# Stehsaer/nodey-audio-editor

Measured on AMD Instinct MI355X. Metric: stereo f32 sample-frames/s through the 4-node graph input->mix(2)->pitch->FFT-spectrum @48 kHz, higher is better.
Workload: dtype f32

## Files before the change

### include/nae_gpu.h

```cpp
#ifndef NAE_GPU_H
#define NAE_GPU_H
#include <stddef.h>
#include <stdint.h>

#ifdef __cplusplus
extern "C" {
#endif

#define NAE_ABI_VERSION 3

typedef enum nae_status {
    NAE_OK = 0,
    NAE_ERR_INVALID = -1,
    NAE_ERR_UNSUPPORTED = -2,
    NAE_ERR_HIP = -3,
    NAE_ERR_NOMEM = -4,
    NAE_ERR_STATE = -5
} nae_status;

typedef enum nae_fmt {
    NAE_FMT_S16 = 1, NAE_FMT_S32 = 2, NAE_FMT_FLT = 3, NAE_FMT_S16P = 6, NAE_FMT_S32P = 7, NAE_FMT_FLTP = 8
} nae_fmt;

typedef struct nae_ctx nae_ctx;
typedef struct nae_event nae_event;
typedef struct nae_stretch nae_stretch;
typedef struct nae_spectrum nae_spectrum;
typedef struct nae_fir nae_fir;
typedef struct nae_conv nae_conv;
typedef struct nae_eq nae_eq;
typedef struct nae_dyn nae_dyn;

int nae_abi_version(void);
int nae_device_count(void);
int nae_ctx_create(int device, nae_ctx** out);
int nae_ctx_destroy(nae_ctx* ctx);
int nae_ctx_set_stream(nae_ctx* ctx, void* hip_stream);
void* nae_ctx_stream(nae_ctx* ctx);
int nae_sync(nae_ctx* ctx);
int nae_poll(nae_ctx* ctx);
const char* nae_last_error(nae_ctx* ctx);
const char* nae_device_name(nae_ctx* ctx);

int nae_malloc(nae_ctx* ctx, size_t bytes, void** dptr);
int nae_free(nae_ctx* ctx, void* dptr);
int nae_malloc_host(nae_ctx* ctx, size_t bytes, void** hptr);
int nae_free_host(nae_ctx* ctx, void* hptr);
int nae_memcpy_h2d(nae_ctx* ctx, void* dst, const void* src_host, size_t bytes);
int nae_memcpy_d2h(nae_ctx* ctx, void* dst_host, const void* src, size_t bytes);
int nae_memcpy_d2d(nae_ctx* ctx, void* dst, const void* src, size_t bytes);
int nae_memset(nae_ctx* ctx, void* dst, int value, size_t bytes);

int nae_event_create(nae_ctx* ctx, nae_event** ev);
int nae_event_record(nae_ctx* ctx, nae_event* ev);
int nae_event_query(nae_event* ev);
int nae_ctx_wait_event(nae_ctx* ctx, nae_event* ev);
int nae_event_elapsed_ms(nae_event* start, nae_event* stop, float* ms);
int nae_event_destroy(nae_event* ev);

int nae_prof_enable(nae_ctx* ctx, int on);
int nae_prof_reset(nae_ctx* ctx);
int nae_prof_get(nae_ctx* ctx, int index, char* name, size_t name_cap, double* total_ms, uint64_t* launches);

int nae_debug_clock_ghz(nae_ctx* ctx, double* ghz);

int nae_debug_set(nae_ctx* ctx, const char* key, long long value);

int nae_debug_diff_u32(nae_ctx* ctx, const void* a, const void* b, size_t n_words, uint64_t* d_count);

int nae_fill_uniform_f32(nae_ctx* ctx, float* dst, size_t n_per_stream, size_t stream_stride, size_t n_streams,
                         uint64_t first_stream, uint64_t input_index);

typedef struct nae_sig {
    void* base;
    size_t stream_stride;
    size_t chan_stride;
    size_t frame_stride;
} nae_sig;

int nae_gain_f32(nae_ctx* ctx, const float* const* src_planes, float* const* dst_planes, int planes,
                 size_t elems, float volume);
int nae_gain_s16(nae_ctx* ctx, const int16_t* const* src_planes, int16_t* const* dst_planes, int planes,
                 size_t elems, float volume);
int nae_gain_s32(nae_ctx* ctx, const int32_t* const* src_planes, int32_t* const* dst_planes, int planes,
                 size_t elems, float volume);
int nae_gain_frame(nae_ctx* ctx, int fmt, const void* const* src_planes, void* const* dst_planes, size_t S,
                   int ch, float volume);

int nae_deinterleave_f32(nae_ctx* ctx, const float* src, float* const* dst_planes, size_t S, int ch);
int nae_interleave_f32(nae_ctx* ctx, const float* const* src_planes, float* dst, size_t S, int ch);
int nae_copy_sig_f32(nae_ctx* ctx, const nae_sig* src, const nae_sig* dst, size_t S, int ch, size_t n_streams);
int nae_gain_sig_f32(nae_ctx* ctx, const nae_sig* src, const nae_sig* dst, size_t S, int ch, size_t n_streams,
                     float volume);

int nae_amix_f32(nae_ctx* ctx, const float* const* inL, const float* const* inR, const float* vol_host, int n,
                 float* outL, float* outR, size_t S);
int nae_amix_sig_f32(nae_ctx* ctx, const nae_sig* inputs, const float* vol_host, int n, const nae_sig* out,
                     size_t S, size_t n_streams);

int nae_bimix_f32(nae_ctx* ctx, const float* ll, const float* lr, const float* rl, const float* rr, float bias,
                  float* outL, float* outR, size_t S);

int nae_bimix2_downmix_f32(nae_ctx* ctx, const float* l, const float* r, float* mono, size_t S);
int nae_bimix2_interleave_f32(nae_ctx* ctx, float* dst, const float* earlier, const float* later,
                              size_t unaligned, size_t aligned, int earlier_offset);

int nae_to_f32_interleaved(nae_ctx* ctx, int fmt, const void* const* planes, size_t S, int ch, float* dst);

int nae_clamp_f32(nae_ctx* ctx, float* data, size_t n);

typedef struct nae_stretch_plan {
    int pv_on, rs_on;
    double tempo_eff, rate_eff;
    int64_t ha_q24;
    int32_t d0;
    uint32_t r_q24[2];
    uint64_t step_q32;
    size_t out_len, mid_len, frames;
    int rs_first;
} nae_stretch_plan;
int nae_stretch_plan_make(double rate, double pitch, size_t in_len, nae_stretch_plan* plan);

int nae_stretch_block_f32(nae_ctx* ctx, double rate, double pitch, const nae_sig* src, size_t in_len, int ch,
                          size_t n_streams, const nae_sig* dst);
int nae_debug_pv_tile_phase(nae_ctx* ctx, double rate, double pitch, const nae_sig* src, size_t in_len, int ch,
                            size_t n_streams, int32_t* dst_host, size_t dst_capacity, size_t* n_tiles,
                            size_t* tile_frames);

#define NAE_STRETCH_PHASE_LOCK 1u
int nae_stretch_block_ex_f32(nae_ctx* ctx, double rate, double pitch, unsigned flags, const nae_sig* src, size_t in_len, int ch,
                             size_t n_streams, const nae_sig* dst);
int nae_debug_pv_tile_phase_ex(nae_ctx* ctx, double rate, double pitch, unsigned flags, const nae_sig* src, size_t in_len, int ch,
                               size_t n_streams, int32_t* dst_host, size_t dst_capacity, size_t* n_tiles, size_t* tile_frames);

int nae_stretch_create(nae_ctx* ctx, int sample_rate, int channels, float rate, float pitch, nae_stretch** h);
int nae_stretch_create_ex(nae_ctx* ctx, int sample_rate, int channels, float rate, float pitch, unsigned flags, nae_stretch** h);

int nae_stretch_plan_make_n(double rate, double pitch, int n_fft, size_t in_len, nae_stretch_plan* plan);
int nae_stretch_block_n_f32(nae_ctx* ctx, double rate, double pitch, unsigned flags, int n_fft, const nae_sig* src, size_t in_len, int ch,
                            size_t n_streams, const nae_sig* dst);
int nae_debug_pv_tile_phase_n(nae_ctx* ctx, double rate, double pitch, unsigned flags, int n_fft, const nae_sig* src, size_t in_len, int ch,
                              size_t n_streams, int32_t* dst_host, size_t dst_capacity, size_t* n_tiles, size_t* tile_frames);
int nae_stretch_create_n(nae_ctx* ctx, int sample_rate, int channels, float rate, float pitch, unsigned flags, int n_fft, nae_stretch** h);

int nae_stretch_formant_lifter(int sample_rate, int n_fft);
int nae_stretch_block_formant_f32(nae_ctx* ctx, double rate, double pitch, unsigned flags, int n_fft, int lifter,
                                  const nae_sig* src, size_t in_len, int ch, size_t n_streams, const nae_sig* dst);
int nae_stretch_create_formant(nae_ctx* ctx, int sample_rate, int channels, float rate, float pitch, unsigned flags,
                               int n_fft, int lifter, nae_stretch** h);

int nae_stretch_plan_make_shift(double rate, double pitch, double formant_ratio, int lifter, int n_fft, size_t in_len, nae_stretch_plan* plan);
int nae_stretch_block_formant_shift_f32(nae_ctx* ctx, double rate, double pitch, unsigned flags, int n_fft, int lifter, double formant_ratio,
                                        const nae_sig* src, size_t in_len, int ch, size_t n_streams, const nae_sig* dst);
int nae_stretch_create_formant_shift(nae_ctx* ctx, int sample_rate, int channels, float rate, float pitch, unsigned flags, int n_fft, int lifter,
                                     double formant_ratio, nae_stretch** h);

#define NAE_STRETCH_TRANSIENTS 4u
#define NAE_STRETCH_LINK_CHANNELS 16u
int nae_stretch_put(nae_stretch* h, const float* interleaved, size_t S);
int nae_stretch_put_host(nae_stretch* h, const float* interleaved_host, size_t S);
int nae_stretch_flush(nae_stretch* h);
size_t nae_stretch_available(nae_stretch* h);
int nae_stretch_receive(nae_stretch* h, float* dst, size_t max_frames, size_t* got);
int nae_stretch_receive_host(nae_stretch* h, float* dst_host, size_t max_frames, size_t* got);
int nae_stretch_destroy(nae_stretch* h);

typedef struct nae_wsola nae_wsola;
typedef struct nae_wsola_plan {
    int sample_rate, channels;
    double rate_eff, tempo_eff;
    int order;
    int overlap_len, seq_len, seek_len, sample_req;
    double nominal_skip;
    size_t in_len, flush_zeros;
    size_t n_seq;
    size_t td_out_len, aa_out_len, cu_out_len;
    size_t out_len;
} nae_wsola_plan;
int nae_wsola_plan_make(int sample_rate, int channels, double rate, double pitch, size_t in_len, nae_wsola_plan* plan);
int nae_wsola_block_f32(nae_ctx* ctx, int sample_rate, double rate, double pitch, const nae_sig* src, size_t in_len, int ch,
                        size_t n_streams, const nae_sig* dst, int32_t* offsets_dbg);
int nae_wsola_create(nae_ctx* ctx, int sample_rate, int channels, double rate, double pitch, nae_wsola** h);
int nae_wsola_put(nae_wsola* h, const float* interleaved, size_t S);
int nae_wsola_put_host(nae_wsola* h, const float* interleaved_host, size_t S);
int nae_wsola_flush(nae_wsola* h);
size_t nae_wsola_available(const nae_wsola* h);
int nae_wsola_receive(nae_wsola* h, float* dst, size_t max_frames, size_t* got);
int nae_wsola_receive_host(nae_wsola* h, float* dst_host, size_t max_frames, size_t* got);
int nae_wsola_destroy(nae_wsola* h);

typedef struct nae_swr nae_swr;
int nae_swr_create(nae_ctx* ctx, int in_fmt, int in_rate, int in_channels, int out_rate, nae_swr** h);
int nae_swr_convert_host(nae_swr* h, const void* const* planes_host, size_t n_in, float* outL_host, float* outR_host,
                         size_t max_out, size_t* n_out);
int nae_swr_convert(nae_swr* h, const void* const* planes_host, size_t n_in, float* outL_dev, float* outR_dev,
                    size_t max_out, size_t* n_out);
size_t nae_swr_buffered(nae_swr* h);
int nae_swr_destroy(nae_swr* h);
int nae_mono_to_stereo_f32(nae_ctx* ctx, const float* mono, float* dst_interleaved, size_t S, float gain);

size_t nae_spectrum_frames(size_t T);
int nae_spectrum_block_f32(nae_ctx* ctx, const nae_sig* src, size_t T, int ch, size_t n_streams, float* dst,
                           size_t dst_stream_stride);
size_t nae_spectrum_frames_ex(size_t T, int n_fft, int hop);
int nae_spectrum_block_ex_f32(nae_ctx* ctx, int n_fft, int hop, const nae_sig* src, size_t T, int ch, size_t n_streams, float* dst,
                              size_t dst_stream_stride);
int nae_spectrum_create(nae_ctx* ctx, int n_fft, int hop, int channels, nae_spectrum** h);
int nae_spectrum_put(nae_spectrum* h, const float* interleaved, size_t S);
size_t nae_spectrum_available(nae_spectrum* h);
int nae_spectrum_receive(nae_spectrum* h, float* dst, size_t max_frames, size_t* got);
int nae_spectrum_destroy(nae_spectrum* h);

int nae_fir_pick_n_fft(int n_taps);
int nae_fir_block_f32(nae_ctx* ctx, const float* taps_host, int n_taps, int n_fft, const nae_sig* src, size_t in_len, int ch, size_t n_streams,
                      const nae_sig* dst);
int nae_fir_create(nae_ctx* ctx, const float* taps_host, int n_taps, int n_fft, int channels, nae_fir** h);
int nae_fir_put(nae_fir* h, const float* interleaved, size_t S);
int nae_fir_put_host(nae_fir* h, const float* interleaved_host, size_t S);
int nae_fir_flush(nae_fir* h);
// ... 74 lines not shown
```

### nodey-audio-editor_amd/binding.py

```python
from __future__ import annotations

import ctypes as C
import os
import subprocess
from typing import Iterable, Optional, Sequence

import numpy as np

_HERE = os.path.dirname(os.path.abspath(__file__))

FMT_S16, FMT_S32, FMT_FLT, FMT_S16P, FMT_S32P, FMT_FLTP = 1, 2, 3, 6, 7, 8
FFT_N, HOP, BINS = 1024, 256, 513

EXPORTED_SYMBOLS = [
    "nae_abi_version", "nae_device_count", "nae_ctx_create", "nae_ctx_destroy", "nae_ctx_set_stream",
    "nae_ctx_stream", "nae_sync", "nae_poll", "nae_last_error", "nae_device_name", "nae_malloc", "nae_free",
    "nae_memcpy_h2d", "nae_memcpy_d2h", "nae_memcpy_d2d", "nae_memset", "nae_event_create", "nae_event_record",
    "nae_event_query", "nae_ctx_wait_event", "nae_debug_graph4_stages",
    "nae_event_elapsed_ms", "nae_event_destroy", "nae_prof_enable", "nae_prof_reset", "nae_prof_get",
    "nae_malloc_host", "nae_free_host", "nae_debug_clock_ghz", "nae_debug_set", "nae_debug_diff_u32", "nae_fill_uniform_f32", "nae_gain_f32", "nae_gain_s16", "nae_gain_s32", "nae_gain_frame",
    "nae_deinterleave_f32", "nae_interleave_f32", "nae_copy_sig_f32", "nae_gain_sig_f32", "nae_amix_f32",
    "nae_amix_sig_f32", "nae_bimix_f32", "nae_bimix2_downmix_f32", "nae_bimix2_interleave_f32",
    "nae_to_f32_interleaved", "nae_clamp_f32", "nae_stretch_plan_make", "nae_stretch_block_f32",
    "nae_debug_pv_tile_phase", "nae_stretch_block_ex_f32", "nae_debug_pv_tile_phase_ex", "nae_stretch_create_ex",
    "nae_stretch_plan_make_n", "nae_stretch_block_n_f32", "nae_debug_pv_tile_phase_n", "nae_stretch_create_n",
    "nae_stretch_formant_lifter", "nae_stretch_block_formant_f32", "nae_stretch_create_formant",
    "nae_stretch_plan_make_shift", "nae_stretch_block_formant_shift_f32", "nae_stretch_create_formant_shift", "nae_stretch_create", "nae_stretch_put", "nae_stretch_put_host", "nae_stretch_flush",
    "nae_stretch_available", "nae_stretch_receive", "nae_stretch_receive_host", "nae_stretch_destroy",
    "nae_swr_create", "nae_swr_convert_host", "nae_swr_convert", "nae_swr_buffered", "nae_swr_destroy", "nae_mono_to_stereo_f32",
    "nae_spectrum_frames", "nae_spectrum_block_f32", "nae_spectrum_frames_ex", "nae_spectrum_block_ex_f32", "nae_spectrum_create", "nae_spectrum_put",
    "nae_spectrum_available", "nae_spectrum_receive", "nae_spectrum_destroy", "nae_graph4_run",
    "nae_wsola_plan_make", "nae_wsola_block_f32", "nae_wsola_create", "nae_wsola_put", "nae_wsola_put_host",
    "nae_wsola_flush", "nae_wsola_available", "nae_wsola_receive", "nae_wsola_receive_host", "nae_wsola_destroy",
    "nae_fir_pick_n_fft", "nae_fir_block_f32", "nae_fir_design", "nae_fir_create", "nae_fir_put", "nae_fir_put_host", "nae_fir_flush",
    "nae_fir_available", "nae_fir_receive", "nae_fir_receive_host", "nae_fir_destroy",
    "nae_conv_pick_n_fft", "nae_conv_block_f32", "nae_conv_reverb_taps", "nae_conv_design_reverb", "nae_conv_create", "nae_conv_put",
    "nae_conv_put_host", "nae_conv_flush", "nae_conv_available", "nae_conv_receive", "nae_conv_receive_host", "nae_conv_destroy",
    "nae_eq_design", "nae_eq_block_f32", "nae_eq_create", "nae_eq_put", "nae_eq_put_host", "nae_eq_flush", "nae_eq_available", "nae_eq_receive",
    "nae_eq_receive_host", "nae_eq_destroy",
    "nae_dyn_design", "nae_dyn_block_f32", "nae_dyn_create", "nae_dyn_put", "nae_dyn_put_host", "nae_dyn_flush", "nae_dyn_available",
    "nae_dyn_receive", "nae_dyn_receive_host", "nae_dyn_destroy",
]


STRETCH_PHASE_LOCK = 1
STRETCH_TRANSIENTS = 4
STRETCH_LINK_CHANNELS = 16
FORMANT_SHIFT_MIN, FORMANT_SHIFT_MAX = 0.25, 4.0
FIR_SIZES = (512, 1024, 2048, 4096)
FIR_KINDS = {"lowpass": 0, "highpass": 1, "bandpass": 2, "bandstop": 3}
EQ_KINDS = ("peak", "lowshelf", "highshelf", "lowpass", "highpass", "notch")
HANDLE_PREFIXES = ("nae_stretch", "nae_wsola", "nae_fir", "nae_conv", "nae_eq", "nae_dyn")


class NaeError(RuntimeError):
    pass


def lib_path() -> str:
    return os.environ.get("NAE_GPU_LIB") or os.path.join(_HERE, "libnae_gpu.so")


def build_library(verbose: bool = False) -> str:
    r = subprocess.run(["make", "-C", _HERE, "-j4"], capture_output=True, text=True)
    if verbose or r.returncode:
        print(r.stdout[-4000:], r.stderr[-4000:])
    if r.returncode:
        raise NaeError("building libnae_gpu.so failed")
    return lib_path()


class Sig(C.Structure):
    _fields_ = [("base", C.c_void_p), ("stream_stride", C.c_size_t), ("chan_stride", C.c_size_t),
                ("frame_stride", C.c_size_t)]

    @staticmethod
    def interleaved(ptr: int, S: int, ch: int, shared: bool = False, stream_stride: Optional[int] = None) -> "Sig":
        ss = 0 if shared else (S * ch if stream_stride is None else stream_stride)
        return Sig(ptr, ss, 1, ch)

    @staticmethod
    def planar(ptr: int, S: int, ch: int, shared: bool = False, plane_stride: Optional[int] = None,
               stream_stride: Optional[int] = None) -> "Sig":
        ps = S if plane_stride is None else plane_stride
        ss = 0 if shared else (ps * ch if stream_stride is None else stream_stride)
        return Sig(ptr, ss, ps, 1)


class DynParams(C.Structure):
    _fields_ = [("threshold_db", C.c_double), ("slope", C.c_double), ("knee_db", C.c_double), ("alpha_attack", C.c_double),
                ("alpha_release", C.c_double), ("makeup_db", C.c_double), ("lookahead", C.c_int), ("link", C.c_int)]


class StretchPlan(C.Structure):
    _fields_ = [("pv_on", C.c_int), ("rs_on", C.c_int), ("tempo_eff", C.c_double), ("rate_eff", C.c_double),
                ("ha_q24", C.c_int64), ("d0", C.c_int32), ("r_q24", C.c_uint32 * 2), ("step_q32", C.c_uint64),
                ("out_len", C.c_size_t), ("mid_len", C.c_size_t), ("frames", C.c_size_t), ("rs_first", C.c_int)]


class WsolaPlan(C.Structure):
    _fields_ = [("sample_rate", C.c_int), ("channels", C.c_int), ("rate_eff", C.c_double), ("tempo_eff", C.c_double),
                ("order", C.c_int), ("overlap_len", C.c_int), ("seq_len", C.c_int), ("seek_len", C.c_int),
                ("sample_req", C.c_int), ("nominal_skip", C.c_double), ("in_len", C.c_size_t),
                ("flush_zeros", C.c_size_t), ("n_seq", C.c_size_t), ("td_out_len", C.c_size_t),
                ("aa_out_len", C.c_size_t), ("cu_out_len", C.c_size_t), ("out_len", C.c_size_t)]


class Graph4(C.Structure):
    _fields_ = [("in_a", Sig), ("in_b", Sig), ("vol_a", C.c_float), ("vol_b", C.c_float), ("mix_out", Sig),
                ("rate", C.c_double), ("pitch", C.c_double), ("pitch_out", Sig), ("spec_out", C.c_void_p),
                ("spec_stream_stride", C.c_size_t), ("S", C.c_size_t), ("n_streams", C.c_size_t)]


_lib = None


def load_library() -> C.CDLL:
    global _lib
    if _lib is not None:
        return _lib
    p = lib_path()
    if not os.path.exists(p):
        raise NaeError(f"{p} is missing: run `python -c 'import __graft_entry__ as g; g.build()'` (hipcc, gfx950)")
    lib = C.CDLL(p)
    vp, sz, i, u, f, d = C.c_void_p, C.c_size_t, C.c_int, C.c_uint, C.c_float, C.c_double
    P = C.POINTER
    sigs = {
        "nae_abi_version": (i, []), "nae_device_count": (i, []),
        "nae_ctx_create": (i, [i, P(vp)]), "nae_ctx_destroy": (i, [vp]), "nae_ctx_set_stream": (i, [vp, vp]),
        "nae_ctx_stream": (vp, [vp]), "nae_sync": (i, [vp]), "nae_poll": (i, [vp]),
        "nae_last_error": (C.c_char_p, [vp]), "nae_device_name": (C.c_char_p, [vp]),
        "nae_malloc": (i, [vp, sz, P(vp)]), "nae_free": (i, [vp, vp]),
        "nae_memcpy_h2d": (i, [vp, vp, vp, sz]), "nae_memcpy_d2h": (i, [vp, vp, vp, sz]),
        "nae_memcpy_d2d": (i, [vp, vp, vp, sz]), "nae_memset": (i, [vp, vp, i, sz]),
        "nae_event_create": (i, [vp, P(vp)]), "nae_event_record": (i, [vp, vp]),
        "nae_event_query": (i, [vp]), "nae_ctx_wait_event": (i, [vp, vp]), "nae_debug_graph4_stages": (i, [vp, P(Graph4), i]),
        "nae_event_elapsed_ms": (i, [vp, vp, P(f)]), "nae_event_destroy": (i, [vp]),
        "nae_prof_enable": (i, [vp, i]), "nae_prof_reset": (i, [vp]),
        "nae_prof_get": (i, [vp, i, C.c_char_p, sz, P(d), P(C.c_uint64)]),
        "nae_malloc_host": (i, [vp, sz, P(vp)]), "nae_free_host": (i, [vp, vp]),
        "nae_debug_clock_ghz": (i, [vp, P(C.c_double)]), "nae_debug_set": (i, [vp, C.c_char_p, C.c_longlong]),
        "nae_debug_diff_u32": (i, [vp, vp, vp, sz, vp]),
        "nae_fill_uniform_f32": (i, [vp, vp, sz, sz, sz, C.c_uint64, C.c_uint64]),
        "nae_gain_f32": (i, [vp, P(vp), P(vp), i, sz, f]), "nae_gain_s16": (i, [vp, P(vp), P(vp), i, sz, f]),
        "nae_gain_s32": (i, [vp, P(vp), P(vp), i, sz, f]),
        "nae_gain_frame": (i, [vp, i, P(vp), P(vp), sz, i, f]),
        "nae_deinterleave_f32": (i, [vp, vp, P(vp), sz, i]), "nae_interleave_f32": (i, [vp, P(vp), vp, sz, i]),
        "nae_copy_sig_f32": (i, [vp, P(Sig), P(Sig), sz, i, sz]),
        "nae_gain_sig_f32": (i, [vp, P(Sig), P(Sig), sz, i, sz, f]),
        "nae_amix_f32": (i, [vp, P(vp), P(vp), P(f), i, vp, vp, sz]),
        "nae_amix_sig_f32": (i, [vp, P(Sig), P(f), i, P(Sig), sz, sz]),
        "nae_bimix_f32": (i, [vp, vp, vp, vp, vp, f, vp, vp, sz]),
        "nae_bimix2_downmix_f32": (i, [vp, vp, vp, vp, sz]),
        "nae_bimix2_interleave_f32": (i, [vp, vp, vp, vp, sz, sz, i]),
        "nae_to_f32_interleaved": (i, [vp, i, P(vp), sz, i, vp]), "nae_clamp_f32": (i, [vp, vp, sz]),
        "nae_stretch_plan_make": (i, [d, d, sz, P(StretchPlan)]),
        "nae_stretch_block_f32": (i, [vp, d, d, P(Sig), sz, i, sz, P(Sig)]),
        "nae_debug_pv_tile_phase": (i, [vp, d, d, P(Sig), sz, i, sz, vp, sz, P(sz), P(sz)]),
        "nae_stretch_block_ex_f32": (i, [vp, d, d, u, P(Sig), sz, i, sz, P(Sig)]),
        "nae_debug_pv_tile_phase_ex": (i, [vp, d, d, u, P(Sig), sz, i, sz, vp, sz, P(sz), P(sz)]),
        "nae_stretch_create_ex": (i, [vp, i, i, f, f, u, P(vp)]),
        "nae_stretch_plan_make_n": (i, [d, d, i, sz, P(StretchPlan)]),
        "nae_stretch_block_n_f32": (i, [vp, d, d, u, i, P(Sig), sz, i, sz, P(Sig)]),
        "nae_debug_pv_tile_phase_n": (i, [vp, d, d, u, i, P(Sig), sz, i, sz, vp, sz, P(sz), P(sz)]),
        "nae_stretch_create_n": (i, [vp, i, i, f, f, u, i, P(vp)]),
        "nae_stretch_formant_lifter": (i, [i, i]),
        "nae_stretch_block_formant_f32": (i, [vp, d, d, u, i, i, P(Sig), sz, i, sz, P(Sig)]),
        "nae_stretch_create_formant": (i, [vp, i, i, f, f, u, i, i, P(vp)]),
        "nae_stretch_plan_make_shift": (i, [d, d, d, i, i, sz, P(StretchPlan)]),
        "nae_stretch_block_formant_shift_f32": (i, [vp, d, d, u, i, i, d, P(Sig), sz, i, sz, P(Sig)]),
        "nae_stretch_create_formant_shift": (i, [vp, i, i, f, f, u, i, i, d, P(vp)]),
        "nae_stretch_create": (i, [vp, i, i, f, f, P(vp)]),
        "nae_swr_create": (i, [vp, i, i, i, i, P(vp)]),
        "nae_swr_convert_host": (i, [vp, P(vp), sz, vp, vp, sz, P(sz)]), "nae_swr_convert": (i, [vp, P(vp), sz, vp, vp, sz, P(sz)]),
        "nae_swr_buffered": (sz, [vp]),
        "nae_swr_destroy": (i, [vp]), "nae_mono_to_stereo_f32": (i, [vp, vp, vp, sz, f]),
        "nae_spectrum_frames": (sz, [sz]), "nae_spectrum_block_f32": (i, [vp, P(Sig), sz, i, sz, vp, sz]),
        "nae_spectrum_frames_ex": (sz, [sz, i, i]), "nae_spectrum_block_ex_f32": (i, [vp, i, i, P(Sig), sz, i, sz, vp, sz]),
        "nae_spectrum_create": (i, [vp, i, i, i, P(vp)]), "nae_spectrum_put": (i, [vp, vp, sz]),
        "nae_spectrum_available": (sz, [vp]), "nae_spectrum_receive": (i, [vp, vp, sz, P(sz)]),
        "nae_spectrum_destroy": (i, [vp]), "nae_graph4_run": (i, [vp, P(Graph4)]),
        "nae_wsola_plan_make": (i, [i, i, d, d, sz, P(WsolaPlan)]),
        "nae_wsola_block_f32": (i, [vp, i, d, d, P(Sig), sz, i, sz, P(Sig), vp]),
        "nae_wsola_create": (i, [vp, i, i, d, d, P(vp)]),
        "nae_fir_pick_n_fft": (i, [i]), "nae_fir_block_f32": (i, [vp, vp, i, i, P(Sig), sz, i, sz, P(Sig)]),
        "nae_fir_design": (i, [i, i, d, d, i, vp]), "nae_fir_create": (i, [vp, vp, i, i, i, P(vp)]),
        "nae_conv_pick_n_fft": (i, [i]), "nae_conv_block_f32": (i, [vp, vp, i, i, i, P(Sig), sz, i, sz, P(Sig)]),
        "nae_conv_reverb_taps": (i, [i, d, d]), "nae_conv_design_reverb": (i, [i, d, d, d, d, C.c_uint64, i, vp]),
        "nae_conv_create": (i, [vp, vp, i, i, i, i, P(vp)]),
        "nae_eq_design": (i, [i, i, d, d, d, vp]), "nae_eq_block_f32": (i, [vp, vp, i, P(Sig), sz, i, sz, P(Sig)]),
        "nae_eq_create": (i, [vp, vp, i, i, P(vp)]),
        "nae_dyn_design": (i, [i, d, d, d, d, d, d, d, i, P(DynParams)]), "nae_dyn_block_f32": (i, [vp, P(DynParams), P(Sig), sz, i, sz, P(Sig)]),
        "nae_dyn_create": (i, [vp, P(DynParams), i, P(vp)]),
    }
    for prefix in HANDLE_PREFIXES:
        sigs.update({prefix + "_put": (i, [vp, vp, sz]), prefix + "_put_host": (i, [vp, vp, sz]), prefix + "_flush": (i, [vp]),
                     prefix + "_available": (sz, [vp]), prefix + "_receive": (i, [vp, vp, sz, P(sz)]),
                     prefix + "_receive_host": (i, [vp, vp, sz, P(sz)]), prefix + "_destroy": (i, [vp])})
    for name, (res, args) in sigs.items():
        fn = getattr(lib, name)
        fn.restype = res
        fn.argtypes = args
    _lib = lib
    return lib


class DeviceArray:

    def __init__(self, ctx: "Context", shape: Sequence[int], dtype=np.float32):
        self.ctx = ctx
        self.shape = tuple(int(x) for x in (shape if isinstance(shape, (tuple, list)) else (shape,)))
        self.dtype = np.dtype(dtype)
        self.nbytes = int(np.prod(self.shape, dtype=np.int64)) * self.dtype.itemsize
        p = C.c_void_p()
        ctx._ck(ctx.lib.nae_malloc(ctx.h, max(self.nbytes, 16), C.byref(p)))
        self.ptr = p.value
        ctx._allocs.add(self)

    @property
    def size(self) -> int:
        return self.nbytes // self.dtype.itemsize

    def at(self, elem_offset: int) -> int:
        return self.ptr + int(elem_offset) * self.dtype.itemsize

    def upload(self, host: np.ndarray) -> "DeviceArray":
        host = np.ascontiguousarray(host, dtype=self.dtype)
        assert host.nbytes == self.nbytes, (host.nbytes, self.nbytes)
        self.ctx._ck(self.ctx.lib.nae_memcpy_h2d(self.ctx.h, self.ptr, host.ctypes.data, self.nbytes))
        self.ctx.sync()
        return self

    def download(self) -> np.ndarray:
        out = np.empty(self.shape, self.dtype)
        self.ctx._ck(self.ctx.lib.nae_memcpy_d2h(self.ctx.h, out.ctypes.data, self.ptr, self.nbytes))
        self.ctx.sync()
        return out

    def zero(self) -> "DeviceArray":
        self.ctx._ck(self.ctx.lib.nae_memset(self.ctx.h, self.ptr, 0, self.nbytes))
        return self

    def free(self) -> None:
        if self.ptr:
            self.ctx.sync()
            self.ctx.lib.nae_free(self.ctx.h, self.ptr)
            self.ptr = 0
            self.ctx._allocs.discard(self)


def _ptr_array(ptrs: Iterable[int]):
    ptrs = list(ptrs)
    return (C.c_void_p * len(ptrs))(*ptrs)


class Context:

    def __init__(self, device: int = 0):
        self.lib = load_library()
        h = C.c_void_p()
        rc = self.lib.nae_ctx_create(device, C.byref(h))
        if rc != 0:
            why = ("no such device, or a bad assignment in $NAE_DEBUG" if rc == -1 else "no usable HIP device")
            raise NaeError(f"nae_ctx_create(device={device}) failed with {rc}: {why} — this library has no CPU fallback")
        self.h = h
        self.device = device
        self._allocs = set()
        self._pinned = {}

    def _ck(self, rc: int) -> None:
        if rc != 0:
            raise NaeError(f"nae error {rc}: {self.lib.nae_last_error(self.h).decode(errors='replace')}")

    def name(self) -> str:
        return self.lib.nae_device_name(self.h).decode()

    def sync(self) -> None:
        self._ck(self.lib.nae_sync(self.h))

    def poll(self) -> int:
        return self.lib.nae_poll(self.h)

    def set_stream(self, hip_stream: int) -> None:
        self._ck(self.lib.nae_ctx_set_stream(self.h, C.c_void_p(hip_stream)))

    def empty(self, shape, dtype=np.float32) -> DeviceArray:
        return DeviceArray(self, shape, dtype)

    def array(self, host: np.ndarray) -> DeviceArray:
        host = np.ascontiguousarray(host)
        return DeviceArray(self, host.shape, host.dtype).upload(host)

    def close(self) -> None:
        if self.h:
            for a in list(self._allocs):
                a.free()
            self.lib.nae_ctx_destroy(self.h)
            self.h = None

    def __enter__(self):
        return self

    def __exit__(self, *a):
        self.close()

    def debug_set(self, key: str, value: int) -> "Context":
        self._ck(self.lib.nae_debug_set(self.h, key.encode(), int(value)))
        return self

    def event(self) -> C.c_void_p:
        e = C.c_void_p()
        self._ck(self.lib.nae_event_create(self.h, C.byref(e)))
        return e

    def destroy_event(self, ev) -> None:
        rc = self.lib.nae_event_destroy(ev)
        if rc:
            raise NaeError(f"nae_event_destroy failed: {rc}")

    def record(self, ev) -> None:
        self._ck(self.lib.nae_event_record(self.h, ev))

    def query(self, ev) -> int:
        rc = self.lib.nae_event_query(ev)
        if rc < 0:
            raise NaeError(f"nae_event_query failed: {rc}")
        return rc

    def wait_event(self, ev) -> None:
        self._ck(self.lib.nae_ctx_wait_event(self.h, ev))

    def elapsed_ms(self, a, b) -> float:
        ms = C.c_float()
        rc = self.lib.nae_event_elapsed_ms(a, b, C.byref(ms))
        if rc:
            raise NaeError(f"nae_event_elapsed_ms failed: {rc}")
        return float(ms.value)

    def prof_enable(self, on: bool = True) -> None:
        self._ck(self.lib.nae_prof_enable(self.h, 1 if on else 0))

    def prof_reset(self) -> None:
        self._ck(self.lib.nae_prof_reset(self.h))

    def prof_report(self) -> dict:
        out = {}
        n = self.lib.nae_prof_get(self.h, -1, None, 0, None, None)
        for k in range(n):
            name = C.create_string_buffer(128)
            ms, cnt = C.c_double(), C.c_uint64()
            self.lib.nae_prof_get(self.h, k, name, 128, C.byref(ms), C.byref(cnt))
            out[name.value.decode()] = (ms.value, cnt.value)
        return out

    def pinned(self, shape, dtype=np.float32) -> np.ndarray:
        shape = tuple(int(x) for x in (shape if isinstance(shape, (tuple, list)) else (shape,)))
        nbytes = int(np.prod(shape, dtype=np.int64)) * np.dtype(dtype).itemsize
        p = C.c_void_p()
        self._ck(self.lib.nae_malloc_host(self.h, max(nbytes, 16), C.byref(p)))
        buf = (C.c_char * max(nbytes, 16)).from_address(p.value)
        arr = np.frombuffer(buf, dtype=dtype, count=int(np.prod(shape, dtype=np.int64))).reshape(shape)
        self._pinned[arr.ctypes.data] = p.value
        return arr

    def free_pinned(self, arr: np.ndarray) -> None:
        p = self._pinned.pop(arr.ctypes.data, None)
        if p:
            self.sync()
            self.lib.nae_free_host(self.h, p)

    def diff_words(self, a: int, b: int, n_words: int, d_count: int) -> None:
        self._ck(self.lib.nae_debug_diff_u32(self.h, a, b, n_words, d_count))

    def clock_ghz(self) -> float:
        g = C.c_double()
        self._ck(self.lib.nae_debug_clock_ghz(self.h, C.byref(g)))
        return g.value

    def fill_uniform(self, dst: int, n_per_stream: int, stream_stride: int, n_streams: int, first_stream: int = 0,
                     input_index: int = 0) -> None:
        self._ck(self.lib.nae_fill_uniform_f32(self.h, dst, n_per_stream, stream_stride, n_streams, first_stream,
                                               input_index))

    def gain(self, fmt_dtype, src_planes: Sequence[int], dst_planes: Sequence[int], elems: int, volume: float):
        fn = {np.dtype(np.float32): self.lib.nae_gain_f32, np.dtype(np.int16): self.lib.nae_gain_s16,
              np.dtype(np.int32): self.lib.nae_gain_s32}[np.dtype(fmt_dtype)]
        self._ck(fn(self.h, _ptr_array(src_planes), _ptr_array(dst_planes), len(src_planes), elems, volume))

    def gain_frame(self, fmt: int, src_planes, dst_planes, S: int, ch: int, volume: float) -> int:
        return self.lib.nae_gain_frame(self.h, fmt, _ptr_array(src_planes), _ptr_array(dst_planes), S, ch, volume)

    def deinterleave(self, src: int, dst_planes: Sequence[int], S: int, ch: int):
        self._ck(self.lib.nae_deinterleave_f32(self.h, src, _ptr_array(dst_planes), S, ch))

    def interleave(self, src_planes: Sequence[int], dst: int, S: int, ch: int):
        self._ck(self.lib.nae_interleave_f32(self.h, _ptr_array(src_planes), dst, S, ch))

    def copy_sig(self, src: Sig, dst: Sig, S: int, ch: int, n_streams: int):
        self._ck(self.lib.nae_copy_sig_f32(self.h, C.byref(src), C.byref(dst), S, ch, n_streams))

    def gain_sig(self, src: Sig, dst: Sig, S: int, ch: int, n_streams: int, volume: float):
        self._ck(self.lib.nae_gain_sig_f32(self.h, C.byref(src), C.byref(dst), S, ch, n_streams, volume))

    def amix(self, inL: Sequence[int], inR: Sequence[int], vol: Sequence[float], outL: int, outR: int, S: int):
        n = len(inL)
        v = (C.c_float * n)(*[float(x) for x in vol])
        self._ck(self.lib.nae_amix_f32(self.h, _ptr_array(inL), _ptr_array(inR), v, n, outL, outR, S))

    def amix_sig(self, inputs: Sequence[Sig], vol: Sequence[float], out: Sig, S: int, n_streams: int):
        n = len(inputs)
        arr = (Sig * n)(*inputs)
        v = (C.c_float * n)(*[float(x) for x in vol])
        self._ck(self.lib.nae_amix_sig_f32(self.h, arr, v, n, C.byref(out), S, n_streams))

    def bimix(self, ll, lr, rl, rr, bias: float, outL, outR, S: int):
        self._ck(self.lib.nae_bimix_f32(self.h, ll, lr, rl, rr, bias, outL, outR, S))

    def bimix2_downmix(self, l, r, mono, S: int):
        self._ck(self.lib.nae_bimix2_downmix_f32(self.h, l, r, mono, S))

    def bimix2_interleave(self, dst, earlier, later, unaligned: int, aligned: int, earlier_offset: int):
        self._ck(self.lib.nae_bimix2_interleave_f32(self.h, dst, earlier, later, unaligned, aligned, earlier_offset))

    def to_f32_interleaved(self, fmt: int, planes: Sequence[int], S: int, ch: int, dst: int) -> int:
        return self.lib.nae_to_f32_interleaved(self.h, fmt, _ptr_array(planes), S, ch, dst)

    def clamp(self, data: int, n: int):
        self._ck(self.lib.nae_clamp_f32(self.h, data, n))

    @staticmethod
    def stretch_plan(rate: float, pitch: float, in_len: int, n_fft: int = 1024, formant: int = 0,
                     formant_ratio: Optional[float] = None) -> StretchPlan:
        pl = StretchPlan()
        if formant_ratio is not None:
            rc = load_library().nae_stretch_plan_make_shift(rate, pitch, formant_ratio, formant, n_fft, in_len, C.byref(pl))
        elif n_fft == 1024:
            rc = load_library().nae_stretch_plan_make(rate, pitch, in_len, C.byref(pl))
        else:
            rc = load_library().nae_stretch_plan_make_n(rate, pitch, n_fft, in_len, C.byref(pl))
        if rc:
            raise NaeError(f"nae_stretch_plan_make({rate}, {pitch}, n_fft={n_fft}) failed: {rc}")
        return pl

    def stretch_block(self, rate: float, pitch: float, src: Sig, in_len: int, ch: int, n_streams: int, dst: Sig,
                      phase_lock: bool = False, n_fft: int = 1024, formant: int = 0, transients: bool = False,
                      formant_ratio: Optional[float] = None, link_channels: bool = False):
        flags = (STRETCH_PHASE_LOCK if phase_lock else 0) | (STRETCH_TRANSIENTS if transients else 0) | (STRETCH_LINK_CHANNELS if link_channels else 0)
        if formant_ratio is not None:
            self._ck(self.lib.nae_stretch_block_formant_shift_f32(self.h, rate, pitch, flags, n_fft, formant, formant_ratio,
                                                                  C.byref(src), in_len, ch, n_streams, C.byref(dst)))
        elif formant:
            self._ck(self.lib.nae_stretch_block_formant_f32(self.h, rate, pitch, flags, n_fft, formant,
                                                            C.byref(src), in_len, ch, n_streams, C.byref(dst)))
        elif n_fft != 1024 or transients or link_channels:
            self._ck(self.lib.nae_stretch_block_n_f32(self.h, rate, pitch, flags, n_fft, C.byref(src), in_len,
                                                      ch, n_streams, C.byref(dst)))
        elif phase_lock:
            self._ck(self.lib.nae_stretch_block_ex_f32(self.h, rate, pitch, STRETCH_PHASE_LOCK, C.byref(src), in_len, ch, n_streams,
                                                       C.byref(dst)))
        else:
            self._ck(self.lib.nae_stretch_block_f32(self.h, rate, pitch, C.byref(src), in_len, ch, n_streams, C.byref(dst)))

# ... 234 lines not shown
```

### nodey-audio-editor_amd/csrc/kernels_pvpipe.hip

```cpp
#include "stft_common.h"
#include "pv_roles.h"

namespace nae {

constexpr int kPipeSlots = 4;
constexpr int kPipeThreads = 64 * 4 * kPipeSlots;
constexpr size_t kPipeLdsTables = NAE_FFT_N * sizeof(float) + (kT1024Pad + 64 + kTwaCf) * sizeof(cf);

constexpr size_t kPipeLdsPerSlot = (2 * kPadScratchCf + kYCf) * sizeof(cf);
constexpr int pipe_ola_gens(int kG) { return kG >= 3 ? 2 : 3; }
constexpr size_t kPipeXchgPerSlot = 1024;
constexpr size_t pipe_lds_x_per_slot(int kG) { return kG == 1 ? kPipeXchgPerSlot : 3 * kPhasePad * sizeof(uint32_t) + (size_t)pipe_ola_gens(kG) * 3 * kOlaQuarter * sizeof(float); }
constexpr size_t pipe_lds(int kG) { return kPipeLdsTables + kPipeSlots * (kPipeLdsPerSlot + pipe_lds_x_per_slot(kG)); }
static_assert(2 * pipe_lds(1) <= 160 * 1024, "two workgroups per CU");
static_assert(pipe_lds(2) <= 160 * 1024 && pipe_lds(4) <= 160 * 1024, "one workgroup per CU");

__device__ unsigned g_cu_arrivals[8 * 4 * 16];

template <bool kUnit, int kG, bool kRich>
__global__ __launch_bounds__(kPipeThreads, kRich ? 4 : 8) void pv_pipe_kernel(SigViewD src, PvParams p, long long n_sc,
                                                                            const uint32_t* __restrict__ base_phase, OutViewD out, Tables tb)
{
    static_assert(kPipeSlots % kG == 0, "a unit's frames share a workgroup");
    static_assert(kG == 1 || kRich, "the frame-interleaved modes run one workgroup per CU");
    constexpr int kUnits = kPipeSlots / kG;
    constexpr int kDepth = kG == 1 ? 2 : 4;
    constexpr int kGens = pipe_ola_gens(kG);
    extern __shared__ __attribute__((aligned(16))) unsigned char smem[];
    float* hann; cf *t1024, *w64, *twa;
    stage_tables(smem, tb, kPipeThreads, hann, t1024, w64, twa);
    __shared__ int s_slot;
    if (kG == 1 && threadIdx.x == 0) s_slot = pipe_cu_arrival(g_cu_arrivals);
    __syncthreads();
    const int prio_slot = kG == 1 ? __builtin_amdgcn_readfirstlane(s_slot) : 0;

    const int wave = wave_id();
    const int role = wave / kPipeSlots, slot = wave % kPipeSlots;
    const int unit = slot / kG, j = slot % kG;
    const int lane = threadIdx.x & 63;
    PipeItem it;
    if (!pipe_item(p, (long long)kUnits * blockIdx.x + unit, n_sc, it)) return;
    const int c = it.c, n = it.n;
    const long long sc = it.sc, b0 = it.b0, b_end = it.b_end, f_first = it.f_first;

    cf* S1 = reinterpret_cast<cf*>(smem + kPipeLdsTables + slot * kPipeLdsPerSlot);
    cf* Y = S1 + kPadScratchCf;
    cf* S3 = Y + kYCf;
    unsigned char* xbase = smem + kPipeLdsTables + kPipeSlots * kPipeLdsPerSlot;
    constexpr size_t kXPer = pipe_lds_x_per_slot(kG);
    auto x_qa = [&](int sl, int gen) { return reinterpret_cast<uint32_t*>(xbase + sl * kXPer) + gen * kPhasePad; };
    auto x_inc = [&](int sl) { return reinterpret_cast<uint32_t*>(xbase + sl * kXPer) + 2 * kPhasePad; };
    auto x_ola = [&](int sl, int gen) { return reinterpret_cast<float*>(xbase + sl * kXPer + 3 * kPhasePad * sizeof(uint32_t)) + gen * 3 * kOlaQuarter; };

    const int steps = (n + kG - 1) / kG;
    const bool dense_shape = kG == 1 && p.ch == 2 && out.fs == 2 && out.cs == 1;
    const int T = steps + kDepth + (dense_shape ? 1 : 0);
    unsigned long long now = 0;
    if (kG > 1 && role == 2) __builtin_amdgcn_s_setprio(1);

    if (role == 0) {
        ChanView in{src.base + it.s_idx * src.ss + c * src.cs, src.fs, p.in_len};
        cf nxt[8], va[8];
        if (j < n) load_frame_raw<kUnit>(nxt, in, frame_start(p, f_first + j), lane);
        FftRegs R;
        if (kRich) load_fft_regs_lds(R, hann, twa, w64, lane);
#pragma unroll 1
        for (int t = 0; t < T; t++) {
            const bool cur = kG * t + j < n;
            pipe_barrier();
            if (kG == 1) pipe_prio(prio_slot, role, now);
            if (cur) r1_window_pass_a<kRich>(va, nxt, R, hann, twa, lane);
            pipe_barrier();
            if (kG == 1) now = __builtin_amdgcn_s_memtime();
            if (cur) {
                const FftLds L = make_fft_lds(S1, twa, w64, pipe_lane<!kRich>(lane));
                cf none[8];
                fft512_pad_bc_g<kRich, false>(va, L, R.tb, nullptr, none);
                r1_store_z(S1, L, va, lane);
                if (kG * (t + 1) + j < n) load_frame_raw<kUnit>(nxt, in, frame_start(p, f_first + kG * (t + 1) + j), lane);
            }
        }
    } else if (role <= 2) {
        PhaseLane P;
        P.init(tb, role - 1, lane);
        uint32_t qs[5], qp[5];
        P.load_base(qs, base_phase, p, it);
#pragma unroll
        for (int q = 0; q < 5; q++) qp[q] = 0;
        cf hx[5];
        uint32_t hqa[5] = {0, 0, 0, 0, 0};
#pragma unroll
        for (int q = 0; q < 5; q++) hx[q] = cf{0.0f, 0.0f};
#pragma unroll 1
        for (int t = 0; t < T; t++) {
            const int ia = kG * (t - 1) + j;
            const bool act_a = t >= 1 && ia < n;
            const long long fa = f_first + ia;
            const int ib = ia - kG;
            const bool act_b = kG > 1 && t >= 2 && ib < n;
            const long long fb = f_first + ib;
            pipe_barrier();
            if (kG == 1) pipe_prio(prio_slot, role, now);
            cf va[5];
            if (act_a) {
                cf A[2], B[2], z256{0.0f, 0.0f};
                P.read_z(S1, A, B, z256);
                P.split(A, B, z256, va);
            }
            if (kG > 1) {
                uint32_t inc[5] = {0, 0, 0, 0, 0};
                if (act_b && fb >= b0) {
                    uint32_t pv[5] = {0, 0, 0, 0, 0};
                    if (fb != 0) P.read5(j > 0 ? x_qa(slot - 1, (t - 1) & 1) : x_qa(slot + kG - 1, t & 1), pv);
                    P.inc_of_frame(p, fb, hqa, pv, inc);
                }
                P.write5(x_inc(slot), inc);
            }
            pipe_barrier();
            if (kG == 1) now = __builtin_amdgcn_s_memtime();
            uint32_t qa[5] = {0, 0, 0, 0, 0};
            if (act_a) P.phases(va, qa);
            if (kG == 1) {
                if (act_a) {
                    if (fa >= b0) {
                        if (fa == 0) {
#pragma unroll
                            for (int q = 0; q < 5; q++) qs[q] += qa[q];
                        } else {
                            const unsigned d = (unsigned)(frame_start(p, fa) - frame_start(p, fa - 1));
                            const unsigned R = (d == (unsigned)p.d0) ? p.r_q24_0 : p.r_q24_1;
                            uint32_t inc[5];
                            P.inc_items(qa, qp, d, R, inc);
#pragma unroll
                            for (int q = 0; q < 5; q++) qs[q] += inc[q];
                        }
                    }
#pragma unroll
                    for (int q = 0; q < 5; q++) qp[q] = qa[q];
                    if (fa == p.carry_frame) P.carry_store(p, sc, qs);
                    if (fa >= b0) P.synth_items(Y, va, qs, qa);
                }
            } else {
                if (act_a) P.write5(x_qa(slot, t & 1), qa);
                if (act_b) {
                    uint32_t iv[kG][5], mine[5];
#pragma unroll
                    for (int i2 = 0; i2 < kG; i2++) P.read5(x_inc(slot - j + i2), iv[i2]);
                    r2_running_phase<kG>(qs, mine, iv, j);
                    if (fb == p.carry_frame) P.carry_store(p, sc, mine);
                    if (fb >= b0) P.synth_items(Y, hx, mine, hqa);
                }
                if (act_a) {
#pragma unroll
                    for (int q = 0; q < 5; q++) { hx[q] = va[q]; hqa[q] = qa[q]; }
                }
            }
        }
    } else {
        float* optr = out.base + it.s_idx * out.ss + c * out.cs;
        const BlockOut bo{optr, out.fs, (out.fs == 1) && ((reinterpret_cast<uintptr_t>(optr) & 15) == 0)};
        float r0[4] = {0.0f, 0.0f, 0.0f, 0.0f}, r1[4] = {0.0f, 0.0f, 0.0f, 0.0f}, r2[4] = {0.0f, 0.0f, 0.0f, 0.0f};
        float y0[4] = {0.0f, 0.0f, 0.0f, 0.0f};
        FftRegs R;
        if (kRich) load_fft_regs_lds(R, hann, twa, w64, lane);
        bool had = false;
        const bool dense = dense_shape && ((reinterpret_cast<uintptr_t>(optr - c) & 15) == 0);
        int pend_be = -1;
        auto xchg = [&]() { return reinterpret_cast<cf*>(xbase + (size_t)(slot & ~1) * kPipeXchgPerSlot); };
#pragma unroll 1
        for (int t = 0; t < T; t++) {
            const int iz = kG * (t - (kDepth - (kG == 1 ? 0 : 1))) + j;
            const long long fz = f_first + iz;
            const bool active = iz >= 0 && iz < n && fz >= b0;
            pipe_barrier();
            if (kG == 1) pipe_prio(prio_slot, role, now);
            if (kG == 1 && pend_be >= 0) {
                const int lx = pipe_lane<!kRich>(lane);
                const cf* XB = xchg();
                r3_store_dense_half(optr - c, pend_be, c, lds_ld(XB + (0 + c) * 64 + lx), lds_ld(XB + (2 + c) * 64 + lx), lx);
                pend_be = -1;
            }
            cf zs[8];
            float4 oq[3];
            const bool finish = kG > 1 && had && fz - kG - 3 >= b0;
            if (finish) {
                const int lq = pipe_lane<!kRich>(lane);
#pragma unroll
                for (int i = 3; i >= 1; i--) {
                    int sl, gen;
                    r3_quarter_source<kG>(slot, j, i, t, kGens, sl, gen);
                    oq[i - 1] = *reinterpret_cast<const float4*>(x_ola(sl, gen) + (i - 1) * kOlaQuarter + 4 * lq);
                }
            }
            if (active) {
                const int la = pipe_lane<!kRich>(lane);
                const cf* Zi = Y + la;
                const cf* ta = twa + la;
#pragma unroll
                for (int r = 0; r < 8; r++) zs[r] = lds_ld(Zi + 64 * r);
                if (kRich) {
                    fft512_pad_a_tw(zs, R.ta);
                } else {
                    cf tw[7];
#pragma unroll
                    for (int q = 0; q < 7; q++) tw[q] = lds_ld(ta + 64 * q);
                    fft512_pad_a_tw(zs, tw);
                }
            }
            if (finish) {
                float o[4];
                r3_ola_finish(oq, y0, o);
                r3_store_block(p, it, bo, fz - kG - 3, o, pipe_lane<!kRich>(lane));
            }
            pipe_barrier();
            if (kG == 1) now = __builtin_amdgcn_s_memtime();
            had = active;
            if (active) {
                const int lb = pipe_lane<!kRich>(lane);
                const FftLds L = make_fft_lds(S3, twa, w64, lb);
                const cf* hw = reinterpret_cast<const cf*>(hann) + lb;
                cf wn[8];
                fft512_pad_bc_g<kRich, !kRich>(zs, L, R.tb, hw, wn);
                if (kRich) {
#pragma unroll
                    for (int r = 0; r < 8; r++) wn[r] = R.w[r];
                }
                float y[4][4];
                r3_window(zs, wn, y);
                if (kG == 1) {
                    float o[4];
                    r3_ola_shift(r0, r1, r2, y, o);
                    const long long be = fz - 3;
                    if (dense && be >= b0 && be < b_end && (be + 1) * NAE_HOP <= p.mid_len) {
                        const int lx = pipe_lane<!kRich>(lane);
                        cf* XB = xchg();
                        lds_st(XB + (2 * c + 0) * 64 + lx, cf{o[0], o[1]});
                        lds_st(XB + (2 * c + 1) * 64 + lx, cf{o[2], o[3]});
                        pend_be = (int)be;
                    } else {
                        r3_store_block(p, it, bo, be, o, pipe_lane<!kRich>(lane));
                    }
                } else {
                    float* po = x_ola(slot, t % kGens) + 4 * lb;
#pragma unroll
                    for (int q = 1; q < 4; q++) *reinterpret_cast<float4*>(po + (q - 1) * kOlaQuarter) = float4{y[q][0], y[q][1], y[q][2], y[q][3]};
#pragma unroll
                    for (int i = 0; i < 4; i++) y0[i] = y[0][i];
                }
            }
        }
    }
}

constexpr int flow_ola_gens(int kG) { return kG == 1 ? 0 : kG == 2 ? 4 : 3; }
constexpr size_t kFlowBuf = kPadScratchCf * sizeof(cf);
constexpr size_t flow_lds_per_slot(int kG)
{
    return 4 * kFlowBuf + (kG == 1 ? 0 : 4 * kPhasePad * sizeof(uint32_t) + (size_t)flow_ola_gens(kG) * 3 * kOlaQuarter * sizeof(float));
}
constexpr size_t flow_lds(int kG) { return kPipeSlots * flow_lds_per_slot(kG); }
static_assert(flow_lds(1) <= 160 * 1024 && flow_lds(2) <= 160 * 1024 && flow_lds(4) <= 160 * 1024, "one workgroup per CU");

template <bool kUnit, int kG>
__global__ __launch_bounds__(kPipeThreads, 4) void pv_flow_kernel(SigViewD src, PvParams p, long long n_sc, const uint32_t* __restrict__ base_phase,
                                                                  OutViewD out, Tables tb)
{
    static_assert(kPipeSlots % kG == 0, "a unit's frames share a workgroup");
    constexpr int kUnits = kPipeSlots / kG;
    constexpr int kGens = flow_ola_gens(kG);
    constexpr size_t kPer = flow_lds_per_slot(kG);
    extern __shared__ __attribute__((aligned(16))) unsigned char smem[];
// ... 49 lines not shown
#pragma unroll
        for (int q = 0; q < 5; q++) qp[q] = 0;
        cf x1[5], x2[5];
        uint32_t qa1[5] = {0, 0, 0, 0, 0}, qa2[5] = {0, 0, 0, 0, 0};
        uint32_t pcur[5] = {0, 0, 0, 0, 0};
#pragma unroll
        for (int q = 0; q < 5; q++) { x1[q] = cf{0.0f, 0.0f}; x2[q] = cf{0.0f, 0.0f}; }
#pragma unroll 1
        for (int t = 0; t < T; t++) {
            const int ia = kG * (t - 1) + j;
            const bool act_a = t >= 1 && ia < n;
            const long long fa = f_first + ia;
            const int ib = ia - kG;
            const bool act_b = kG > 1 && t >= 2 && ib < n;
            const long long fb = f_first + ib;
            const int ic = ib - kG;
            const bool act_c = kG > 1 && t >= 3 && ic < n;
            const long long fc = f_first + ic;
            const int gen = t & 1, old = gen ^ 1;
            pipe_barrier();
            cf A[2], B[2], z256{0.0f, 0.0f};
            if (act_a) P.read_z(x_z(slot, old), A, B, z256);
            uint32_t pv[5] = {0, 0, 0, 0, 0}, pnext[5] = {0, 0, 0, 0, 0}, iv[kG > 1 ? kG : 1][5];
            if (kG > 1) {
                if (j > 0) {
                    P.read5(x_qa(slot - 1, old), pv);
                } else {
                    P.read5(x_qa(slot + kG - 1, old), pnext);
#pragma unroll
                    for (int q = 0; q < 5; q++) pv[q] = pcur[q];
                }
                if (act_c) {
#pragma unroll
                    for (int i2 = 0; i2 < kG; i2++) P.read5(x_inc(slot - j + i2, old), iv[i2]);
                }
            }
            cf va[5];
            uint32_t qa[5] = {0, 0, 0, 0, 0};
            if (act_a) {
                P.split(A, B, z256, va);
                P.phases(va, qa);
            }
            if (kG == 1) {
                if (act_a) {
                    if (fa >= b0) {
                        uint32_t inc[5];
                        P.inc_of_frame(p, fa, qa, qp, inc);
#pragma unroll
                        for (int q = 0; q < 5; q++) qs[q] += inc[q];
                    }
#pragma unroll
                    for (int q = 0; q < 5; q++) qp[q] = qa[q];
                    if (fa == p.carry_frame) P.carry_store(p, sc, qs);
                    if (fa >= b0) P.synth_items(x_y(slot, gen), va, qs, qa);
                }
            } else {
                if (act_a) P.write5(x_qa(slot, gen), qa);
                uint32_t inc[5] = {0, 0, 0, 0, 0};
                if (act_b && fb >= b0) P.inc_of_frame(p, fb, qa1, pv, inc);
                P.write5(x_inc(slot, gen), inc);
                if (act_c) {
                    uint32_t mine[5];
                    r2_running_phase<(kG > 1 ? kG : 1)>(qs, mine, iv, j);
                    if (fc == p.carry_frame) P.carry_store(p, sc, mine);
                    if (fc >= b0) P.synth_items(x_y(slot, gen), x2, mine, qa2);
                }
#pragma unroll
                for (int q = 0; q < 5; q++) { x2[q] = x1[q]; qa2[q] = qa1[q]; pcur[q] = pnext[q]; }
                if (act_a) {
#pragma unroll
                    for (int q = 0; q < 5; q++) { x1[q] = va[q]; qa1[q] = qa[q]; }
                }
            }
        }
    } else {
        float* optr = out.base + it.s_idx * out.ss + c * out.cs;
        const BlockOut bo{optr, out.fs, (out.fs == 1) && ((reinterpret_cast<uintptr_t>(optr) & 15) == 0)};
        float r0[4] = {0.0f, 0.0f, 0.0f, 0.0f}, r1[4] = {0.0f, 0.0f, 0.0f, 0.0f}, r2[4] = {0.0f, 0.0f, 0.0f, 0.0f};
        float y0[4] = {0.0f, 0.0f, 0.0f, 0.0f};
        FftRegs R;
        load_fft_regs_global(R, tb, lane);
        bool had = false;
        const bool dense = dense_shape && ((reinterpret_cast<uintptr_t>(optr - c) & 15) == 0);
        int pend_be = -1;
        cf keep{0.0f, 0.0f};
#pragma unroll 1
        for (int t = 0; t < T; t++) {
            const int iz = kG * (t - kR3Lag) + j;
            const long long fz = f_first + iz;
            const bool active = iz >= 0 && iz < n && fz >= b0;
            pipe_barrier();
            cf zs[8];
            cf* Yi = x_y(slot, (t & 1) ^ 1);
            cf xh{0.0f, 0.0f};
            if (kG == 1 && pend_be >= 0) xh = lds_ld(x_y(slot ^ 1, t & 1) + 512 + lane);
            float4 oq[3];
            const bool finish = kG > 1 && had && fz - kG - 3 >= b0;
            if (finish) {
#pragma unroll
                for (int i = 3; i >= 1; i--) {
                    int sl, gen;
                    r3_quarter_source<kG>(slot, j, i, t, kGens > 0 ? kGens : 1, sl, gen);
                    oq[i - 1] = *reinterpret_cast<const float4*>(x_ola(sl, gen) + (i - 1) * kOlaQuarter + 4 * lane);
                }
            }
            if (active) {
#pragma unroll
                for (int r = 0; r < 8; r++) zs[r] = lds_ld(Yi + lane + 64 * r);
            }
            if (kG == 1 && pend_be >= 0) {
                r3_store_dense_half(optr - c, pend_be, c, c == 0 ? keep : xh, c == 0 ? xh : keep, lane);
                pend_be = -1;
            }
            if (finish) {
                float o[4];
                r3_ola_finish(oq, y0, o);
                r3_store_block(p, it, bo, fz - kG - 3, o, lane);
            }
            had = active;
            if (active) {
                fft512_pad_a_tw(zs, R.ta);
                const FftLds L = make_fft_lds(Yi, nullptr, nullptr, lane);
                cf none[8];
                fft512_pad_bc_g<true, false>(zs, L, R.tb, nullptr, none);
                float y[4][4];
                r3_window(zs, R.w, y);
                if (kG == 1) {
                    float o[4];
                    r3_ola_shift(r0, r1, r2, y, o);
                    const long long be = fz - 3;
                    if (dense && be >= b0 && be < b_end && (be + 1) * NAE_HOP <= p.mid_len) {
                        lds_st(Yi + 512 + lane, c == 0 ? cf{o[2], o[3]} : cf{o[0], o[1]});
                        keep = c == 0 ? cf{o[0], o[1]} : cf{o[2], o[3]};
                        pend_be = (int)be;
                    } else {
                        r3_store_block(p, it, bo, be, o, lane);
                    }
                } else {
                    float* po = x_ola(slot, t % (kGens > 0 ? kGens : 1)) + 4 * lane;
#pragma unroll
                    for (int q = 1; q < 4; q++) *reinterpret_cast<float4*>(po + (q - 1) * kOlaQuarter) = float4{y[q][0], y[q][1], y[q][2], y[q][3]};
#pragma unroll
                    for (int i = 0; i < 4; i++) y0[i] = y[0][i];
                }
            }
        }
    }
}

}

using namespace nae;

template <int kG, typename K>
static int pv_launch(nae_ctx* ctx, const char* name, K kernel, size_t lds, const PvJob& j)
{
    const Tables tb{ctx->d_w512, ctx->d_t1024, ctx->d_hann};
    return nae_launch_tiles(ctx, name, "pv_pipe_kernel: grid too large", kernel, j.n_sc * j.p.n_tiles, kPipeSlots / kG, kPipeThreads, lds, j.src, j.p,
                            j.n_sc, j.phase_ws, j.out, tb);
}

template <int kG, bool kRich>
static int pipe_launch(nae_ctx* ctx, const PvJob& j)
{
    return with_flags(j.unit_stride, [&](auto u) { return pv_launch<kG>(ctx, "pv_pipe_kernel", &pv_pipe_kernel<u.value, kG, kRich>, pipe_lds(kG), j); });
}
template <int kG>
static int flow_launch(nae_ctx* ctx, const PvJob& j)
{
    return with_flags(j.unit_stride, [&](auto u) { return pv_launch<kG>(ctx, "pv_flow_kernel", &pv_flow_kernel<u.value, kG>, flow_lds(kG), j); });
}

int nae_launch_pv_pipe(nae_ctx* ctx, const PvJob& j, int frames_per_step)
{
    const long long items = j.n_sc * j.p.n_tiles;
    if (items == 0) return NAE_OK;
    if (frames_per_step != 1 && frames_per_step != 2 && frames_per_step != 4) return nae_fail(ctx, NAE_ERR_INVALID, "pv_pipe_kernel: frames per step");
    const int units = kPipeSlots / frames_per_step;
    const long long groups = (items + units - 1) / units;
    const bool one_per_cu = groups <= (long long)ctx->n_cu && !ctx->pv_lean;
    if (one_per_cu && (ctx->pv_flow >= 2 || (ctx->pv_flow == 1 && frames_per_step == 1))) {
        if (frames_per_step == 1) return flow_launch<1>(ctx, j);
        if (frames_per_step == 2) return flow_launch<2>(ctx, j);
        return flow_launch<4>(ctx, j);
    }
    if (frames_per_step == 1) return with_flags(one_per_cu, [&](auto rich) { return pipe_launch<1, rich.value>(ctx, j); });
    if (frames_per_step == 2) return pipe_launch<2, true>(ctx, j);
    return pipe_launch<4, true>(ctx, j);
}
```

### nodey-audio-editor_amd/csrc/kernels_stft.hip

```cpp
#include "stft_common.h"
#include <stdlib.h>

namespace nae {

constexpr size_t kLdsPhase = kLdsTablesPad + kWaves * kPadScratchCf * sizeof(cf);
static_assert(3 * kLdsPhase <= 160 * 1024, "three workgroups per CU");
template <bool kUnit>
__global__ __launch_bounds__(kThreads, 6) void pv_phase_kernel(SigViewD src, PvParams p, long long n_items,
                                                              uint32_t* __restrict__ sums, Tables tb)
{
    extern __shared__ __attribute__((aligned(16))) unsigned char smem[];
    float* hann; cf *t1024, *w64, *twa;
    stage_tables(smem, tb, kThreads, hann, t1024, w64, twa);
    __syncthreads();
    const int lane = threadIdx.x & 63;
    cf* scratch = reinterpret_cast<cf*>(smem + kLdsTablesPad) + wave_id() * kPadScratchCf;
    const long long item = (long long)blockIdx.x * kWaves + wave_id();
    if (item >= n_items) return;
    const WaveTile w = wave_tile(item, p.n_tiles, p.ch);
    const long long s_idx = w.s_idx;
    const int tile = w.tile, c = w.c;
    if (tile >= p.skip_from) return;
    ChanView in{src.base + s_idx * src.ss + c * src.cs, src.fs, p.in_len};
    const int kl = kl_of_lane(lane);
// ... 130 lines not shown
        const float4* t1 = reinterpret_cast<const float4*>(stab + rs_slot(ph + 1, p.rot) * kRsRow);
        float coef[NAE_RS_TAPS];
#pragma unroll
        for (int q = 0; q < NAE_RS_TAPS / 4; q++) {
            const float4 a = t0[q], b = t1[q];
            coef[4 * q + 0] = a.x + alpha * (b.x - a.x);
            coef[4 * q + 1] = a.y + alpha * (b.y - a.y);
            coef[4 * q + 2] = a.z + alpha * (b.z - a.z);
            coef[4 * q + 3] = a.w + alpha * (b.w - a.w);
        }
        const int o = (int)(idx - (NAE_RS_TAPS / 2 - 1) - m_lo);
        const bool odd = (o & 1) != 0;
        float cz[NAE_RS_TAPS + 1];
        cz[0] = coef[0];
#pragma unroll
        for (int i = 1; i < NAE_RS_TAPS; i++) cz[i] = odd ? coef[i - 1] : coef[i];
        cz[NAE_RS_TAPS] = coef[NAE_RS_TAPS - 1];
        const int q0 = (o - (odd ? 1 : 0)) >> 1;
#pragma unroll
        for (int k = 0; k < NS; k++) {
            if (s0 + k < n_streams) {
                const float4* st = reinterpret_cast<const float4*>(stage + (size_t)k * 2 * span_alloc) + q0;
                float4 x[NAE_RS_TAPS / 2];
#pragma unroll
                for (int t = 0; t < NAE_RS_TAPS / 2; t++) x[t] = st[t];
                const float2 xe = *reinterpret_cast<const float2*>(st + NAE_RS_TAPS / 2);
                const float e0 = 0.0f + cz[0] * x[0].x, e1 = 0.0f + cz[0] * x[0].y;
                float a0 = odd ? 0.0f : e0, a1 = odd ? 0.0f : e1;
#pragma unroll
                for (int i = 1; i < NAE_RS_TAPS; i++) {
                    const float xl = (i & 1) ? x[i >> 1].z : x[i >> 1].x, xr = (i & 1) ? x[i >> 1].w : x[i >> 1].y;
                    a0 += cz[i] * xl;
                    a1 += cz[i] * xr;
                }
                const float f0 = a0 + cz[NAE_RS_TAPS] * xe.x, f1 = a1 + cz[NAE_RS_TAPS] * xe.y;
                a0 = odd ? f0 : a0;
                a1 = odd ? f1 : a1;
                if (live) {
                    float* ob = out.base + (s0 + k) * out.ss;
                    if (out_pair) {
                        *reinterpret_cast<float2*>(ob + 2 * j) = float2{a0, a1};
                    } else {
                        ob[j * out.fs] = a0;
                        ob[out.cs + j * out.fs] = a1;
                    }
                }
            }
        }
    }
}

template <bool kStereo, int NS>
__global__ __launch_bounds__(kRsThreads) void resample_tile_kernel(SigViewD src, RsParams p, const float* __restrict__ tab,
                                                           OutViewD out, int span_alloc, long long n_streams)
{
    extern __shared__ __attribute__((aligned(16))) unsigned char rs_smem[];
    float* stab = reinterpret_cast<float*>(rs_smem);
    float* stage = stab + (NAE_RS_PHASES + 1) * kRsRow;
    rs_fill_table(stab, tab, p.rot);
    const long long s0 = (long long)blockIdx.y * NS;
    const long long j0 = p.j_begin + (long long)blockIdx.x * p.tile_out;
    long long j1 = j0 + p.tile_out;
    if (j1 > p.out_len) j1 = p.out_len;
    const unsigned long long lo0 = (unsigned long long)j0 * p.step_q32, hi0 = __umul64hi((unsigned long long)j0, p.step_q32);
    const unsigned long long lo1 = (unsigned long long)(j1 - 1) * p.step_q32, hi1 = __umul64hi((unsigned long long)(j1 - 1), p.step_q32);
    const long long idx_first = (long long)((hi0 << 32) | (lo0 >> 32));
    const long long idx_last = (long long)((hi1 << 32) | (lo1 >> 32));
    const long long m_lo = (idx_first - (NAE_RS_TAPS / 2 - 1)) & ~3ll;
    const long long m_hi = idx_last + NAE_RS_TAPS / 2 + 1;
    const int span = (int)(m_hi - m_lo);
    if (kStereo) {
#pragma unroll 1
        for (int k = 0; k < NS; k++) {
            if (s0 + k >= n_streams) break;
            const float* v0 = src.base + (s0 + k) * src.ss;
            const float* v1 = v0 + src.cs;
            float* stg = stage + (size_t)k * 2 * span_alloc;
            const bool vec = (src.fs == 1) && (((reinterpret_cast<uintptr_t>(v0) | reinterpret_cast<uintptr_t>(v1)) & 15) == 0);
            if (vec) {
                for (int i = 4 * threadIdx.x; i < span; i += 4 * 256) {
                    const long long m = m_lo + i;
                    float4 x, y;
                    if (m >= 0 && m + 4 <= p.src_len) {
                        x = *reinterpret_cast<const float4*>(v0 + m);
                        y = *reinterpret_cast<const float4*>(v1 + m);
                    } else {
                        float xe[4], ye[4];
#pragma unroll
                        for (int e = 0; e < 4; e++) {
                            const bool ok = (m + e >= 0) && (m + e < p.src_len);
                            xe[e] = ok ? v0[m + e] : 0.0f;
                            ye[e] = ok ? v1[m + e] : 0.0f;
                        }
                        x = float4{xe[0], xe[1], xe[2], xe[3]};
                        y = float4{ye[0], ye[1], ye[2], ye[3]};
                    }
                    *reinterpret_cast<float4*>(stg + 2 * i) = float4{x.x, y.x, x.y, y.y};
                    *reinterpret_cast<float4*>(stg + 2 * i + 4) = float4{x.z, y.z, x.w, y.w};
                }
            } else {
                for (int i = threadIdx.x; i < span; i += 256) {
                    const long long m = m_lo + i;
                    const bool ok = m >= 0 && m < p.src_len;
                    *reinterpret_cast<float2*>(stg + 2 * i) = float2{ok ? v0[m * src.fs] : 0.0f, ok ? v1[m * src.fs] : 0.0f};
                }
            }
        }
    } else {
        const float* v0 = src.base + s0 * src.ss;
        for (int c = 0; c < p.ch; c++) {
            const float* v = v0 + c * src.cs;
            float* st = stage + c * span_alloc;
            for (int i = threadIdx.x; i < span; i += 256) {
                const long long m = m_lo + i;
                st[i] = (m >= 0 && m < p.src_len) ? v[m * src.fs] : 0.0f;
            }
        }
    }
    __syncthreads();
    if (kStereo) {
        rs_apply_stereo<NS>(stab, stage, span_alloc, p, j0, j1, m_lo, out, s0, n_streams);
    } else {
        for (long long j = j0 + threadIdx.x; j < j1; j += 256) {
            const unsigned long long lo = (unsigned long long)j * p.step_q32;
            const unsigned long long hi = __umul64hi((unsigned long long)j, p.step_q32);
            const long long idx = (long long)((hi << 32) | (lo >> 32));
            const unsigned frac = (unsigned)lo;
            const unsigned ph = frac >> 25;
            const float alpha = (float)(frac & 0x1FFFFFFu) * (1.0f / 33554432.0f);
            const float* t0 = stab + rs_slot(ph, p.rot) * kRsRow;
            const float* t1 = stab + rs_slot(ph + 1, p.rot) * kRsRow;
            float coef[NAE_RS_TAPS];
#pragma unroll
            for (int i = 0; i < NAE_RS_TAPS; i++) coef[i] = t0[i] + alpha * (t1[i] - t0[i]);
            const int o = (int)(idx - (NAE_RS_TAPS / 2 - 1) - m_lo);
            for (int c = 0; c < p.ch; c++) {
                const float* st = stage + c * span_alloc + o;
                float a = 0.0f;
#pragma unroll
                for (int i = 0; i < NAE_RS_TAPS; i++) a += coef[i] * st[i];
                out.base[s0 * out.ss + c * out.cs + j * out.fs] = a;
            }
        }
    }
}

struct MixFuseD {
    const float* a; long long a_ss;
    const float* b; long long b_ss;
    float va, vb;
    float* mix; long long mix_ss, mix_cs, mix_fs;
};

template <int NS>
__global__ __launch_bounds__(kRsThreads) void mix_resample_tile_kernel(MixFuseD f, RsParams p, const float* __restrict__ tab, OutViewD out,
                                                               int span_alloc, long long n_streams)
{
    extern __shared__ __attribute__((aligned(16))) unsigned char rs_smem[];
    float* stab = reinterpret_cast<float*>(rs_smem);
    float* stage = stab + (NAE_RS_PHASES + 1) * kRsRow;
    const long long s0 = (long long)blockIdx.y * NS;
    const long long j0 = (long long)blockIdx.x * p.tile_out;
    long long j1 = j0 + p.tile_out;
    const bool last = j1 >= p.out_len;
    if (last) j1 = p.out_len;
    auto idx_of = [&](long long j) {
        const unsigned long long lo = (unsigned long long)j * p.step_q32, hi = __umul64hi((unsigned long long)j, p.step_q32);
        return (long long)((hi << 32) | (lo >> 32));
    };
    const long long idx_first = idx_of(j0), idx_last = idx_of(j1 - 1);
    const long long m_lo = (idx_first - (NAE_RS_TAPS / 2 - 1)) & ~3ll;
    const long long m_hi = idx_last + NAE_RS_TAPS / 2 + 1;
    const long long own_lo = blockIdx.x == 0 ? 0 : idx_first;
    const long long own_hi = last ? p.src_len : idx_of(j1);
    const bool mix_planar = f.mix_fs == 1;
    const long long m_end = last ? (p.src_len > m_hi ? p.src_len : m_hi) : m_hi;
    auto load = [&](long long m, float4 (&xa)[NS][2], float4 (&xb)[NS][2]) {
        const bool inside = m >= 0 && m + 4 <= p.src_len;
#pragma unroll
        for (int k = 0; k < NS; k++) {
            xa[k][0] = xa[k][1] = xb[k][0] = xb[k][1] = float4{0.0f, 0.0f, 0.0f, 0.0f};
            if (s0 + k < n_streams) {
                const float* __restrict__ a = f.a + (s0 + k) * f.a_ss;
                const float* __restrict__ b = f.b + (s0 + k) * f.b_ss;
                if (inside) {
                    xa[k][0] = *reinterpret_cast<const float4*>(a + 2 * m);
                    xa[k][1] = *reinterpret_cast<const float4*>(a + 2 * m + 4);
                    xb[k][0] = *reinterpret_cast<const float4*>(b + 2 * m);
                    xb[k][1] = *reinterpret_cast<const float4*>(b + 2 * m + 4);
                } else {
                    float ta[8], tb[8];
#pragma unroll
                    for (int e = 0; e < 4; e++) {
                        const bool ok = m + e >= 0 && m + e < p.src_len;
                        ta[2 * e] = ok ? a[2 * (m + e)] : 0.0f;
                        ta[2 * e + 1] = ok ? a[2 * (m + e) + 1] : 0.0f;
                        tb[2 * e] = ok ? b[2 * (m + e)] : 0.0f;
                        tb[2 * e + 1] = ok ? b[2 * (m + e) + 1] : 0.0f;
                    }
                    xa[k][0] = float4{ta[0], ta[1], ta[2], ta[3]}; xa[k][1] = float4{ta[4], ta[5], ta[6], ta[7]};
                    xb[k][0] = float4{tb[0], tb[1], tb[2], tb[3]}; xb[k][1] = float4{tb[4], tb[5], tb[6], tb[7]};
                }
            }
        }
    };
    auto finish = [&](long long m, const float4 (&xa)[NS][2], const float4 (&xb)[NS][2]) {
        bool own[4], in[4];
#pragma unroll
        for (int e = 0; e < 4; e++) {
            own[e] = m + e >= own_lo && m + e < own_hi;
            in[e] = m + e >= 0 && m + e < p.src_len;
        }
        const bool own_all = own[0] && own[3];
#pragma unroll
        for (int k = 0; k < NS; k++) {
            if (s0 + k < n_streams) {
                float y[8];
                const float av[8] = {xa[k][0].x, xa[k][0].y, xa[k][0].z, xa[k][0].w, xa[k][1].x, xa[k][1].y, xa[k][1].z, xa[k][1].w};
                const float bv[8] = {xb[k][0].x, xb[k][0].y, xb[k][0].z, xb[k][0].w, xb[k][1].x, xb[k][1].y, xb[k][1].z, xb[k][1].w};
#pragma unroll
                for (int i = 0; i < 8; i++) y[i] = in[i >> 1] ? (0.0f + av[i] * f.va) + bv[i] * f.vb : 0.0f;
                float* stg = stage + (size_t)k * 2 * span_alloc + 2 * (m - m_lo);
                if (m + 3 < m_hi) {
                    *reinterpret_cast<float4*>(stg) = float4{y[0], y[1], y[2], y[3]};
                    *reinterpret_cast<float4*>(stg + 4) = float4{y[4], y[5], y[6], y[7]};
                } else {
#pragma unroll
                    for (int e = 0; e < 4; e++)
                        if (m + e < m_hi) *reinterpret_cast<float2*>(stg + 2 * e) = float2{y[2 * e], y[2 * e + 1]};
                }
                float* __restrict__ mx = f.mix + (s0 + k) * f.mix_ss;
                if (own_all && mix_planar) {
                    *reinterpret_cast<float4*>(mx + m) = float4{y[0], y[2], y[4], y[6]};
                    *reinterpret_cast<float4*>(mx + f.mix_cs + m) = float4{y[1], y[3], y[5], y[7]};
                } else {
#pragma unroll
                    for (int e = 0; e < 4; e++)
                        if (own[e]) { mx[(m + e) * f.mix_fs] = y[2 * e]; mx[f.mix_cs + (m + e) * f.mix_fs] = y[2 * e + 1]; }
                }
            }
        }
    };
    {
        float4 xa[NS][2], xb[NS][2];
        const long long m = m_lo + 4 * threadIdx.x;
        const bool has = m < m_end;
        if (has) load(m, xa, xb);
        rs_fill_table(stab, tab, p.rot);
        if (has) finish(m, xa, xb);
    }
    for (long long m = m_lo + 4 * threadIdx.x + 4 * 256; m < m_end; m += 4 * 256) {
        float4 xa[NS][2], xb[NS][2];
        load(m, xa, xb);
        finish(m, xa, xb);
    }
    __syncthreads();
    rs_apply_stereo<NS>(stab, stage, span_alloc, p, j0, j1, m_lo, out, s0, n_streams);
}

}

using namespace nae;

static int rs_pick_rot(unsigned long long step_q32)
{
    int best = 0;
    long best_cost = -1;
    for (int rot = 0; rot < 4; rot++) {
        long cost = 0;
        for (int g = 0; g < 16; g++) {
            int n0[16] = {0}, n1[16] = {0};
            unsigned seen0[16], seen1[16];
            for (int l = 0; l < 16; l++) {
                const unsigned long long pos = (unsigned long long)(16 * g + l) * step_q32;
                const unsigned ph = (unsigned)(pos & 0xFFFFFFFFull) >> 25;
                const unsigned s0 = rs_slot(ph, rot), s1 = rs_slot(ph + 1, rot);
                bool dup0 = false, dup1 = false;
                for (int k = 0; k < l; k++) { dup0 |= seen0[k] == s0; dup1 |= seen1[k] == s1; }
                seen0[l] = s0; seen1[l] = s1;
                if (!dup0) n0[(5 * s0) & 15]++;
                if (!dup1) n1[(5 * s1) & 15]++;
            }
            int m0 = 0, m1 = 0;
            for (int b = 0; b < 16; b++) { m0 = n0[b] > m0 ? n0[b] : m0; m1 = n1[b] > m1 ? n1[b] : m1; }
            cost += m0 + m1;
        }
        if (best_cost < 0 || cost < best_cost) { best_cost = cost; best = rot; }
    }
    return best;
}

static int rs_pick_tile(double rho, long long* span_need)
{
    auto need = [&](int tile) { return (long long)(tile * rho) + NAE_RS_TAPS + 8 + 4; };
    const int tile = need(kRsOutWide) <= 1536 ? kRsOutWide : kRsOut;
    *span_need = need(tile);
    return tile;
}

size_t nae_pv_workspace_bytes(bool lock, int n_fft, size_t n_frames, int ch, size_t n_streams, int tile)
{
    const size_t recs = n_streams * ch * ((n_frames + tile - 1) / tile);
    return recs * nae_pv_record_pad(n_fft) * (lock ? 2 * sizeof(uint32_t) + sizeof(uint16_t) : sizeof(uint32_t));
}

int nae_pv_reserve_ws(nae_ctx* ctx, const nae_pv_run& r, size_t n_frames, int ch, size_t n_streams, int tile)
{
    if (r.forced) return NAE_OK;
    return nae_ws_reserve(ctx, &ctx->ws_phase, &ctx->ws_phase_bytes, nae_pv_workspace_bytes(r.lock, r.n_fft, n_frames, ch, n_streams, tile));
}

static PvJob make_pv_job(const nae_pv_run& r, const nae_stretch_plan& pl, const nae_sig* src, size_t in_len, int ch, size_t n_streams, int tile,
                         const nae_pv_segment* seg, uint32_t* phase_ws, const nae_sig* out)
{
    return PvJob{r.n_fft, make_pv_params(pl, in_len, ch, tile, seg), to_view(src), out ? to_out(out) : OutViewD{}, (long long)n_streams * ch,
                 src->frame_stride == 1, phase_ws, r.lifter, r.g, r.transients, r.link};
}

int nae_launch_pv_phase(nae_ctx* ctx, const nae_pv_run& r, const nae_stretch_plan* pl, const nae_sig* src, size_t in_len, int ch, size_t n_streams,
                        int tile, int synth_tile, uint32_t* phase_ws, const nae_pv_segment* seg)
{
    if (tile <= 0 || synth_tile < tile || synth_tile % tile) return nae_fail(ctx, NAE_ERR_INVALID, "phase tile must divide the synthesis tile");
    if (r.forced) return NAE_OK;
    PvJob j = make_pv_job(r, *pl, src, in_len, ch, n_streams, tile, seg, phase_ws, nullptr);
    PvParams& p = j.p;
    const long long n_sc = j.n_sc;
    if (n_sc * p.n_tiles == 0) return NAE_OK;
    const bool need_last = seg && seg->carry_out && !seg->carry_by_synth;
    const int step = synth_tile / tile;
    const int n_synth = (p.n_tiles + step - 1) / step;
    const int n_needed = need_last ? p.n_tiles : (n_synth - 1) * step;
    const uint32_t* carry_in = seg ? seg->carry_in : nullptr;
    uint32_t* carry_out = seg ? seg->carry_out : nullptr;
    const size_t pad = nae_pv_record_pad(r.n_fft);
    if (n_needed == 0) {
        hipError_t e = hipSuccess;
        if (!carry_in) {
            if (p.n_tiles != 1) e = hipMemsetAsync(phase_ws, 0, (size_t)n_sc * p.n_tiles * pad * sizeof(uint32_t), ctx->stream);
        }
        else if (p.n_tiles == 1)
            e = hipMemcpyAsync(phase_ws, carry_in, (size_t)n_sc * pad * sizeof(uint32_t), hipMemcpyDeviceToDevice, ctx->stream);
        else
            e = hipMemcpy2DAsync(phase_ws, (size_t)p.n_tiles * pad * sizeof(uint32_t), carry_in, pad * sizeof(uint32_t),
                                 pad * sizeof(uint32_t), (size_t)n_sc, hipMemcpyDeviceToDevice, ctx->stream);
        return nae_check(ctx, e, "phase base init");
    }
    p.skip_from = n_needed;
    const PvKernels pass1 = nae_pv_route_of(ctx, r).pass1;
    if (pass1 == PvKernels::kLock) {
        const size_t n_rec = (size_t)n_sc * p.n_tiles;
        uint32_t* maps = phase_ws + n_rec * kT1024Pad;
        uint16_t* sig16 = reinterpret_cast<uint16_t*>(maps + n_rec * kT1024Pad);
        return nae_launch_pvlock_phase(ctx, j, n_needed, maps, sig16, carry_in, carry_out);
    }
    if (pass1 == PvKernels::kAny) {
        const int rc = nae_launch_pvany_phase(ctx, j);
        if (rc) return rc;
    } else {
        const long long items = n_sc * p.n_tiles;
        const Tables tb{ctx->d_w512, ctx->d_t1024, ctx->d_hann};
        const int rc = with_flags(j.unit_stride, [&](auto unit) {
            return nae_launch_tiles(ctx, "pv_phase_kernel", "pv_phase_kernel: grid too large", pv_phase_kernel<unit.value>, items, kWaves, kThreads,
                                    kLdsPhase, j.src, p, items, phase_ws, tb);
        });
        if (rc) return rc;
    }
    return nae_launch_pv_scan(ctx, r.n_fft, pass1 == PvKernels::kAny ? "pv_any_scan_kernel" : "pv_scan_kernel", phase_ws, n_sc, p.n_tiles, carry_in,
                              carry_out, n_needed, r.transients);
}

int nae_launch_pv_synth(nae_ctx* ctx, const nae_pv_run& r, const nae_stretch_plan* pl, const nae_sig* src, size_t in_len, int ch, size_t n_streams,
                        int tile, int phase_tile, uint32_t* phase_ws, const nae_sig* out, const nae_pv_segment* seg, int frames_per_step)
{
    if (phase_tile <= 0 || tile < phase_tile || tile % phase_tile) return nae_fail(ctx, NAE_ERR_INVALID, "phase tile must divide the synthesis tile");
    PvJob j = make_pv_job(r, *pl, src, in_len, ch, n_streams, tile, seg, phase_ws, out);
    PvParams& p = j.p;
    const long long cnt = p.f_stop - p.f_origin;
    p.phase_step = tile / phase_tile;
    p.phase_tiles = (int)((cnt + phase_tile - 1) / phase_tile);
    p.base_zero = (p.n_tiles == 1 && p.phase_tiles == 1 && !(seg && seg->carry_in)) ? 1 : 0;
    if (seg && seg->carry_by_synth && seg->carry_out) {
        if (p.n_tiles != 1) return nae_fail(ctx, NAE_ERR_INVALID, "carry_by_synth needs a single synthesis tile");
        p.carry_out = seg->carry_out;
        p.carry_frame = p.f_stop - 1;
    }
    const PvKernels pass3 = nae_pv_route_of(ctx, r).pass3;
    if (pass3 == PvKernels::kEnv) return nae_launch_pvenv(ctx, j);
    if (pass3 == PvKernels::kLock) return nae_launch_pvlock_synth(ctx, j);
    if (pass3 == PvKernels::kAny) return nae_launch_pvany_synth(ctx, j);
    return nae_launch_pv_pipe(ctx, j, frames_per_step);
}

int nae_launch_resample(nae_ctx* ctx, const nae_stretch_plan* pl, const nae_sig* src, size_t src_len, int ch,
                        size_t n_streams, const float* d_tab, const nae_sig* out, size_t j_begin, size_t j_end)
{
    if (j_end <= j_begin || n_streams == 0) return NAE_OK;
    const size_t count = j_end - j_begin;
    const double rho = (double)pl->step_q32 / 4294967296.0;
    long long span_need = 0;
    const int tile_out = rs_pick_tile(rho, &span_need);
    RsParams p{pl->step_q32, (long long)src_len, (long long)j_end, ch, (long long)j_begin, rs_pick_rot(pl->step_q32), tile_out};
    const bool tiled = span_need <= kRsMaxSpan && !ctx->dbg_rs_direct;
    const int span_alloc = (int)((span_need + 3) & ~3ll);
    const int group = (tiled && ch == 2 && n_streams >= 4 && span_alloc <= 1536 && !ctx->dbg_rs_single) ? 4 : 1;
    const size_t lds = ((NAE_RS_PHASES + 1) * kRsRow + (size_t)ch * span_alloc * group) * sizeof(float);
    const unsigned gx = tiled ? (unsigned)((count + tile_out - 1) / tile_out) : (unsigned)((count + 255) / 256);
    const size_t per_launch = (size_t)65535 * group;
    for (size_t s0 = 0; s0 < n_streams; s0 += per_launch) {
        const size_t ns = (n_streams - s0 < per_launch) ? n_streams - s0 : per_launch;
        SigViewD sv = to_view(src);
        OutViewD ov = to_out(out);
        sv.base += (long long)s0 * sv.ss;
        ov.base += (long long)s0 * ov.ss;
        if (tiled && ch == 2 && group == 4)
            NAE_KLAUNCH(ctx, "resample_tile_kernel", (resample_tile_kernel<true, 4>), dim3(gx, (unsigned)((ns + 3) / 4)), dim3(256), lds,
                        ctx->stream, sv, p, d_tab, ov, span_alloc, (long long)ns);
        else if (tiled && ch == 2)
            NAE_KLAUNCH(ctx, "resample_tile_kernel", (resample_tile_kernel<true, 1>), dim3(gx, (unsigned)ns), dim3(256), lds, ctx->stream,
                        sv, p, d_tab, ov, span_alloc, (long long)ns);
        else if (tiled)
            NAE_KLAUNCH(ctx, "resample_tile_kernel", (resample_tile_kernel<false, 1>), dim3(gx, (unsigned)ns), dim3(256), lds, ctx->stream,
                        sv, p, d_tab, ov, span_alloc, (long long)ns);
        else
            NAE_KLAUNCH(ctx, "resample_kernel", resample_kernel, dim3(gx, (unsigned)ns), dim3(256), 0, ctx->stream, sv, p,
                        (long long)ns, d_tab, ov);
        int rc = nae_check(ctx, hipGetLastError(), "resample kernel");
        if (rc) return rc;
    }
    return NAE_OK;
}

int nae_launch_mix_resample(nae_ctx* ctx, const nae_stretch_plan* pl, const nae_sig* a, const nae_sig* b, float va, float vb,
                            const nae_sig* mix_out, size_t S, size_t n_streams, const float* d_tab, const nae_sig* out)
{
    const double rho = (double)pl->step_q32 / 4294967296.0;
    long long span_need = 0;
    const int tile_out = rs_pick_tile(rho, &span_need);
    const int span_alloc = (int)((span_need + 3) & ~3ll);
    auto inter16 = [](const nae_sig* v) {
        return v->chan_stride == 1 && v->frame_stride == 2 && (reinterpret_cast<uintptr_t>(v->base) & 15) == 0 && (v->stream_stride & 3) == 0;
    };
    const bool mix_ok = mix_out->frame_stride != 1 ||
                        ((reinterpret_cast<uintptr_t>(mix_out->base) & 15) == 0 && (mix_out->stream_stride & 3) == 0 &&
                         (mix_out->chan_stride & 3) == 0);
    if (ctx->dbg_no_mix_fuse || !inter16(a) || !inter16(b) || !mix_ok || span_need > kRsMaxSpan || span_alloc > 1536 || n_streams == 0 ||
        pl->mid_len == 0 || S == 0)
        return 1;
    RsParams p{pl->step_q32, (long long)S, (long long)pl->mid_len, 2, 0, rs_pick_rot(pl->step_q32), tile_out};
    const size_t lds = ((NAE_RS_PHASES + 1) * kRsRow + (size_t)2 * span_alloc * 4) * sizeof(float);
    const unsigned gx = (unsigned)((pl->mid_len + tile_out - 1) / tile_out);
    const size_t per_launch = (size_t)65535 * 4;
    for (size_t s0 = 0; s0 < n_streams; s0 += per_launch) {
        const size_t ns = (n_streams - s0 < per_launch) ? n_streams - s0 : per_launch;
        MixFuseD f;
        f.a = static_cast<const float*>(a->base) + s0 * a->stream_stride; f.a_ss = (long long)a->stream_stride;
        f.b = static_cast<const float*>(b->base) + s0 * b->stream_stride; f.b_ss = (long long)b->stream_stride;
        f.va = va; f.vb = vb;
        f.mix = static_cast<float*>(mix_out->base) + s0 * mix_out->stream_stride;
        f.mix_ss = (long long)mix_out->stream_stride; f.mix_cs = (long long)mix_out->chan_stride; f.mix_fs = (long long)mix_out->frame_stride;
        OutViewD ov = to_out(out);
        ov.base += (long long)s0 * ov.ss;
        NAE_KLAUNCH(ctx, "mix_resample_tile_kernel", (mix_resample_tile_kernel<4>), dim3(gx, (unsigned)((ns + 3) / 4)), dim3(256), lds,
                    ctx->stream, f, p, d_tab, ov, span_alloc, (long long)ns);
        int rc = nae_check(ctx, hipGetLastError(), "mix_resample_tile_kernel");
        if (rc) return rc;
    }
    return NAE_OK;
}
```

### nodey-audio-editor_amd/csrc/nae_api.hip

```cpp
#include "nae_internal.h"
#include <string>
#include <initializer_list>
#include <cmath>
#include <math.h>
#include <stdio.h>
#include <stdlib.h>
#include <string.h>
#include <new>

namespace nae { struct cf { float x, y; }; }

int nae_fail(nae_ctx* ctx, int code, const char* what)
{
    if (ctx) snprintf(ctx->err, sizeof ctx->err, "%s", what);
    return code;
}

int nae_check(nae_ctx* ctx, hipError_t e, const char* what)
{
    if (e == hipSuccess) return NAE_OK;
    if (ctx) snprintf(ctx->err, sizeof ctx->err, "%s: %s", what, hipGetErrorString(e));
    return NAE_ERR_HIP;
}

// ... 56 lines not shown
static void build_tables(std::vector<nae::cf>& w512, std::vector<nae::cf>& t1024, std::vector<float>& hann)
{
    const double two_pi = 6.283185307179586476925286766559;
    w512.resize(512);
    t1024.resize(513);
    hann.resize(1024);
    for (int k = 0; k < 512; k++) w512[k] = nae::cf{(float)cos(two_pi * k / 512.0), (float)(-sin(two_pi * k / 512.0))};
    for (int k = 0; k <= 512; k++) t1024[k] = nae::cf{(float)cos(two_pi * k / 1024.0), (float)(-sin(two_pi * k / 1024.0))};
    for (int n = 0; n < 1024; n++) hann[n] = (float)(0.5 - 0.5 * cos(two_pi * n / 1024.0));
}

double nae_bessel_i0(double x)
{
    double sum = 1.0, term = 1.0;
    const double q = x * x / 4.0;
    for (int k = 1; k < 64; k++) {
        term *= q / ((double)k * (double)k);
        sum += term;
        if (term < 1e-18 * sum) break;
    }
    return sum;
}

static void build_rs_table(double rate_eff, std::vector<float>& tab)
{
    const double pi = 3.14159265358979323846;
    const double c = NAE_RS_CUTOFF * (rate_eff > 1.0 ? 1.0 / rate_eff : 1.0);
    const double half = NAE_RS_TAPS / 2.0;
    const double i0b = nae_bessel_i0(NAE_RS_KAISER_BETA);
    tab.resize((NAE_RS_PHASES + 1) * NAE_RS_TAPS);
    for (int p = 0; p <= NAE_RS_PHASES; p++) {
        double row[NAE_RS_TAPS], sum = 0.0;
        for (int i = 0; i < NAE_RS_TAPS; i++) {
            const double x = (double)(i - (NAE_RS_TAPS / 2 - 1)) - (double)p / NAE_RS_PHASES;
            const double a = x / half;
            double w = 0.0;
            if (a > -1.0 && a < 1.0) w = nae_bessel_i0(NAE_RS_KAISER_BETA * sqrt(1.0 - a * a)) / i0b;
            else if (a == 1.0 || a == -1.0) w = 1.0 / i0b;
            const double arg = pi * c * x;
            const double sinc = (fabs(arg) < 1e-12) ? 1.0 : sin(arg) / arg;
            row[i] = c * sinc * w;
            sum += row[i];
        }
        for (int i = 0; i < NAE_RS_TAPS; i++) tab[p * NAE_RS_TAPS + i] = (float)(row[i] / sum);
    }
}

int nae_ensure_rs_table(nae_ctx* ctx, double rate_eff)
{
    if (ctx->d_rs_tab && ctx->rs_tab_rate == rate_eff) return NAE_OK;
    (void)nae_use_device(ctx);
    if (!ctx->d_rs_tab) {
        hipError_t e = hipMalloc((void**)&ctx->d_rs_tab, (NAE_RS_PHASES + 1) * NAE_RS_TAPS * sizeof(float));
        if (e != hipSuccess) return nae_check(ctx, e, "hipMalloc(rs table)");
    } else {
        hipError_t e = hipStreamSynchronize(ctx->stream);
        if (e != hipSuccess) return nae_check(ctx, e, "hipStreamSynchronize");
    }
    build_rs_table(rate_eff, ctx->h_rs_tab);
    hipError_t e = hipMemcpy(ctx->d_rs_tab, ctx->h_rs_tab.data(), ctx->h_rs_tab.size() * sizeof(float), hipMemcpyHostToDevice);
    if (e != hipSuccess) return nae_check(ctx, e, "hipMemcpy(rs table)");
    ctx->rs_tab_rate = rate_eff;
    return NAE_OK;
}

int nae_pick_pv_shape(nae_ctx* ctx, size_t frames, size_t n_sc, int* phase_tile, int* frames_per_step)
{
    const size_t n_cu = (size_t)(ctx->n_cu > 0 ? ctx->n_cu : 256);
    int fps = n_sc > 2 * n_cu ? 1 : n_sc > n_cu ? 2 : 4;
    if (n_sc > 2 * n_cu && n_sc <= 3 * n_cu) fps = 4;
    if (ctx->pv_fps == 1 || ctx->pv_fps == 2 || ctx->pv_fps == 4) fps = ctx->pv_fps;
    *frames_per_step = fps;
    if (ctx->pv_tile > 0) { *phase_tile = ctx->pv_tile; return ctx->pv_tile; }
    *phase_tile = 64;
    if (frames == 0 || n_sc == 0) return 64;
    if (ctx->pv_fps == 0 && 2 * n_sc <= n_cu) {
        const size_t want = 8 * n_cu / n_sc;
        if (want >= 2 && frames >= 128 * want) {
            size_t third = ((frames + want - 1) / want + 2) / 3;
            if (third < 64) third = 64;
            *frames_per_step = 1;
            *phase_tile = (int)third;
            return (int)(3 * third);
        }
    }
    const size_t kMinPhase = ctx->dbg_pv_min_ptile > 0 ? (size_t)ctx->dbg_pv_min_ptile : 16;
    const size_t max_synth = (frames + 63) / 64, max_phase = (frames + kMinPhase - 1) / kMinPhase;
    const size_t wg = (n_sc * (size_t)fps + 3) / 4;
    size_t n_synth = wg >= n_cu ? 1 : n_cu / wg;
    if (n_synth > max_synth) n_synth = max_synth;
    size_t n_phase = n_synth == 1 ? 1 : (24 * n_cu + n_sc - 1) / n_sc;
    if (n_phase > max_phase) n_phase = max_phase;
    size_t step = (n_phase + n_synth - 1) / n_synth;
    if (step < 1) step = 1;
    size_t pt = (frames + n_synth * step - 1) / (n_synth * step);
    if (pt < kMinPhase) pt = kMinPhase;
    if (pt * step < 64) pt = (64 + step - 1) / step;
    *phase_tile = (int)pt;
    return (int)(pt * step);
}

int nae_pick_tile(nae_ctx* ctx, int forced, size_t units, size_t n_sc, size_t resident, size_t min_tile, bool max_tiles_down)
{
    if (forced > 0) return forced;
    const size_t n_cu = (size_t)(ctx->n_cu > 0 ? ctx->n_cu : 256);
    if (units == 0 || n_sc == 0) return (int)min_tile;
    size_t n_tiles = (resident * n_cu + n_sc - 1) / n_sc;
    const size_t max_tiles = (units + (max_tiles_down ? 0 : min_tile - 1)) / min_tile;
    if (n_tiles > max_tiles) n_tiles = max_tiles;
    if (n_tiles < 1) n_tiles = 1;
    const size_t tile = (units + n_tiles - 1) / n_tiles;
    return (int)(tile < 0x40000000 ? tile : 0x40000000);
}

struct PvBlockShape { int tile, phase_tile, frames_per_step; };
static int pv_block_shape(nae_ctx* ctx, const nae_pv_run& r, size_t frames, int ch, size_t n_streams, PvBlockShape* s)
{
    const PvKernels pass3 = nae_pv_route_of(ctx, r).pass3;
    const size_t n_sc = n_streams * ch;
    s->frames_per_step = 1;
    if (pass3 == PvKernels::kShipped) s->tile = nae_pick_pv_shape(ctx, frames, n_sc, &s->phase_tile, &s->frames_per_step);
    else {
        const size_t min_tile = pass3 != PvKernels::kLock && ctx->dbg_pv_min_ptile > 0 ? (size_t)ctx->dbg_pv_min_ptile : 64;
        s->tile = s->phase_tile = nae_pick_tile(ctx, ctx->pv_tile, frames, n_sc, (size_t)nae_pv_resident(ctx, r, pass3), min_tile, false);
    }
    return nae_pv_reserve_ws(ctx, r, frames, ch, n_streams, s->phase_tile);
}

extern "C" {

int nae_abi_version(void) { return NAE_ABI_VERSION; }

int nae_device_count(void)
{
    int n = 0;
    if (hipGetDeviceCount(&n) != hipSuccess) return 0;
    return n;
}

int nae_debug_set(nae_ctx* ctx, const char* key, long long value)
{
    if (!ctx || !key) return NAE_ERR_INVALID;
    const std::string k(key);
    const bool flag = value == 0 || value == 1;
    const bool count = value >= 0 && value <= 0x7fffffffll;
    auto one_of = [&](std::initializer_list<long long> ok) { for (long long v : ok) if (v == value) return true; return false; };
    if (k == "pv_tile" && count) ctx->pv_tile = (int)value;
    else if (k == "fir_tile" && count) ctx->fir_tile = (int)value;
    else if (k == "conv_tile" && count) ctx->conv_tile = (int)value;
    else if (k == "conv_ring" && count) ctx->conv_ring = (int)value;
    else if (k == "pv_fps" && one_of({0, 1, 2, 4})) ctx->pv_fps = (int)value;
    else if (k == "pv_flow" && one_of({0, 1, 2})) ctx->pv_flow = (int)value;
    else if (k == "pv_lean" && flag) ctx->pv_lean = value != 0;
    else if (k == "pv_min_ptile" && count) ctx->dbg_pv_min_ptile = (int)value;
    else if (k == "rs_single" && flag) ctx->dbg_rs_single = value != 0;
    else if (k == "rs_direct" && flag) ctx->dbg_rs_direct = value != 0;
    else if (k == "no_mix_fuse" && flag) ctx->dbg_no_mix_fuse = value != 0;
    else if (k == "spec_generic" && flag) ctx->dbg_spec_generic = value != 0;
    else if (k == "spec_narrow" && flag) ctx->dbg_spec_narrow = value != 0;
    else if (k == "spec_chunk" && count) ctx->dbg_spec_chunk = (int)value;
    else if (k == "spec_any" && flag) ctx->dbg_spec_any = value != 0;
    else if (k == "pv_any" && flag) ctx->dbg_pv_any = value != 0;
    else if (k == "spec_fine" && count) ctx->dbg_spec_fine = (int)value;
    else if (k == "spec_fine_rounds" && count) ctx->dbg_spec_fine_rounds = (int)value;
    else if (k == "td_nc" && one_of({0, 1, 2, 4})) ctx->dbg_td_nc = (int)value;
    else if (k == "st_unfused" && flag) ctx->dbg_st_unfused = value != 0;
    else return nae_fail(ctx, NAE_ERR_INVALID, "nae_debug_set: unknown key or value out of range");
    return NAE_OK;
}

int nae_ctx_create(int device, nae_ctx** out)
{
    if (!out) return NAE_ERR_INVALID;
    *out = nullptr;
    int n = 0;
    if (hipGetDeviceCount(&n) != hipSuccess || n <= 0) return NAE_ERR_HIP;
    if (device < 0 || device >= n) return NAE_ERR_INVALID;
    if (hipSetDevice(device) != hipSuccess) return NAE_ERR_HIP;
    nae_ctx* ctx = new (std::nothrow) nae_ctx();
    if (!ctx) return NAE_ERR_NOMEM;
    ctx->device = device;
    hipDeviceProp_t prop;
    if (hipGetDeviceProperties(&prop, device) == hipSuccess) {
        snprintf(ctx->name, sizeof ctx->name, "%s (%s)", prop.name, prop.gcnArchName);
        if (prop.multiProcessorCount > 0) ctx->n_cu = prop.multiProcessorCount;
    }
    if (hipStreamCreateWithFlags(&ctx->stream, hipStreamNonBlocking) != hipSuccess) { delete ctx; return NAE_ERR_HIP; }
    ctx->own_stream = true;
    if (const char* e = getenv("NAE_DEBUG")) {
        std::string all(e);
        size_t pos = 0;
        while (pos < all.size()) {
            size_t end = all.find(',', pos);
            if (end == std::string::npos) end = all.size();
            const std::string kv = all.substr(pos, end - pos);
            const size_t eq = kv.find('=');
            if (!kv.empty() && (eq == std::string::npos || nae_debug_set(ctx, kv.substr(0, eq).c_str(), atoll(kv.c_str() + eq + 1)) != NAE_OK)) {
                fprintf(stderr, "libnae_gpu: NAE_DEBUG: bad assignment '%s'\n", kv.c_str());
                (void)hipStreamDestroy(ctx->stream);
                delete ctx;
                return NAE_ERR_INVALID;
            }
            pos = end + 1;
        }
    }
    std::vector<nae::cf> w512, t1024;
    std::vector<float> hann;
    build_tables(w512, t1024, hann);
    bool ok = hipMalloc((void**)&ctx->d_w512, 512 * sizeof(nae::cf)) == hipSuccess &&
              hipMalloc((void**)&ctx->d_t1024, 520 * sizeof(nae::cf)) == hipSuccess &&
              hipMalloc((void**)&ctx->d_hann, 1024 * sizeof(float)) == hipSuccess &&
              hipMalloc((void**)&ctx->d_spec_ctr, 64) == hipSuccess && hipMemset(ctx->d_spec_ctr, 0, 64) == hipSuccess;
    ok = ok && hipMemcpy(ctx->d_w512, w512.data(), 512 * sizeof(nae::cf), hipMemcpyHostToDevice) == hipSuccess &&
         hipMemcpy(ctx->d_t1024, t1024.data(), 513 * sizeof(nae::cf), hipMemcpyHostToDevice) == hipSuccess &&
         hipMemcpy(ctx->d_hann, hann.data(), 1024 * sizeof(float), hipMemcpyHostToDevice) == hipSuccess;
    if (!ok) { nae_ctx_destroy(ctx); return NAE_ERR_HIP; }
    *out = ctx;
    return NAE_OK;
}

int nae_ctx_destroy(nae_ctx* ctx)
{
    if (!ctx) return NAE_OK;
    (void)nae_use_device(ctx);
    if (ctx->stream) (void)hipStreamSynchronize(ctx->stream);
    prof_collect(ctx);
    if (ctx->d_w512) (void)hipFree(ctx->d_w512);
    if (ctx->d_t1024) (void)hipFree(ctx->d_t1024);
    if (ctx->d_hann) (void)hipFree(ctx->d_hann);
    if (ctx->d_spec_ctr) (void)hipFree(ctx->d_spec_ctr);
    nae_spec_any_free(ctx);
    if (ctx->d_rs_tab) (void)hipFree(ctx->d_rs_tab);
    if (ctx->ws_phase) (void)hipFree(ctx->ws_phase);
    if (ctx->ws_mid) (void)hipFree(ctx->ws_mid);
    nae_wsola_cache_free(ctx);
    nae_fir_cache_free(ctx);
    nae_conv_cache_free(ctx);
    nae_eq_cache_free(ctx);
    if (ctx->own_stream && ctx->stream) (void)hipStreamDestroy(ctx->stream);
    delete ctx;
    return NAE_OK;
}

int nae_ctx_set_stream(nae_ctx* ctx, void* hip_stream)
{
    if (!ctx) return NAE_ERR_INVALID;
    if (ctx->stream) (void)hipStreamSynchronize(ctx->stream);
    if (ctx->own_stream && ctx->stream) (void)hipStreamDestroy(ctx->stream);
    ctx->stream = static_cast<hipStream_t>(hip_stream);
    ctx->own_stream = false;
    return NAE_OK;
}

void* nae_ctx_stream(nae_ctx* ctx) { return ctx ? (void*)ctx->stream : nullptr; }

int nae_sync(nae_ctx* ctx)
{
    if (!ctx) return NAE_ERR_INVALID;
    (void)nae_use_device(ctx);
    return nae_check(ctx, hipStreamSynchronize(ctx->stream), "hipStreamSynchronize");
}

int nae_poll(nae_ctx* ctx)
{
    if (!ctx) return NAE_ERR_INVALID;
    (void)nae_use_device(ctx);
    hipError_t e = hipStreamQuery(ctx->stream);
    if (e == hipSuccess) return 1;
    if (e == hipErrorNotReady) return 0;
    return nae_check(ctx, e, "hipStreamQuery");
}

const char* nae_last_error(nae_ctx* ctx) { return ctx ? ctx->err : "null context"; }
const char* nae_device_name(nae_ctx* ctx) { return ctx ? ctx->name : ""; }

int nae_malloc(nae_ctx* ctx, size_t bytes, void** dptr)
{
    if (!ctx || !dptr) return NAE_ERR_INVALID;
    *dptr = nullptr;
    if (bytes == 0) bytes = 16;
    (void)nae_use_device(ctx);
    hipError_t e = hipMalloc(dptr, bytes);
    if (e != hipSuccess) { nae_check(ctx, e, "hipMalloc"); return NAE_ERR_NOMEM; }
    return NAE_OK;
}
int nae_free(nae_ctx* ctx, void* dptr)
{
    if (!dptr) return NAE_OK;
    if (ctx) (void)nae_use_device(ctx);
    return nae_check(ctx, hipFree(dptr), "hipFree");
}
int nae_malloc_host(nae_ctx* ctx, size_t bytes, void** hptr)
{
    if (!ctx || !hptr) return NAE_ERR_INVALID;
    *hptr = nullptr;
    if (bytes == 0) bytes = 16;
    (void)nae_use_device(ctx);
    hipError_t e = hipHostMalloc(hptr, bytes, hipHostMallocDefault);
    if (e != hipSuccess) { nae_check(ctx, e, "hipHostMalloc"); return NAE_ERR_NOMEM; }
    return NAE_OK;
}
int nae_free_host(nae_ctx* ctx, void* hptr)
{
    if (!hptr) return NAE_OK;
    if (ctx) (void)nae_use_device(ctx);
    return nae_check(ctx, hipHostFree(hptr), "hipHostFree");
}
int nae_memcpy_h2d(nae_ctx* ctx, void* dst, const void* src, size_t bytes)
{
    if (!ctx || (bytes && (!dst || !src))) return NAE_ERR_INVALID;
    (void)nae_use_device(ctx);
    return nae_check(ctx, hipMemcpyAsync(dst, src, bytes, hipMemcpyHostToDevice, ctx->stream), "hipMemcpyAsync(h2d)");
}
int nae_memcpy_d2h(nae_ctx* ctx, void* dst, const void* src, size_t bytes)
{
    if (!ctx || (bytes && (!dst || !src))) return NAE_ERR_INVALID;
    (void)nae_use_device(ctx);
    return nae_check(ctx, hipMemcpyAsync(dst, src, bytes, hipMemcpyDeviceToHost, ctx->stream), "hipMemcpyAsync(d2h)");
}
int nae_memcpy_d2d(nae_ctx* ctx, void* dst, const void* src, size_t bytes)
// ... 26 lines not shown
    return nae_check(ctx, hipEventRecord(ev->ev, ctx->stream), "hipEventRecord");
}
int nae_event_query(nae_event* ev)
{
    if (!ev) return NAE_ERR_INVALID;
    const hipError_t e = hipEventQuery(ev->ev);
    if (e == hipSuccess) return 1;
    if (e == hipErrorNotReady) return 0;
    return NAE_ERR_HIP;
}
int nae_ctx_wait_event(nae_ctx* ctx, nae_event* ev)
{
    if (!ctx || !ev) return NAE_ERR_INVALID;
    (void)nae_use_device(ctx);
    return nae_check(ctx, hipStreamWaitEvent(ctx->stream, ev->ev, 0), "hipStreamWaitEvent");
}
int nae_event_elapsed_ms(nae_event* start, nae_event* stop, float* ms)
{
    if (!start || !stop || !ms) return NAE_ERR_INVALID;
    if (hipEventSynchronize(stop->ev) != hipSuccess) return NAE_ERR_HIP;
    return hipEventElapsedTime(ms, start->ev, stop->ev) == hipSuccess ? NAE_OK : NAE_ERR_HIP;
}
int nae_event_destroy(nae_event* ev)
{
    if (!ev) return NAE_OK;
    (void)hipEventDestroy(ev->ev);
    delete ev;
    return NAE_OK;
}

int nae_prof_enable(nae_ctx* ctx, int on)
{
    if (!ctx) return NAE_ERR_INVALID;
    prof_collect(ctx);
    ctx->prof_on = on != 0;
    return NAE_OK;
}
int nae_prof_reset(nae_ctx* ctx)
{
    if (!ctx) return NAE_ERR_INVALID;
    prof_collect(ctx);
    ctx->prof_slots.clear();
    return NAE_OK;
}
int nae_prof_get(nae_ctx* ctx, int index, char* name, size_t name_cap, double* total_ms, uint64_t* launches)
{
    if (!ctx) return NAE_ERR_INVALID;
    prof_collect(ctx);
    if (index < 0 || index >= (int)ctx->prof_slots.size()) return (int)ctx->prof_slots.size();
    if (name && name_cap) snprintf(name, name_cap, "%s", ctx->prof_slots[index].name);
    if (total_ms) *total_ms = ctx->prof_slots[index].total_ms;
    if (launches) *launches = ctx->prof_slots[index].launches;
    return (int)ctx->prof_slots.size();
}

int nae_stretch_plan_make(double rate, double pitch, size_t in_len, nae_stretch_plan* pl)
{
    return nae_stretch_plan_make_n(rate, pitch, NAE_FFT_N, in_len, pl);
}

int nae_stretch_plan_make_n(double rate, double pitch, int n_fft, size_t in_len, nae_stretch_plan* pl)
{
    return nae_stretch_plan_make_shift(rate, pitch, 1.0, 0, n_fft, in_len, pl);
}

int nae_stretch_plan_make_shift(double rate, double pitch, double formant_ratio, int lifter, int n_fft, size_t in_len, nae_stretch_plan* pl)
{
    if (!pl) return NAE_ERR_INVALID;
    memset(pl, 0, sizeof *pl);
    if (!nae_size_ok(n_fft)) return NAE_ERR_UNSUPPORTED;
    const int hop = n_fft / 4;
    if (!(rate > 0.0) || !(pitch > 0.0)) return NAE_ERR_INVALID;
    if (!std::isfinite(formant_ratio) || !(formant_ratio > 0.0) || lifter < 0 || lifter > n_fft / 4) return NAE_ERR_INVALID;
    if (formant_ratio < NAE_FORMANT_SHIFT_MIN || formant_ratio > NAE_FORMANT_SHIFT_MAX) return NAE_ERR_UNSUPPORTED;
    double tempo = 1.0 / pitch, rho = rate * pitch;
    if (fabs(tempo - 1.0) < 1e-6) tempo = 1.0;
    if (fabs(rho - 1.0) < 1e-6) rho = 1.0;
    pl->pv_on = tempo != 1.0 || nae_formant_stage_on(rho, lifter, formant_ratio);
    pl->rs_on = rho != 1.0;
    if (pl->pv_on && (tempo < NAE_TEMPO_MIN || tempo > NAE_TEMPO_MAX)) return NAE_ERR_UNSUPPORTED;
    if (pl->rs_on && (rho < NAE_RATE_MIN || rho > NAE_RATE_MAX)) return NAE_ERR_UNSUPPORTED;
    pl->tempo_eff = tempo;
    pl->rate_eff = rho;
    pl->ha_q24 = (int64_t)llround((double)hop * tempo * (double)(1 << NAE_HA_FRAC_BITS));
    pl->d0 = (int32_t)(pl->ha_q24 >> NAE_HA_FRAC_BITS);
    for (int i = 0; i < 2; i++) {
        const uint64_t d = (uint64_t)(pl->d0 + i);
        pl->r_q24[i] = (uint32_t)((((uint64_t)hop << NAE_R_FRAC_BITS) + d / 2) / d);
    }
    pl->step_q32 = (uint64_t)llround(rho * 4294967296.0);
    pl->out_len = (size_t)floor((double)in_len / (tempo * rho) + 0.5);
    pl->rs_first = pl->pv_on && pl->rs_on && rho > 1.0;
    size_t pv_out;
    if (pl->rs_first) {
        pl->mid_len = (size_t)floor((double)in_len / rho + 0.5);
        pv_out = pl->out_len;
    } else if (pl->rs_on) {
        if (pl->out_len == 0) pl->mid_len = 0;
        else {
            const unsigned __int128 pos = (unsigned __int128)(pl->out_len - 1) * pl->step_q32;
            pl->mid_len = (size_t)(pos >> 32) + NAE_RS_TAPS / 2 + 1;
        }
        pv_out = pl->mid_len;
    } else {
        pl->mid_len = pl->out_len;
        pv_out = pl->out_len;
    }
    pl->frames = pl->pv_on ? (pv_out + n_fft / 2 + hop - 1) / hop + 1 : 0;
    return NAE_OK;
}

static int check_sig(nae_ctx* ctx, const nae_sig* s, const char* what)
{
    if (!s || !s->base) return nae_fail(ctx, NAE_ERR_INVALID, what);
    return NAE_OK;
}

}

static int reserve_mid(nae_ctx* ctx, const nae_stretch_plan& pl, int ch, size_t n_streams, nae_sig* mid)
{
    const size_t mid_stride = (pl.mid_len + 3) & ~(size_t)3;
    const int rc = nae_ws_reserve(ctx, &ctx->ws_mid, &ctx->ws_mid_bytes, n_streams * ch * mid_stride * sizeof(float));
    if (rc) return rc;
    *mid = nae_sig{ctx->ws_mid, (size_t)ch * mid_stride, mid_stride, 1};
    return NAE_OK;
}

int nae_pv_opts_check(nae_ctx* ctx, unsigned flags, unsigned allowed, int n_fft, int lifter, const double* formant_ratio, nae_pv_opts* o)
{
    if (!ctx) return NAE_ERR_INVALID;
    if (flags & ~allowed) return nae_fail(ctx, NAE_ERR_INVALID, "unknown stretch flag");
    if (!nae_size_ok(n_fft)) return nae_fail(ctx, NAE_ERR_UNSUPPORTED, "vocoder: n_fft must be 512, 1024, 2048 or 4096");
    if ((flags & NAE_STRETCH_PHASE_LOCK) && n_fft != NAE_FFT_N) return nae_fail(ctx, NAE_ERR_UNSUPPORTED, "phase locking runs at n_fft = 1024 only");
    if (lifter < 0 || lifter > n_fft / 4) return nae_fail(ctx, NAE_ERR_INVALID, "formant lifter must be in [0, n_fft / 4]");
    *o = nae_pv_opts{n_fft, lifter, (flags & NAE_STRETCH_PHASE_LOCK) != 0, (flags & NAE_STRETCH_TRANSIENTS) != 0, formant_ratio != nullptr,
                     formant_ratio ? *formant_ratio : 1.0, (flags & NAE_STRETCH_LINK_CHANNELS) != 0};
    return NAE_OK;
}

int nae_pv_plan_make(nae_ctx* ctx, const nae_pv_opts& o, double rate, double pitch, size_t in_len, nae_stretch_plan* pl)
{
    const int rc = o.shift ? nae_stretch_plan_make_shift(rate, pitch, o.formant_ratio, o.lifter, o.n_fft, in_len, pl)
                           : nae_stretch_plan_make_n(rate, pitch, o.n_fft, in_len, pl);
    return rc ? nae_fail(ctx, rc, o.shift ? "rate/pitch/formant ratio outside the supported range" : "rate/pitch outside the supported range") : NAE_OK;
}

struct nae_mix_front {
    const nae_sig* a;
    const nae_sig* b;
    float va, vb;
};

static int stretch_block_impl(nae_ctx* ctx, const nae_pv_opts& o, double rate, double pitch, const nae_sig* src, size_t in_len, int ch,
                              size_t n_streams, const nae_sig* dst, const nae_mix_front* front, int stages)
{
    int rc;
    if ((rc = check_sig(ctx, src, "null source view")) || (rc = check_sig(ctx, dst, "null destination view"))) return rc;
    if (ch < 1 || ch > 2) return nae_fail(ctx, NAE_ERR_INVALID, "channel count must be 1 or 2");
    nae_stretch_plan pl;
    if ((rc = nae_pv_plan_make(ctx, o, rate, pitch, in_len, &pl))) return rc;
    bool mix_pending = front != nullptr && (stages & 1);
    auto run_mix = [&]() -> int {
        if (!mix_pending) return NAE_OK;
        mix_pending = false;
        const nae_sig ins[2] = {*front->a, *front->b};
        const float vol[2] = {front->va, front->vb};
        return nae_amix_sig_f32(ctx, ins, vol, 2, src, in_len, n_streams);
    };
    if (n_streams == 0 || pl.out_len == 0) return run_mix();
    if (!pl.pv_on && !pl.rs_on) {
        if ((rc = run_mix())) return rc;
        return (stages & 2) ? nae_launch_copy_sig(ctx, src, dst, in_len, ch, n_streams, false, 1.0f) : NAE_OK;
    }

    nae_sig mid{};
    if (pl.pv_on && pl.rs_on && (rc = reserve_mid(ctx, pl, ch, n_streams, &mid))) return rc;
    if (pl.rs_on) {
        rc = nae_ensure_rs_table(ctx, pl.rate_eff);
        if (rc) return rc;
    }
    const nae_sig* pv_src = src;
    size_t pv_in_len = in_len;
    const nae_sig* pv_dst = dst;
    long long pv_out_len = (long long)pl.out_len;
    if (pl.rs_first && !(stages & 1)) {
        pv_src = &mid;
        pv_in_len = pl.mid_len;
    } else if (pl.rs_first) {
        rc = 1;
        if (mix_pending && ch == 2) {
            rc = nae_launch_mix_resample(ctx, &pl, front->a, front->b, front->va, front->vb, src, in_len, n_streams, ctx->d_rs_tab, &mid);
            if (rc < 0) return rc;
            if (rc == 0) mix_pending = false;
        }
        if (rc == 1) {
            if ((rc = run_mix())) return rc;
            rc = nae_launch_resample(ctx, &pl, src, in_len, ch, n_streams, ctx->d_rs_tab, &mid, 0, pl.mid_len);
            if (rc) return rc;
        }
        pv_src = &mid;
        pv_in_len = pl.mid_len;
    } else if (pl.pv_on && pl.rs_on) {
        pv_dst = &mid;
        pv_out_len = (long long)pl.mid_len;
    }
    if ((rc = run_mix())) return rc;
    if (!(stages & 2)) return NAE_OK;
    if (pl.pv_on) {
        const nae_pv_run run = nae_pv_resolve(o, pl, ch);
        PvBlockShape sh;
        if ((rc = pv_block_shape(ctx, run, pl.frames, ch, n_streams, &sh))) return rc;
        const nae_pv_segment seg{0, (long long)pl.frames, (long long)pl.frames, pv_out_len, nullptr, nullptr};
        rc = nae_launch_pv_phase(ctx, run, &pl, pv_src, pv_in_len, ch, n_streams, sh.phase_tile, sh.tile, static_cast<uint32_t*>(ctx->ws_phase), &seg);
        if (rc) return rc;
        rc = nae_launch_pv_synth(ctx, run, &pl, pv_src, pv_in_len, ch, n_streams, sh.tile, sh.phase_tile, static_cast<uint32_t*>(ctx->ws_phase),
                                 pv_dst, &seg, sh.frames_per_step);
        if (rc) return rc;
    }
    if (pl.rs_on && !pl.rs_first) {
        const nae_sig* rs_src = pl.pv_on ? &mid : src;
        const size_t rs_src_len = pl.pv_on ? pl.mid_len : in_len;
        rc = nae_launch_resample(ctx, &pl, rs_src, rs_src_len, ch, n_streams, ctx->d_rs_tab, dst, 0, pl.out_len);
        if (rc) return rc;
    }
    return NAE_OK;
}

extern "C" {

int nae_stretch_block_f32(nae_ctx* ctx, double rate, double pitch, const nae_sig* src, size_t in_len, int ch,
                          size_t n_streams, const nae_sig* dst)
{
    return nae_stretch_block_ex_f32(ctx, rate, pitch, 0u, src, in_len, ch, n_streams, dst);
}

int nae_stretch_block_ex_f32(nae_ctx* ctx, double rate, double pitch, unsigned flags, const nae_sig* src, size_t in_len, int ch,
                             size_t n_streams, const nae_sig* dst)
{
    nae_pv_opts o;
    const int rc = nae_pv_opts_check(ctx, flags, NAE_STRETCH_PHASE_LOCK, NAE_FFT_N, 0, nullptr, &o);
    return rc ? rc : stretch_block_impl(ctx, o, rate, pitch, src, in_len, ch, n_streams, dst, nullptr, 3);
}

int nae_stretch_block_n_f32(nae_ctx* ctx, double rate, double pitch, unsigned flags, int n_fft, const nae_sig* src, size_t in_len, int ch,
                            size_t n_streams, const nae_sig* dst)
{
    return nae_stretch_block_formant_f32(ctx, rate, pitch, flags, n_fft, 0, src, in_len, ch, n_streams, dst);
}

int nae_stretch_formant_lifter(int sample_rate, int n_fft)
{
    if (!nae_size_ok(n_fft) || sample_rate <= 0) return 0;
    int q = sample_rate / 700;
    if (q < 1) q = 1;
    return q < n_fft / 4 ? q : n_fft / 4;
}

int nae_stretch_block_formant_f32(nae_ctx* ctx, double rate, double pitch, unsigned flags, int n_fft, int lifter, const nae_sig* src, size_t in_len,
                                  int ch, size_t n_streams, const nae_sig* dst)
{
    nae_pv_opts o;
    const int rc = nae_pv_opts_check(ctx, flags, kPvFlagsN, n_fft, lifter, nullptr, &o);
    return rc ? rc : stretch_block_impl(ctx, o, rate, pitch, src, in_len, ch, n_streams, dst, nullptr, 3);
}

int nae_stretch_block_formant_shift_f32(nae_ctx* ctx, double rate, double pitch, unsigned flags, int n_fft, int lifter, double formant_ratio,
                                        const nae_sig* src, size_t in_len, int ch, size_t n_streams, const nae_sig* dst)
{
    nae_pv_opts o;
    const int rc = nae_pv_opts_check(ctx, flags, kPvFlagsN, n_fft, lifter, &formant_ratio, &o);
    return rc ? rc : stretch_block_impl(ctx, o, rate, pitch, src, in_len, ch, n_streams, dst, nullptr, 3);
}

static int pv_tile_phase_impl(nae_ctx* ctx, const nae_pv_opts& o, double rate, double pitch, const nae_sig* src, size_t in_len, int ch, size_t n_streams,
                              int32_t* dst_host, size_t dst_capacity, size_t* n_tiles_out, size_t* tile_frames)
{
    if (!dst_host || !n_tiles_out || !tile_frames) return NAE_ERR_INVALID;
    int rc = check_sig(ctx, src, "null source view");
    if (rc) return rc;
    nae_stretch_plan pl;
    if ((rc = nae_pv_plan_make(ctx, o, rate, pitch, in_len, &pl))) return rc;
    if (!pl.pv_on) return nae_fail(ctx, NAE_ERR_STATE, "phase vocoder stage is bypassed for these parameters");
    const int tile = ctx->pv_tile > 0 ? ctx->pv_tile : 64;
    const size_t n_tiles = (pl.frames + tile - 1) / tile;
    *n_tiles_out = n_tiles;
    *tile_frames = (size_t)tile;
    const nae_pv_run run = nae_pv_resolve(o, pl, ch);
    const size_t bins = (size_t)o.n_fft / 2 + 1, pad = nae_pv_record_pad(o.n_fft);
    const size_t need = n_streams * ch * n_tiles * bins;
    if (dst_capacity < need) return nae_fail(ctx, NAE_ERR_INVALID, "destination too small");
    const size_t ws_bytes = nae_pv_workspace_bytes(false, o.n_fft, pl.frames, ch, n_streams, tile);
    if ((rc = nae_pv_reserve_ws(ctx, run, pl.frames, ch, n_streams, tile))) return rc;
    const nae_sig* pv_src = src;
    size_t pv_in_len = in_len;
    nae_sig mid{};
    if (pl.rs_first) {
        rc = reserve_mid(ctx, pl, ch, n_streams, &mid);
        if (rc) return rc;
        rc = nae_ensure_rs_table(ctx, pl.rate_eff);
        if (rc) return rc;
        rc = nae_launch_resample(ctx, &pl, src, in_len, ch, n_streams, ctx->d_rs_tab, &mid, 0, pl.mid_len);
        if (rc) return rc;
        pv_src = &mid;
        pv_in_len = pl.mid_len;
    }
    const nae_pv_segment seg{0, (long long)pl.frames, (long long)pl.frames, 0, nullptr, nullptr};
    rc = nae_launch_pv_phase(ctx, run, &pl, pv_src, pv_in_len, ch, n_streams, tile, tile, static_cast<uint32_t*>(ctx->ws_phase), &seg);
    if (rc) return rc;
    std::vector<int32_t> tmp(ws_bytes / sizeof(int32_t));
    hipError_t e = hipMemcpyAsync(tmp.data(), ctx->ws_phase, ws_bytes, hipMemcpyDeviceToHost, ctx->stream);
    if (e == hipSuccess) e = hipStreamSynchronize(ctx->stream);
    if (e != hipSuccess) return nae_check(ctx, e, "copy phase workspace");
    for (size_t rec = 0; rec < n_streams * ch * n_tiles; rec++)
        memcpy(dst_host + rec * bins, tmp.data() + rec * pad, bins * sizeof(int32_t));
    return NAE_OK;
}

int nae_debug_pv_tile_phase(nae_ctx* ctx, double rate, double pitch, const nae_sig* src, size_t in_len, int ch,
                            size_t n_streams, int32_t* dst_host, size_t dst_capacity, size_t* n_tiles_out,
                            size_t* tile_frames)
{
    return nae_debug_pv_tile_phase_ex(ctx, rate, pitch, 0u, src, in_len, ch, n_streams, dst_host, dst_capacity, n_tiles_out, tile_frames);
}

int nae_debug_pv_tile_phase_ex(nae_ctx* ctx, double rate, double pitch, unsigned flags, const nae_sig* src, size_t in_len, int ch,
                               size_t n_streams, int32_t* dst_host, size_t dst_capacity, size_t* n_tiles_out,
                               size_t* tile_frames)
{
    nae_pv_opts o;
    const int rc = nae_pv_opts_check(ctx, flags, NAE_STRETCH_PHASE_LOCK, NAE_FFT_N, 0, nullptr, &o);
    return rc ? rc : pv_tile_phase_impl(ctx, o, rate, pitch, src, in_len, ch, n_streams, dst_host, dst_capacity, n_tiles_out, tile_frames);
}

int nae_debug_pv_tile_phase_n(nae_ctx* ctx, double rate, double pitch, unsigned flags, int n_fft, const nae_sig* src, size_t in_len, int ch,
                              size_t n_streams, int32_t* dst_host, size_t dst_capacity, size_t* n_tiles_out, size_t* tile_frames)
{
    nae_pv_opts o;
    const int rc = nae_pv_opts_check(ctx, flags, kPvFlagsN, n_fft, 0, nullptr, &o);
    return rc ? rc : pv_tile_phase_impl(ctx, o, rate, pitch, src, in_len, ch, n_streams, dst_host, dst_capacity, n_tiles_out, tile_frames);
}

size_t nae_spectrum_frames(size_t T) { return nae_spectrum_frames_ex(T, NAE_FFT_N, NAE_HOP); }

int nae_spectrum_block_f32(nae_ctx* ctx, const nae_sig* src, size_t T, int ch, size_t n_streams, float* dst,
                           size_t dst_stream_stride)
{
    return nae_spectrum_block_ex_f32(ctx, NAE_FFT_N, NAE_HOP, src, T, ch, n_streams, dst, dst_stream_stride);
}

size_t nae_spectrum_frames_ex(size_t T, int n_fft, int hop)
{
    if (nae_spectrum_check(n_fft, hop) != NAE_OK) return 0;
    return T < (size_t)n_fft ? 0 : (T - (size_t)n_fft) / (size_t)hop + 1;
}

int nae_spectrum_block_ex_f32(nae_ctx* ctx, int n_fft, int hop, const nae_sig* src, size_t T, int ch, size_t n_streams, float* dst,
                              size_t dst_stream_stride)
{
    if (!ctx || !dst) return NAE_ERR_INVALID;
    const int chk = nae_spectrum_check(n_fft, hop);
    if (chk != NAE_OK)
        return nae_fail(ctx, chk, chk == NAE_ERR_UNSUPPORTED ? "spectrum: n_fft must be a power of two in [256, 4096]" : "spectrum: hop must be in [1, n_fft]");
    int rc = check_sig(ctx, src, "null source view");
    if (rc) return rc;
    if (ch < 1 || ch > 2) return nae_fail(ctx, NAE_ERR_INVALID, "channel count must be 1 or 2");
    return nae_launch_spectrum(ctx, n_fft, hop, src, T, ch, n_streams, dst, dst_stream_stride);
}

static int graph4_stages(nae_ctx* ctx, const nae_graph4* g, int mask)
{
// ... 27 lines not shown
```

### nodey-audio-editor_amd/csrc/nae_internal.h

```cpp
#pragma once
#include <hip/hip_runtime.h>
#include <stddef.h>
#include <stdint.h>
#include <vector>
#include "../../include/nae_gpu.h"
#include "../../include/nae_dsp_spec.h"

namespace nae { struct cf; }

struct nae_ctx {
    int device = 0;
    hipStream_t stream = nullptr;
    bool own_stream = false;
    char err[512] = {0};
    char name[256] = {0};
    int n_cu = 256;
    nae::cf* d_w512 = nullptr;
    nae::cf* d_t1024 = nullptr;
    float* d_hann = nullptr;
    unsigned* d_spec_ctr = nullptr;
    struct SpecAnyTab { float* hann = nullptr; nae::cf* tn = nullptr; nae::cf* wm = nullptr; };
    SpecAnyTab spec_any_tab[5];
    void* ws_phase = nullptr; size_t ws_phase_bytes = 0;
    void* ws_mid = nullptr;   size_t ws_mid_bytes = 0;
    float* d_rs_tab = nullptr; double rs_tab_rate = 0.0;
    std::vector<float> h_rs_tab;
    struct nae_wsola_cache* wsola_cache = nullptr;
    int pv_tile = 0;
    int pv_fps = 0;
    int fir_tile = 0;
    float* d_fir_spec = nullptr; int fir_spec_n_fft = 0;
    std::vector<float> h_fir_taps;
    int conv_tile = 0;
    int conv_ring = 0;
    float* d_conv_spec = nullptr; size_t conv_spec_floats = 0; int conv_spec_n_fft = 0, conv_spec_taps_ch = 0;
    std::vector<float> h_conv_taps;
    void* ws_conv = nullptr; size_t ws_conv_bytes = 0;
    double* d_eq_block = nullptr;
    std::vector<double> h_eq_coef;
    bool dbg_st_unfused = false;
    int dbg_td_nc = 0;
    bool dbg_no_mix_fuse = false;
    bool dbg_rs_single = false;
    bool dbg_rs_direct = false;
    bool dbg_spec_generic = false;
    bool dbg_spec_narrow = false;
    int dbg_spec_fine = 0, dbg_spec_fine_rounds = 0;
    int dbg_spec_chunk = 0;
    bool dbg_spec_any = false;
    bool dbg_pv_any = false;
    int dbg_pv_min_ptile = 0;
    int pv_flow = 1;
    bool pv_lean = false;
    std::vector<const void*> lds_attr_done;
    bool prof_on = false;
    struct ProfSlot { const char* name; double total_ms; uint64_t launches; };
    struct ProfPair { int slot; hipEvent_t a, b; };
    std::vector<ProfSlot> prof_slots;
    std::vector<ProfPair> prof_pairs;
};

struct NaeProfScope {
    nae_ctx* ctx; int idx;
    NaeProfScope(nae_ctx* c, const char* name);
    ~NaeProfScope();
};

static inline int nae_use_device(nae_ctx* ctx)
{
    int cur = -1;
    if (hipGetDevice(&cur) == hipSuccess && cur == ctx->device) return 0;
    return hipSetDevice(ctx->device) == hipSuccess ? 0 : -3 ;
}

#define NAE_KLAUNCH(ctx, name_str, ...)          \
    do {                                          \
        (void)nae_use_device(ctx);                \
        NaeProfScope nae_ps_(ctx, name_str);      \
        hipLaunchKernelGGL(__VA_ARGS__);          \
    } while (0)

struct nae_event { hipEvent_t ev; };

int nae_check(nae_ctx* ctx, hipError_t e, const char* what);
int nae_fail(nae_ctx* ctx, int code, const char* what);
int nae_ws_reserve(nae_ctx* ctx, void** p, size_t* have, size_t want);

int nae_launch_spectrum(nae_ctx* ctx, int n_fft, int hop, const nae_sig* src, size_t T, int ch, size_t n_streams, float* dst,
                        size_t dst_stream_stride);
void nae_spec_any_free(nae_ctx* ctx);
inline int nae_spectrum_check(int n_fft, int hop)
{
    if (n_fft < 256 || n_fft > 4096 || (n_fft & (n_fft - 1)) != 0) return NAE_ERR_UNSUPPORTED;
    if (hop < 1 || hop > n_fft) return NAE_ERR_INVALID;
    return NAE_OK;
}
inline bool nae_size_ok(int n_fft) { return n_fft == 512 || n_fft == 1024 || n_fft == 2048 || n_fft == 4096; }
double nae_bessel_i0(double x);
int nae_pick_tile(nae_ctx* ctx, int forced, size_t units, size_t n_sc, size_t resident, size_t min_tile, bool max_tiles_down);
struct nae_pv_segment {
    long long f_origin, f_count;
    long long f_limit;
    long long mid_limit;
    const uint32_t* carry_in;
    uint32_t* carry_out;
    bool carry_by_synth = false;
};
struct nae_pv_opts {
    int n_fft = NAE_FFT_N, lifter = 0;
    bool lock = false, transients = false, shift = false;
    double formant_ratio = 1.0;
    bool link = false;
};
constexpr unsigned kPvFlagsN = NAE_STRETCH_PHASE_LOCK | NAE_STRETCH_TRANSIENTS | NAE_STRETCH_LINK_CHANNELS;
int nae_pv_opts_check(nae_ctx* ctx, unsigned flags, unsigned allowed, int n_fft, int lifter, const double* formant_ratio, nae_pv_opts* o);
int nae_pv_plan_make(nae_ctx* ctx, const nae_pv_opts& o, double rate, double pitch, size_t in_len, nae_stretch_plan* pl);
inline bool nae_formant_stage_on(double rate_eff, int lifter, double formant_ratio)
{
    const double r = rate_eff / formant_ratio - 1.0;
    return lifter > 0 && (r <= -1e-6 || r >= 1e-6);
}
inline int nae_formant_lifter_eff(const nae_stretch_plan& pl, int lifter, double formant_ratio)
{
    return pl.pv_on && nae_formant_stage_on(pl.rate_eff, lifter, formant_ratio) ? lifter : 0;
}
inline float nae_formant_g(const nae_stretch_plan& pl, double formant_ratio) { return (float)(pl.rate_eff / formant_ratio); }
inline bool nae_plan_forced(const nae_stretch_plan& pl) { return pl.pv_on && pl.tempo_eff == 1.0; }
struct nae_pv_run {
    int n_fft; bool lock;
    int lifter;
    float g;
    bool forced;
    bool transients;
    bool link;
};
inline nae_pv_run nae_pv_resolve(const nae_pv_opts& o, const nae_stretch_plan& pl, int ch)
{
    const int lifter = nae_formant_lifter_eff(pl, o.lifter, o.formant_ratio);
    const bool forced = nae_plan_forced(pl);
    const bool stage = pl.pv_on && !forced;
    const bool transients = o.transients && stage;
    return {o.n_fft, o.lock, lifter, lifter > 0 ? nae_formant_g(pl, o.formant_ratio) : 0.0f, forced, transients,
            o.link && ch == 2 && stage && (o.lock || transients)};
}
enum class PvKernels { kShipped, kAny, kLock, kEnv };
struct nae_pv_route { PvKernels pass1, pass3; };
inline nae_pv_route nae_pv_route_of(const nae_ctx* ctx, const nae_pv_run& r)
{
    if (r.forced) return {PvKernels::kEnv, PvKernels::kEnv};
    if (r.lock) return {PvKernels::kLock, PvKernels::kLock};
    const PvKernels pass1 = r.n_fft != NAE_FFT_N || ctx->dbg_pv_any || r.transients || r.link ? PvKernels::kAny : PvKernels::kShipped;
    return {pass1, r.lifter > 0 ? PvKernels::kAny : pass1};
}
size_t nae_pv_workspace_bytes(bool lock, int n_fft, size_t n_frames, int ch, size_t n_streams, int tile);
int nae_pv_reserve_ws(nae_ctx* ctx, const nae_pv_run& r, size_t n_frames, int ch, size_t n_streams, int tile);
int nae_launch_pv_phase(nae_ctx* ctx, const nae_pv_run& r, const nae_stretch_plan* pl, const nae_sig* src, size_t in_len, int ch, size_t n_streams,
                        int tile, int synth_tile, uint32_t* phase_ws, const nae_pv_segment* seg);
int nae_launch_pv_synth(nae_ctx* ctx, const nae_pv_run& r, const nae_stretch_plan* pl, const nae_sig* src, size_t in_len, int ch, size_t n_streams,
                        int tile, int phase_tile, uint32_t* phase_ws, const nae_sig* out, const nae_pv_segment* seg, int frames_per_step);
size_t nae_pv_record_pad(int n_fft);
int nae_pv_resident(nae_ctx* ctx, const nae_pv_run& r, PvKernels pass3);
int nae_launch_resample(nae_ctx* ctx, const nae_stretch_plan* pl, const nae_sig* src, size_t src_len, int ch,
                        size_t n_streams, const float* d_tab, const nae_sig* out, size_t j_begin, size_t j_end);
int nae_launch_mix_resample(nae_ctx* ctx, const nae_stretch_plan* pl, const nae_sig* a, const nae_sig* b, float va, float vb,
                            const nae_sig* mix_out, size_t S, size_t n_streams, const float* d_tab, const nae_sig* out);
int nae_ensure_rs_table(nae_ctx* ctx, double rate_eff);
int nae_pick_pv_shape(nae_ctx* ctx, size_t frames, size_t n_sc, int* phase_tile, int* frames_per_step);
constexpr int kPhasePad = 520;

void nae_wsola_cache_free(nae_ctx* ctx);

int nae_fir_check(nae_ctx* ctx, int n_taps, int ch, int* n_fft);
size_t nae_fir_spec_floats(int n_fft);
int nae_fir_make_spec(nae_ctx* ctx, const float* taps_host, int n_taps, int n_fft, float* d_spec);
int nae_launch_fir(nae_ctx* ctx, int n_fft, const float* d_spec, const nae_sig* src, size_t in_len, int ch, size_t n_streams, const nae_sig* dst,
                   size_t b_origin, size_t b_stop);
int nae_pick_fir_tile(nae_ctx* ctx, int n_fft, size_t blocks, size_t n_sc);
void nae_fir_cache_free(nae_ctx* ctx);

constexpr size_t NAE_CONV_WS_BYTES = (size_t)256 << 20;
constexpr int NAE_CONV_MIN_SLAB = 8, NAE_CONV_HANDLE_SLAB = 64;
int nae_conv_check(nae_ctx* ctx, int n_taps, int taps_ch, int ch, int* n_fft);
int nae_conv_parts(int n_taps, int n_fft);
size_t nae_conv_spec_floats(int n_fft, int parts, int taps_ch);
size_t nae_conv_ring_floats(int n_fft, size_t n_sc, size_t ring);
int nae_conv_make_spec(nae_ctx* ctx, const float* taps_host, int n_taps, int taps_ch, int n_fft, float* d_spec);
int nae_launch_conv(nae_ctx* ctx, int n_fft, int parts, int taps_ch, const float* d_spec, float* d_ring, size_t ring, const nae_sig* src,
                    size_t in_len, int ch, size_t n_streams, const nae_sig* dst, size_t b_origin, size_t b_stop);
int nae_pick_conv_tile(nae_ctx* ctx, int n_fft);
size_t nae_pick_conv_ring(nae_ctx* ctx, int n_fft, int parts, size_t blocks, size_t n_sc);
void nae_conv_cache_free(nae_ctx* ctx);

size_t nae_eq_block_doubles();
int nae_eq_check(nae_ctx* ctx, const double* coef, int n_sections, int ch);
int nae_eq_make_block(nae_ctx* ctx, const double* coef, int n_sections, double* d_block);
int nae_launch_eq(nae_ctx* ctx, const double* d_block, int n_sections, const nae_sig* src, size_t in_len, int ch, size_t n_streams,
                  const nae_sig* dst, size_t c_origin, size_t c_stop, double* d_state);
void nae_eq_cache_free(nae_ctx* ctx);

int nae_dyn_check(nae_ctx* ctx, const nae_dyn_params* p, int ch);
size_t nae_dyn_detectors(const nae_dyn_params* p, int ch, size_t n_streams);
int nae_launch_dyn(nae_ctx* ctx, const nae_dyn_params* p, const nae_sig* src, size_t in_len, int ch, size_t n_streams, const nae_sig* dst,
                   size_t c_origin, size_t c_stop, double* d_state);

int nae_launch_copy_sig(nae_ctx* ctx, const nae_sig* src, const nae_sig* dst, size_t S, int ch, size_t n_streams,
                        bool scale, float volume);
```

### nodey-audio-editor_amd/csrc/pv_roles.h

```cpp
#pragma once
#include "stft_common.h"

namespace nae {

constexpr int kYCf = 520;
constexpr int kOlaQuarter = 256;

__device__ __forceinline__ void pipe_barrier() { asm volatile("s_waitcnt lgkmcnt(0)\n\ts_barrier" ::: "memory"); }

template <bool kHide = true>
__device__ __forceinline__ int pipe_lane(int lane)
{
    if (kHide) asm volatile("" : "+v"(lane));
    return lane;
}

__device__ __forceinline__ uint32_t pipe_inc(uint32_t qa, uint32_t qp, unsigned k, unsigned d, unsigned R)
{
    const uint32_t e = ((k * d) & (NAE_FFT_N - 1)) << 22;
    const int32_t dw = (int32_t)(qa - qp - e);
    const uint32_t adv = ((k * NAE_HOP) & (NAE_FFT_N - 1)) << 22;
    const long long scaled = ((long long)dw * (long long)(int32_t)R + (1ll << (NAE_R_FRAC_BITS - 1))) >> NAE_R_FRAC_BITS;
    return adv + (uint32_t)scaled;
}
// ... 66 lines not shown
}
__device__ __forceinline__ void load_fft_regs_global(FftRegs& R, const Tables& tb, int lane)
{
#pragma unroll
    for (int r = 0; r < 8; r++) R.w[r] = reinterpret_cast<const cf*>(tb.hann)[lane + 64 * r];
#pragma unroll
    for (int q = 0; q < 7; q++) { R.ta[q] = tb.w512[lane * (q + 1)]; R.tb[q] = tb.w512[8 * (lane & 7) * (q + 1)]; }
}

template <bool kRich>
__device__ __forceinline__ void r1_window_pass_a(cf (&va)[8], const cf (&raw)[8], const FftRegs& R, const float* hann, const cf* twa, int lane)
{
    if (kRich) {
#pragma unroll
        for (int r = 0; r < 8; r++) va[r] = cf{raw[r].x * R.w[r].x, raw[r].y * R.w[r].y};
        fft512_pad_a_tw(va, R.ta);
    } else {
        const int la = pipe_lane<true>(lane);
        const cf* hw = reinterpret_cast<const cf*>(hann) + la;
        const cf* ta = twa + la;
        cf w[8], tw[7];
#pragma unroll
        for (int r = 0; r < 8; r++) w[r] = lds_ld(hw + 64 * r);
#pragma unroll
        for (int q = 0; q < 7; q++) tw[q] = lds_ld(ta + 64 * q);
#pragma unroll
        for (int r = 0; r < 8; r++) va[r] = cf{raw[r].x * w[r].x, raw[r].y * w[r].y};
        fft512_pad_a_tw(va, tw);
    }
}

__device__ __forceinline__ void r1_store_z(cf* Z, const FftLds& L, const cf (&va)[8], int lane)
{
#pragma unroll
    for (int r = 0; r < 8; r++) lds_st(L.nat + 64 * r, va[r]);
    if (lane == 0) Z[512] = va[0];
}

struct PhaseLane {
    int h, k0, km0;
    bool dc;
    cf tk[2], tm[2], tms;

    __device__ __forceinline__ void init(const Tables& tb, int half, int lane)
    {
        h = half;
        k0 = lane + 128 * h;
        dc = (h == 0) && (lane == 0);
        km0 = dc ? 256 : 512 - k0;
#pragma unroll
        for (int i = 0; i < 2; i++) { tk[i] = tb.t1024[k0 + 64 * i]; tm[i] = tb.t1024[i == 0 ? km0 : 448 - k0]; }
        tms = tb.t1024[512 - k0];
    }
    __device__ __forceinline__ void read5(const uint32_t* q, uint32_t (&v)[5]) const
    {
        v[0] = q[k0]; v[1] = q[km0]; v[2] = q[k0 + 64]; v[3] = q[448 - k0];
        v[4] = q[512];
    }
    __device__ __forceinline__ void write5(uint32_t* q, const uint32_t (&v)[5]) const
    {
        q[k0] = v[0]; q[km0] = v[1]; q[k0 + 64] = v[2]; q[448 - k0] = v[3];
        if (dc) q[512] = v[4];
    }
    __device__ __forceinline__ void load_base(uint32_t (&qs)[5], const uint32_t* base_phase, const PvParams& p, const PipeItem& it) const
    {
        if (p.base_zero) {
#pragma unroll
            for (int q = 0; q < 5; q++) qs[q] = 0;
        } else {
            read5(base_phase + (it.sc * p.phase_tiles + (long long)it.tile * p.phase_step) * kT1024Pad, qs);
        }
    }
    __device__ __forceinline__ void read_z(const cf* Z, cf (&A)[2], cf (&B)[2], cf& z256) const
    {
        const cf* Zk = Z + k0;
        const cf* Zm = Z + 512 - k0;
#pragma unroll
        for (int i = 0; i < 2; i++) { A[i] = lds_ld(Zk + 64 * i); B[i] = lds_ld(Zm - 64 * i); }
        if (h == 0) z256 = lds_ld(Z + 256);
    }
    __device__ __forceinline__ void split(const cf (&A)[2], const cf (&B)[2], cf z256, cf (&va)[5]) const
    {
#pragma unroll
        for (int i = 0; i < 2; i++) {
            const cf E = cf{A[i].x + B[i].x, A[i].y - B[i].y};
            const cf O = cf{A[i].x - B[i].x, A[i].y + B[i].y};
            const cf P = cmul_tw(O, tk[i]);
            va[2 * i] = cf{E.x + P.y, E.y - P.x};
            const cf Em = cf{E.x, -E.y};
            const cf Om = cf{-O.x, O.y};
            const cf Pm = cmul_tw(Om, i == 0 ? tms : tm[i]);
            va[2 * i + 1] = cf{Em.x + Pm.y, Em.y - Pm.x};
        }
        va[4] = cf{0.0f, 0.0f};
        if (h == 0) {
            va[4] = va[1];
            const cf E = cf{z256.x + z256.x, z256.y - z256.y};
            const cf O = cf{z256.x - z256.x, z256.y + z256.y};
            const cf P = cmul_tw(O, tm[0]);
            if (dc) va[1] = cf{E.x + P.y, E.y - P.x};
        }
    }
    __device__ __forceinline__ void phases(const cf (&va)[5], uint32_t (&qa)[5]) const
    {
#pragma unroll
        for (int q = 0; q < 4; q++) qa[q] = atan2_q32(va[q].y, va[q].x);
        if (h == 0) qa[4] = (va[4].x < 0.0f) ? 0x80000000u : 0u;
    }
    __device__ __forceinline__ void inc_items(const uint32_t (&qa)[5], const uint32_t (&qv)[5], unsigned d, unsigned R, uint32_t (&inc)[5]) const
    {
        inc[0] = pipe_inc(qa[0], qv[0], (unsigned)k0, d, R);
        inc[1] = pipe_inc(qa[1], qv[1], (unsigned)km0, d, R);
        inc[2] = pipe_inc(qa[2], qv[2], (unsigned)(k0 + 64), d, R);
        inc[3] = pipe_inc(qa[3], qv[3], (unsigned)(448 - k0), d, R);
        inc[4] = (h == 0) ? pipe_inc(qa[4], qv[4], 512u, d, R) : 0u;
    }
    __device__ __forceinline__ void inc_of_frame(const PvParams& p, long long f, const uint32_t (&qa)[5], const uint32_t (&qprev)[5], uint32_t (&inc)[5]) const
    {
        if (f == 0) {
#pragma unroll
            for (int q = 0; q < 5; q++) inc[q] = qa[q];
        } else {
            const unsigned d = (unsigned)(frame_start(p, f) - frame_start(p, f - 1));
            const unsigned R = (d == (unsigned)p.d0) ? p.r_q24_0 : p.r_q24_1;
            inc_items(qa, qprev, d, R, inc);
        }
    }
    __device__ __forceinline__ void carry_store(const PvParams& p, long long sc, const uint32_t (&q)[5]) const { write5(p.carry_out + sc * kT1024Pad, q); }
    __device__ __forceinline__ void synth_items(cf* Y, const cf (&x)[5], const uint32_t (&qsv)[5], const uint32_t (&qav)[5]) const
    {
        const int kk = k0, km = km0;
        cf* Yk = Y + kk;
#pragma unroll
        for (int i = 0; i < 2; i++) {
            cf yk = pipe_rotate(x[2 * i], qsv[2 * i], qav[2 * i]);
            const cf ym = pipe_rotate(x[2 * i + 1], qsv[2 * i + 1], qav[2 * i + 1]);
            cf a = ym, b = yk;
            cf mk = ym;
            if (i == 0 && h == 0) {
                const float y512 = pipe_rotate(x[4], qsv[4], qav[4]).x;
                if (dc) { yk.y = 0.0f; mk = cf{y512, 0.0f}; b = ym; }
            }
            const cf E{yk.x + mk.x, yk.y - mk.y};
            const cf D{yk.x - mk.x, yk.y + mk.y};
            const cf Q{__builtin_fmaf(tk[i].x, D.x, tk[i].y * D.y), __builtin_fmaf(tk[i].x, D.y, -(tk[i].y * D.x))};
            lds_st(Yk + 64 * i, cf{E.x - Q.y, -(E.y + Q.x)});
            const cf Em{a.x + b.x, a.y - b.y};
            const cf Dm{a.x - b.x, a.y + b.y};
            const cf Qm{__builtin_fmaf(tm[i].x, Dm.x, tm[i].y * Dm.y), __builtin_fmaf(tm[i].x, Dm.y, -(tm[i].y * Dm.x))};
            lds_st(Y + (i == 0 ? km : 448 - kk), cf{Em.x - Qm.y, -(Em.y + Qm.x)});
        }
    }
};

template <int kG>
__device__ __forceinline__ void r2_running_phase(uint32_t (&qs)[5], uint32_t (&mine)[5], const uint32_t (&iv)[kG][5], int j)
{
    uint32_t base[5];
#pragma unroll
    for (int q = 0; q < 5; q++) { mine[q] = qs[q]; base[q] = qs[q]; }
#pragma unroll
    for (int i2 = 0; i2 < kG; i2++) {
#pragma unroll
        for (int q = 0; q < 5; q++) {
            base[q] += iv[i2][q];
            if (i2 <= j) mine[q] += iv[i2][q];
        }
    }
#pragma unroll
    for (int q = 0; q < 5; q++) qs[q] = base[q];
}

constexpr float kSynthGain = NAE_OLA_GAIN / 2048.0f;

__device__ __forceinline__ void r3_window(const cf (&zs)[8], const cf (&wn)[8], float (&y)[4][4])
{
#pragma unroll
    for (int r = 0; r < 8; r++) {
        const cf w = wn[r];
        y[r >> 1][2 * (r & 1)] = zs[r].x * w.x;
        y[r >> 1][2 * (r & 1) + 1] = -(zs[r].y * w.y);
    }
}
__device__ __forceinline__ void r3_ola_shift(float (&r0)[4], float (&r1)[4], float (&r2)[4], const float (&y)[4][4], float (&o)[4])
{
#pragma unroll
    for (int i = 0; i < 4; i++) {
        o[i] = (r0[i] + y[0][i]) * kSynthGain;
        r0[i] = r1[i] + y[1][i];
        r1[i] = r2[i] + y[2][i];
        r2[i] = y[3][i];
    }
}
__device__ __forceinline__ void r3_ola_finish(const float4 (&oq)[3], const float (&y0)[4], float (&o)[4])
{
    o[0] = oq[2].x; o[1] = oq[2].y; o[2] = oq[2].z; o[3] = oq[2].w;
    o[0] += oq[1].x; o[1] += oq[1].y; o[2] += oq[1].z; o[3] += oq[1].w;
    o[0] += oq[0].x; o[1] += oq[0].y; o[2] += oq[0].z; o[3] += oq[0].w;
#pragma unroll
    for (int i = 0; i < 4; i++) o[i] = (o[i] + y0[i]) * kSynthGain;
}
template <int kG>
__device__ __forceinline__ void r3_quarter_source(int slot, int j, int i, int t, int gens, int& sl, int& gen)
{
    const int rel = j - i;
    const int back = rel >= 0 ? 0 : (-rel + kG - 1) / kG;
    sl = slot - j + rel + back * kG;
    gen = (t - 1 - back + 2 * gens) % gens;
}

struct BlockOut { float* optr; long long out_fs; bool out_vec; };
__device__ __forceinline__ void r3_store_block(const PvParams& p, const PipeItem& it, const BlockOut& bo, long long be, const float (&o)[4], int ls)
{
    if (be >= it.b0 && be < it.b_end && be * NAE_HOP < p.mid_len) {
        float* pb = bo.optr + be * NAE_HOP * bo.out_fs;
        const __amdgpu_buffer_rsrc_t rs = __builtin_amdgcn_make_buffer_rsrc(pb, 0, -1, 0x00020000);
        auto st = [&](unsigned byte_off, float v) { __builtin_amdgcn_raw_buffer_store_b32(__float_as_uint(v), rs, (int)byte_off, 0, 0); };
        const unsigned fs4 = 4u * (unsigned)bo.out_fs;
        const unsigned oa = 2u * (unsigned)ls * fs4;
        if ((be + 1) * NAE_HOP <= p.mid_len) {
            if (bo.out_vec) {
                typedef unsigned u32x2 __attribute__((ext_vector_type(2)));
                __builtin_amdgcn_raw_buffer_store_b64(u32x2{__float_as_uint(o[0]), __float_as_uint(o[1])}, rs, (int)(8u * ls), 0, 0);
                __builtin_amdgcn_raw_buffer_store_b64(u32x2{__float_as_uint(o[2]), __float_as_uint(o[3])}, rs, (int)(512u + 8u * ls), 0, 0);
            } else {
                st(oa, o[0]); st(oa + fs4, o[1]); st(oa + 128u * fs4, o[2]); st(oa + 129u * fs4, o[3]);
            }
        } else {
            const int rem = (int)(p.mid_len - be * NAE_HOP);
            if (2 * ls + 0 < rem) st(oa, o[0]);
            if (2 * ls + 1 < rem) st(oa + fs4, o[1]);
            if (128 + 2 * ls < rem) st(oa + 128u * fs4, o[2]);
            if (129 + 2 * ls < rem) st(oa + 129u * fs4, o[3]);
        }
    }
}
__device__ __forceinline__ void r3_store_dense_half(float* stream_base, int pend_be, int c, cf ch0, cf ch1, int lx)
{
    const __amdgpu_buffer_rsrc_t rs = __builtin_amdgcn_make_buffer_rsrc(stream_base + (long long)pend_be * (2 * NAE_HOP), 0, -1, 0x00020000);
    typedef unsigned u32x4 __attribute__((ext_vector_type(4)));
    __builtin_amdgcn_raw_buffer_store_b128(u32x4{__float_as_uint(ch0.x), __float_as_uint(ch1.x), __float_as_uint(ch0.y), __float_as_uint(ch1.y)}, rs, 16 * lx, 1024 * c, 0);
}

}
```

### nodey-audio-editor_amd/csrc/stft_common.h

```cpp
#pragma once
#include "launch.h"
#include "stft_device.h"

namespace nae {

constexpr int kT1024Pad = kPhasePad;

struct Tables { const cf* w512; const cf* t1024; const float* hann; };
constexpr int kWaves = 8;
constexpr int kThreads = kWaves * 64;
constexpr size_t kLdsTablesPad = NAE_FFT_N * sizeof(float) + (kT1024Pad + 64 + kTwaCf) * sizeof(cf);

__device__ __forceinline__ void stage_tables(unsigned char* smem, const Tables& tb, int n_threads, float*& hann, cf*& t1024, cf*& w64, cf*& twa)
{
    hann = reinterpret_cast<float*>(smem);
    t1024 = reinterpret_cast<cf*>(smem + NAE_FFT_N * sizeof(float));
    w64 = t1024 + kT1024Pad;
    twa = w64 + 64;
    for (int i = threadIdx.x; i < NAE_FFT_N; i += n_threads) hann[i] = tb.hann[i];
    for (int i = threadIdx.x; i < NAE_FFT_BINS; i += n_threads) t1024[i] = tb.t1024[i];
    if (threadIdx.x < 64) w64[threadIdx.x] = tb.w512[8 * (threadIdx.x >> 3) * (threadIdx.x & 7)];
    fill_twa(twa, tb.w512, threadIdx.x, n_threads);
}

__device__ __forceinline__ int wave_id() { return __builtin_amdgcn_readfirstlane((int)(threadIdx.x >> 6)); }

struct PvParams {
    long long ha_q24;
    long long in_len;
    long long frames;
    long long mid_len;
    int d0;
    unsigned r_q24_0, r_q24_1;
    int ch;
    int tile;
    int n_tiles;
    long long f_origin;
    long long f_stop;
    int skip_from;
    int phase_step;
    int phase_tiles;
    int base_zero;
    uint32_t* carry_out;
    long long carry_frame;
};

inline PvParams make_pv_params(const nae_stretch_plan& pl, size_t in_len, int ch, int tile, const nae_pv_segment* seg)
{
    PvParams p;
    p.ha_q24 = pl.ha_q24;
    p.in_len = (long long)in_len;
    p.frames = seg ? seg->f_limit : (long long)pl.frames;
    p.mid_len = seg ? seg->mid_limit : (long long)pl.mid_len;
    p.d0 = pl.d0;
    p.r_q24_0 = pl.r_q24[0];
    p.r_q24_1 = pl.r_q24[1];
    p.ch = ch;
    p.tile = tile;
    p.f_origin = seg ? seg->f_origin : 0;
    const long long cnt = seg ? seg->f_count : (long long)pl.frames;
    p.f_stop = p.f_origin + cnt;
    p.n_tiles = (int)((cnt + tile - 1) / tile);
    p.skip_from = p.n_tiles;
    p.phase_step = 1;
    p.phase_tiles = p.n_tiles;
    p.carry_out = nullptr;
    p.carry_frame = -1;
    p.base_zero = 0;
    return p;
}

struct WaveTile { long long sc, s_idx; int tile, c; };
__device__ __forceinline__ WaveTile wave_tile(long long item, int n_tiles, int ch)
{
    const long long sc = item / n_tiles;
    return WaveTile{sc, sc / ch, (int)(item % n_tiles), (int)(sc % ch)};
}

__device__ __forceinline__ long long frame_start(const PvParams& p, long long f)
{
    return (((f - 1) * p.ha_q24 + (1ll << (NAE_HA_FRAC_BITS - 1))) >> NAE_HA_FRAC_BITS) - NAE_FFT_N / 2;
}

__device__ __forceinline__ void phases_of(const cf (&v)[8], cf nyq, uint32_t (&qa)[9])
{
#pragma unroll
    for (int r = 0; r < 8; r++) qa[r] = atan2_q32(v[r].y, v[r].x);
    qa[8] = (nyq.x < 0.0f) ? 0x80000000u : 0u;
}

__device__ __forceinline__ void phase_inc(const uint32_t (&qa)[9], const uint32_t (&qp)[9], uint32_t (&acc)[9],
                                          int kl, unsigned d, unsigned R)
{
#pragma unroll
    for (int r = 0; r < 9; r++) {
        const unsigned k = (r < 8) ? (unsigned)(kl + 64 * r) : 512u;
        const uint32_t e = ((k * d) & (NAE_FFT_N - 1)) << 22;
        const int32_t dw = (int32_t)(qa[r] - qp[r] - e);
        const uint32_t adv = ((k * NAE_HOP) & (NAE_FFT_N - 1)) << 22;
        const long long scaled = ((long long)dw * (long long)(int32_t)R + (1ll << (NAE_R_FRAC_BITS - 1))) >> NAE_R_FRAC_BITS;
        acc[r] += adv + (uint32_t)scaled;
    }
}

}

namespace nae {
struct PvJob {
    int n_fft;
    PvParams p;
    SigViewD src; OutViewD out;
    long long n_sc; bool unit_stride;
    uint32_t* phase_ws;
    int lifter; float g; bool transients, link;
};
}

int nae_launch_pv_pipe(nae_ctx* ctx, const nae::PvJob& j, int frames_per_step);
int nae_launch_pvlock_phase(nae_ctx* ctx, const nae::PvJob& j, int n_needed, uint32_t* maps, uint16_t* sig16, const uint32_t* carry_in,
                            uint32_t* carry_out);
int nae_launch_pvlock_synth(nae_ctx* ctx, const nae::PvJob& j);
int nae_launch_pvany_phase(nae_ctx* ctx, const nae::PvJob& j);
int nae_launch_pv_scan(nae_ctx* ctx, int n_fft, const char* name, uint32_t* phase_ws, long long n_sc, int n_tiles, const uint32_t* carry_in,
                       uint32_t* carry_out, int n_read, bool segmented);
int nae_launch_pvany_synth(nae_ctx* ctx, const nae::PvJob& j);
int nae_launch_pvenv(nae_ctx* ctx, const nae::PvJob& j);
```

Before: 44.14 billion.

## Move mix-node output stores from resample kernel into phase-vocoder pipeline kernel

When the graph mixes two stereo inputs before a resample-first pitch stage, the fused mix+resample kernel no longer stores the mix node's output. Instead the phase-vocoder pipeline kernel recomputes the mix in 64-frame pieces between its barriers and writes it, spreading those stores across otherwise memory-idle steps. The aim is to take the mix-output write traffic off the resample kernel's critical path. It adds eligibility checks, a new kernel template variant and register pressure in the pipeline kernel, plus re-reading the two inputs.

```diff
diff --git a/include/nae_gpu.h b/include/nae_gpu.h
--- a/include/nae_gpu.h
+++ b/include/nae_gpu.h
@@ -65,6 +65,7 @@
 int nae_debug_clock_ghz(nae_ctx* ctx, double* ghz);
 
 int nae_debug_set(nae_ctx* ctx, const char* key, long long value);
+int nae_debug_get(nae_ctx* ctx, const char* key, long long* value);
 
 int nae_debug_diff_u32(nae_ctx* ctx, const void* a, const void* b, size_t n_words, uint64_t* d_count);
 
diff --git a/nodey-audio-editor_amd/binding.py b/nodey-audio-editor_amd/binding.py
--- a/nodey-audio-editor_amd/binding.py
+++ b/nodey-audio-editor_amd/binding.py
@@ -18,7 +18,7 @@
     "nae_memcpy_h2d", "nae_memcpy_d2h", "nae_memcpy_d2d", "nae_memset", "nae_event_create", "nae_event_record",
     "nae_event_query", "nae_ctx_wait_event", "nae_debug_graph4_stages",
     "nae_event_elapsed_ms", "nae_event_destroy", "nae_prof_enable", "nae_prof_reset", "nae_prof_get",
-    "nae_malloc_host", "nae_free_host", "nae_debug_clock_ghz", "nae_debug_set", "nae_debug_diff_u32", "nae_fill_uniform_f32", "nae_gain_f32", "nae_gain_s16", "nae_gain_s32", "nae_gain_frame",
+    "nae_malloc_host", "nae_free_host", "nae_debug_clock_ghz", "nae_debug_set", "nae_debug_get", "nae_debug_diff_u32", "nae_fill_uniform_f32", "nae_gain_f32", "nae_gain_s16", "nae_gain_s32", "nae_gain_frame",
     "nae_deinterleave_f32", "nae_interleave_f32", "nae_copy_sig_f32", "nae_gain_sig_f32", "nae_amix_f32",
     "nae_amix_sig_f32", "nae_bimix_f32", "nae_bimix2_downmix_f32", "nae_bimix2_interleave_f32",
     "nae_to_f32_interleaved", "nae_clamp_f32", "nae_stretch_plan_make", "nae_stretch_block_f32",
@@ -140,6 +140,7 @@
         "nae_prof_get": (i, [vp, i, C.c_char_p, sz, P(d), P(C.c_uint64)]),
         "nae_malloc_host": (i, [vp, sz, P(vp)]), "nae_free_host": (i, [vp, vp]),
         "nae_debug_clock_ghz": (i, [vp, P(C.c_double)]), "nae_debug_set": (i, [vp, C.c_char_p, C.c_longlong]),
+        "nae_debug_get": (i, [vp, C.c_char_p, P(C.c_longlong)]),
         "nae_debug_diff_u32": (i, [vp, vp, vp, sz, vp]),
         "nae_fill_uniform_f32": (i, [vp, vp, sz, sz, sz, C.c_uint64, C.c_uint64]),
         "nae_gain_f32": (i, [vp, P(vp), P(vp), i, sz, f]), "nae_gain_s16": (i, [vp, P(vp), P(vp), i, sz, f]),
@@ -308,6 +309,11 @@
         self._ck(self.lib.nae_debug_set(self.h, key.encode(), int(value)))
         return self
 
+    def debug_get(self, key: str) -> int:
+        v = C.c_longlong()
+        self._ck(self.lib.nae_debug_get(self.h, key.encode(), C.byref(v)))
+        return v.value
+
     def event(self) -> C.c_void_p:
         e = C.c_void_p()
         self._ck(self.lib.nae_event_create(self.h, C.byref(e)))
diff --git a/nodey-audio-editor_amd/csrc/kernels_pvpipe.hip b/nodey-audio-editor_amd/csrc/kernels_pvpipe.hip
--- a/nodey-audio-editor_amd/csrc/kernels_pvpipe.hip
+++ b/nodey-audio-editor_amd/csrc/kernels_pvpipe.hip
@@ -17,10 +17,11 @@
 
 __device__ unsigned g_cu_arrivals[8 * 4 * 16];
 
-template <bool kUnit, int kG, bool kRich>
+template <bool kUnit, int kG, bool kRich, bool kMix = false>
 __global__ __launch_bounds__(kPipeThreads, kRich ? 4 : 8) void pv_pipe_kernel(SigViewD src, PvParams p, long long n_sc,
-                                                                            const uint32_t* __restrict__ base_phase, OutViewD out, Tables tb)
-{
+                                                                            const uint32_t* __restrict__ base_phase, OutViewD out, Tables tb, PvMixD mx)
+{
+    static_assert(!kMix || kG == 1, "mix pieces: one frame per step");
     static_assert(kPipeSlots % kG == 0, "a unit's frames share a workgroup");
     static_assert(kG == 1 || kRich, "the frame-interleaved modes run one workgroup per CU");
     constexpr int kUnits = kPipeSlots / kG;
@@ -91,6 +92,12 @@
         uint32_t hqa[5] = {0, 0, 0, 0, 0};
 #pragma unroll
         for (int q = 0; q < 5; q++) hx[q] = cf{0.0f, 0.0f};
+        const int piece0 = 2 * (role - 1) + c;
+        pipe_u32x2 ma, mb;
+        if (kMix) {
+            __builtin_amdgcn_s_waitcnt(0x0F70);
+            mix_piece_load(mx, it.s_idx, piece0, pipe_lane<true>(lane), ma, mb);
+        }
 #pragma unroll 1
         for (int t = 0; t < T; t++) {
             const int ia = kG * (t - 1) + j;
@@ -117,6 +124,7 @@
                 P.write5(x_inc(slot), inc);
             }
             pipe_barrier();
+            if (kMix) mix_piece_step(mx, it.s_idx, 4 * t + piece0, pipe_lane<true>(lane), ma, mb);
             if (kG == 1) now = __builtin_amdgcn_s_memtime();
             uint32_t qa[5] = {0, 0, 0, 0, 0};
             if (act_a) P.phases(va, qa);
@@ -472,18 +480,21 @@
 
 using namespace nae;
 
-template <int kG, typename K>
-static int pv_launch(nae_ctx* ctx, const char* name, K kernel, size_t lds, const PvJob& j)
+template <int kG, typename K, typename... More>
+static int pv_launch(nae_ctx* ctx, const char* name, K kernel, size_t lds, const PvJob& j, const More&... more)
 {
     const Tables tb{ctx->d_w512, ctx->d_t1024, ctx->d_hann};
     return nae_launch_tiles(ctx, name, "pv_pipe_kernel: grid too large", kernel, j.n_sc * j.p.n_tiles, kPipeSlots / kG, kPipeThreads, lds, j.src, j.p,
-                            j.n_sc, j.phase_ws, j.out, tb);
+                            j.n_sc, j.phase_ws, j.out, tb, more...);
 }
 
 template <int kG, bool kRich>
 static int pipe_launch(nae_ctx* ctx, const PvJob& j)
 {
-    return with_flags(j.unit_stride, [&](auto u) { return pv_launch<kG>(ctx, "pv_pipe_kernel", &pv_pipe_kernel<u.value, kG, kRich>, pipe_lds(kG), j); });
+    return with_flags(j.unit_stride, kG == 1 && j.mix.mix != nullptr, [&](auto u, auto mix) {
+        if constexpr (mix.value && kG != 1) return nae_fail(ctx, NAE_ERR_INVALID, "pv_pipe_kernel: mix pieces need one frame per step");
+        else return pv_launch<kG>(ctx, "pv_pipe_kernel", &pv_pipe_kernel<u.value, kG, kRich, mix.value>, pipe_lds(kG), j, j.mix);
+    });
 }
 template <int kG>
 static int flow_launch(nae_ctx* ctx, const PvJob& j)
@@ -491,15 +502,37 @@
     return with_flags(j.unit_stride, [&](auto u) { return pv_launch<kG>(ctx, "pv_flow_kernel", &pv_flow_kernel<u.value, kG>, flow_lds(kG), j); });
 }
 
+static bool pipe_one_per_cu(const nae_ctx* ctx, const PvJob& j, int frames_per_step)
+{
+    const int units = kPipeSlots / frames_per_step;
+    const long long groups = (j.n_sc * j.p.n_tiles + units - 1) / units;
+    return groups <= (long long)ctx->n_cu && !ctx->pv_lean;
+}
+static bool pipe_runs_flow(const nae_ctx* ctx, const PvJob& j, int frames_per_step)
+{
+    return pipe_one_per_cu(ctx, j, frames_per_step) && (ctx->pv_flow >= 2 || (ctx->pv_flow == 1 && frames_per_step == 1));
+}
+
+bool nae_pv_pipe_takes_mix(const nae_ctx* ctx, const PvJob& j, int frames_per_step)
+{
+    if (frames_per_step != 1 || j.p.ch != 2 || j.p.n_tiles != 1 || j.n_sc == 0 || pipe_runs_flow(ctx, j, frames_per_step)) return false;
+    long long f_end = j.p.f_stop + 3;
+    if (f_end > j.p.frames) f_end = j.p.frames;
+    const long long n = f_end - (j.p.f_origin > 0 ? j.p.f_origin - 1 : 0);
+    if (n <= 0) return false;
+    const bool dense_shape = j.out.fs == 2 && j.out.cs == 1;
+    const long long T = n + 2 + (dense_shape ? 1 : 0);
+    return (j.mix.S + kMixPiece - 1) / kMixPiece <= 4 * T;
+}
+
 int nae_launch_pv_pipe(nae_ctx* ctx, const PvJob& j, int frames_per_step)
 {
     const long long items = j.n_sc * j.p.n_tiles;
-    if (items == 0) return NAE_OK;
+    if (items == 0) return j.mix.mix ? nae_fail(ctx, NAE_ERR_INVALID, "pv_pipe_kernel: a mix without a launch") : NAE_OK;
     if (frames_per_step != 1 && frames_per_step != 2 && frames_per_step != 4) return nae_fail(ctx, NAE_ERR_INVALID, "pv_pipe_kernel: frames per step");
-    const int units = kPipeSlots / frames_per_step;
-    const long long groups = (items + units - 1) / units;
-    const bool one_per_cu = groups <= (long long)ctx->n_cu && !ctx->pv_lean;
-    if (one_per_cu && (ctx->pv_flow >= 2 || (ctx->pv_flow == 1 && frames_per_step == 1))) {
+    if (j.mix.mix && !nae_pv_pipe_takes_mix(ctx, j, frames_per_step)) return nae_fail(ctx, NAE_ERR_INVALID, "pv_pipe_kernel: this launch cannot write the mix");
+    const bool one_per_cu = pipe_one_per_cu(ctx, j, frames_per_step);
+    if (pipe_runs_flow(ctx, j, frames_per_step)) {
         if (frames_per_step == 1) return flow_launch<1>(ctx, j);
         if (frames_per_step == 2) return flow_launch<2>(ctx, j);
         return flow_launch<4>(ctx, j);
diff --git a/nodey-audio-editor_amd/csrc/kernels_stft.hip b/nodey-audio-editor_amd/csrc/kernels_stft.hip
--- a/nodey-audio-editor_amd/csrc/kernels_stft.hip
+++ b/nodey-audio-editor_amd/csrc/kernels_stft.hip
@@ -306,7 +306,7 @@
     float* mix; long long mix_ss, mix_cs, mix_fs;
 };
 
-template <int NS>
+template <int NS, bool kMixOut = true>
 __global__ __launch_bounds__(kRsThreads) void mix_resample_tile_kernel(MixFuseD f, RsParams p, const float* __restrict__ tab, OutViewD out,
                                                                int span_alloc, long long n_streams)
 {
@@ -383,14 +383,16 @@
                     for (int e = 0; e < 4; e++)
                         if (m + e < m_hi) *reinterpret_cast<float2*>(stg + 2 * e) = float2{y[2 * e], y[2 * e + 1]};
                 }
-                float* __restrict__ mx = f.mix + (s0 + k) * f.mix_ss;
-                if (own_all && mix_planar) {
-                    *reinterpret_cast<float4*>(mx + m) = float4{y[0], y[2], y[4], y[6]};
-                    *reinterpret_cast<float4*>(mx + f.mix_cs + m) = float4{y[1], y[3], y[5], y[7]};
-                } else {
-#pragma unroll
-                    for (int e = 0; e < 4; e++)
-                        if (own[e]) { mx[(m + e) * f.mix_fs] = y[2 * e]; mx[f.mix_cs + (m + e) * f.mix_fs] = y[2 * e + 1]; }
+                if (kMixOut) {
+                    float* __restrict__ mx = f.mix + (s0 + k) * f.mix_ss;
+                    if (own_all && mix_planar) {
+                        *reinterpret_cast<float4*>(mx + m) = float4{y[0], y[2], y[4], y[6]};
+                        *reinterpret_cast<float4*>(mx + f.mix_cs + m) = float4{y[1], y[3], y[5], y[7]};
+                    } else {
+#pragma unroll
+                        for (int e = 0; e < 4; e++)
+                            if (own[e]) { mx[(m + e) * f.mix_fs] = y[2 * e]; mx[f.mix_cs + (m + e) * f.mix_fs] = y[2 * e + 1]; }
+                    }
                 }
             }
         }
@@ -468,7 +470,7 @@
                          const nae_pv_segment* seg, uint32_t* phase_ws, const nae_sig* out)
 {
     return PvJob{r.n_fft, make_pv_params(pl, in_len, ch, tile, seg), to_view(src), out ? to_out(out) : OutViewD{}, (long long)n_streams * ch,
-                 src->frame_stride == 1, phase_ws, r.lifter, r.g, r.transients, r.link};
+                 src->frame_stride == 1, phase_ws, r.lifter, r.g, r.transients, r.link, PvMixD{}};
 }
 
 int nae_launch_pv_phase(nae_ctx* ctx, const nae_pv_run& r, const nae_stretch_plan* pl, const nae_sig* src, size_t in_len, int ch, size_t n_streams,
@@ -523,11 +525,15 @@
                               carry_out, n_needed, r.transients);
 }
 
-int nae_launch_pv_synth(nae_ctx* ctx, const nae_pv_run& r, const nae_stretch_plan* pl, const nae_sig* src, size_t in_len, int ch, size_t n_streams,
-                        int tile, int phase_tile, uint32_t* phase_ws, const nae_sig* out, const nae_pv_segment* seg, int frames_per_step)
+static int pv_synth_job(nae_ctx* ctx, const nae_pv_run& r, const nae_stretch_plan* pl, const nae_sig* src, size_t in_len, int ch, size_t n_streams,
+                        int tile, int phase_tile, uint32_t* phase_ws, const nae_sig* out, const nae_pv_segment* seg, const nae_pv_mix* mix, PvJob& j)
 {
     if (phase_tile <= 0 || tile < phase_tile || tile % phase_tile) return nae_fail(ctx, NAE_ERR_INVALID, "phase tile must divide the synthesis tile");
-    PvJob j = make_pv_job(r, *pl, src, in_len, ch, n_streams, tile, seg, phase_ws, out);
+    j = make_pv_job(r, *pl, src, in_len, ch, n_streams, tile, seg, phase_ws, out);
+    if (mix)
+        j.mix = PvMixD{static_cast<const float*>(mix->a->base), (long long)mix->a->stream_stride, static_cast<const float*>(mix->b->base),
+                       (long long)mix->b->stream_stride, mix->va, mix->vb, static_cast<float*>(mix->out->base), (long long)mix->out->stream_stride,
+                       (long long)mix->out->chan_stride, (long long)mix->S};
     PvParams& p = j.p;
     const long long cnt = p.f_stop - p.f_origin;
     p.phase_step = tile / phase_tile;
@@ -538,7 +544,31 @@
         p.carry_out = seg->carry_out;
         p.carry_frame = p.f_stop - 1;
     }
+    return NAE_OK;
+}
+
+bool nae_pv_synth_takes_mix(nae_ctx* ctx, const nae_pv_run& r, const nae_stretch_plan* pl, const nae_sig* src, size_t in_len, int ch, size_t n_streams,
+                            int tile, int phase_tile, const nae_sig* out, const nae_pv_segment* seg, int frames_per_step, const nae_pv_mix* mix)
+{
+    auto inter8 = [](const nae_sig* v) {
+        return v->chan_stride == 1 && v->frame_stride == 2 && (reinterpret_cast<uintptr_t>(v->base) & 7) == 0 && (v->stream_stride & 1) == 0;
+    };
+    if (ch != 2 || n_streams == 0 || mix->S == 0 || mix->out->frame_stride != 1 || !inter8(mix->a) || !inter8(mix->b)) return false;
+    if (nae_pv_route_of(ctx, r).pass3 != PvKernels::kShipped) return false;
+    PvJob j;
+    if (pv_synth_job(ctx, r, pl, src, in_len, ch, n_streams, tile, phase_tile, nullptr, out, seg, mix, j)) return false;
+    return nae_pv_pipe_takes_mix(ctx, j, frames_per_step);
+}
+
+int nae_launch_pv_synth(nae_ctx* ctx, const nae_pv_run& r, const nae_stretch_plan* pl, const nae_sig* src, size_t in_len, int ch, size_t n_streams,
+                        int tile, int phase_tile, uint32_t* phase_ws, const nae_sig* out, const nae_pv_segment* seg, int frames_per_step,
+                        const nae_pv_mix* mix)
+{
+    PvJob j;
+    const int rc = pv_synth_job(ctx, r, pl, src, in_len, ch, n_streams, tile, phase_tile, phase_ws, out, seg, mix, j);
+    if (rc) return rc;
     const PvKernels pass3 = nae_pv_route_of(ctx, r).pass3;
+    if (mix && pass3 != PvKernels::kShipped) return nae_fail(ctx, NAE_ERR_INVALID, "only the pipeline writes the mix node's output");
     if (pass3 == PvKernels::kEnv) return nae_launch_pvenv(ctx, j);
     if (pass3 == PvKernels::kLock) return nae_launch_pvlock_synth(ctx, j);
     if (pass3 == PvKernels::kAny) return nae_launch_pvany_synth(ctx, j);
@@ -585,7 +615,7 @@
 }
 
 int nae_launch_mix_resample(nae_ctx* ctx, const nae_stretch_plan* pl, const nae_sig* a, const nae_sig* b, float va, float vb,
-                            const nae_sig* mix_out, size_t S, size_t n_streams, const float* d_tab, const nae_sig* out)
+                            const nae_sig* mix_out, size_t S, size_t n_streams, const float* d_tab, const nae_sig* out, bool store_mix)
 {
     const double rho = (double)pl->step_q32 / 4294967296.0;
     long long span_need = 0;
@@ -614,8 +644,12 @@
         f.mix_ss = (long long)mix_out->stream_stride; f.mix_cs = (long long)mix_out->chan_stride; f.mix_fs = (long long)mix_out->frame_stride;
         OutViewD ov = to_out(out);
         ov.base += (long long)s0 * ov.ss;
-        NAE_KLAUNCH(ctx, "mix_resample_tile_kernel", (mix_resample_tile_kernel<4>), dim3(gx, (unsigned)((ns + 3) / 4)), dim3(256), lds,
-                    ctx->stream, f, p, d_tab, ov, span_alloc, (long long)ns);
+        if (store_mix)
+            NAE_KLAUNCH(ctx, "mix_resample_tile_kernel", (mix_resample_tile_kernel<4, true>), dim3(gx, (unsigned)((ns + 3) / 4)), dim3(256), lds,
+                        ctx->stream, f, p, d_tab, ov, span_alloc, (long long)ns);
+        else
+            NAE_KLAUNCH(ctx, "mix_resample_tile_kernel", (mix_resample_tile_kernel<4, false>), dim3(gx, (unsigned)((ns + 3) / 4)), dim3(256), lds,
+                        ctx->stream, f, p, d_tab, ov, span_alloc, (long long)ns);
         int rc = nae_check(ctx, hipGetLastError(), "mix_resample_tile_kernel");
         if (rc) return rc;
     }
diff --git a/nodey-audio-editor_amd/csrc/nae_api.hip b/nodey-audio-editor_amd/csrc/nae_api.hip
--- a/nodey-audio-editor_amd/csrc/nae_api.hip
+++ b/nodey-audio-editor_amd/csrc/nae_api.hip
@@ -232,6 +232,7 @@
     else if (k == "pv_fps" && one_of({0, 1, 2, 4})) ctx->pv_fps = (int)value;
     else if (k == "pv_flow" && one_of({0, 1, 2})) ctx->pv_flow = (int)value;
     else if (k == "pv_lean" && flag) ctx->pv_lean = value != 0;
+    else if (k == "mix_in_pv" && flag) ctx->mix_in_pv = value != 0;
     else if (k == "pv_min_ptile" && count) ctx->dbg_pv_min_ptile = (int)value;
     else if (k == "rs_single" && flag) ctx->dbg_rs_single = value != 0;
     else if (k == "rs_direct" && flag) ctx->dbg_rs_direct = value != 0;
@@ -246,6 +247,36 @@
     else if (k == "td_nc" && one_of({0, 1, 2, 4})) ctx->dbg_td_nc = (int)value;
     else if (k == "st_unfused" && flag) ctx->dbg_st_unfused = value != 0;
     else return nae_fail(ctx, NAE_ERR_INVALID, "nae_debug_set: unknown key or value out of range");
+    return NAE_OK;
+}
+
+int nae_debug_get(nae_ctx* ctx, const char* key, long long* value)
+{
+    if (!ctx || !key || !value) return NAE_ERR_INVALID;
+    const std::string k(key);
+    if (k == "pv_tile") *value = ctx->pv_tile;
+    else if (k == "fir_tile") *value = ctx->fir_tile;
+    else if (k == "conv_tile") *value = ctx->conv_tile;
+    else if (k == "conv_ring") *value = ctx->conv_ring;
+    else if (k == "pv_fps") *value = ctx->pv_fps;
+    else if (k == "pv_flow") *value = ctx->pv_flow;
+    else if (k == "pv_lean") *value = ctx->pv_lean;
+    else if (k == "mix_in_pv") *value = ctx->mix_in_pv;
+    else if (k == "mix_in_pv_launches") *value = (long long)ctx->mix_in_pv_launches;
+    else if (k == "pv_min_ptile") *value = ctx->dbg_pv_min_ptile;
+    else if (k == "rs_single") *value = ctx->dbg_rs_single;
+    else if (k == "rs_direct") *value = ctx->dbg_rs_direct;
+    else if (k == "no_mix_fuse") *value = ctx->dbg_no_mix_fuse;
+    else if (k == "spec_generic") *value = ctx->dbg_spec_generic;
+    else if (k == "spec_narrow") *value = ctx->dbg_spec_narrow;
+    else if (k == "spec_chunk") *value = ctx->dbg_spec_chunk;
+    else if (k == "spec_any") *value = ctx->dbg_spec_any;
+    else if (k == "pv_any") *value = ctx->dbg_pv_any;
+    else if (k == "spec_fine") *value = ctx->dbg_spec_fine;
+    else if (k == "spec_fine_rounds") *value = ctx->dbg_spec_fine_rounds;
+    else if (k == "td_nc") *value = ctx->dbg_td_nc;
+    else if (k == "st_unfused") *value = ctx->dbg_st_unfused;
+    else return nae_fail(ctx, NAE_ERR_INVALID, "nae_debug_get: unknown key");
     return NAE_OK;
 }
 
@@ -578,6 +609,20 @@
     float va, vb;
 };
 
+static void sig_extent(const nae_sig* v, size_t n_streams, int ch, size_t len, uintptr_t* lo, uintptr_t* hi)
+{
+    const size_t last = (n_streams - 1) * v->stream_stride + (size_t)(ch - 1) * v->chan_stride + (len ? len - 1 : 0) * v->frame_stride;
+    *lo = reinterpret_cast<uintptr_t>(v->base);
+    *hi = *lo + (last + 1) * sizeof(float);
+}
+static bool sigs_overlap(const nae_sig* u, size_t u_len, const nae_sig* v, size_t v_len, size_t n_streams)
+{
+    uintptr_t a0, a1, b0, b1;
+    sig_extent(u, n_streams, 2, u_len, &a0, &a1);
+    sig_extent(v, n_streams, 2, v_len, &b0, &b1);
+    return a0 < b1 && b0 < a1;
+}
+
 static int stretch_block_impl(nae_ctx* ctx, const nae_pv_opts& o, double rate, double pitch, const nae_sig* src, size_t in_len, int ch,
                               size_t n_streams, const nae_sig* dst, const nae_mix_front* front, int stages)
 {
@@ -610,15 +655,27 @@
     size_t pv_in_len = in_len;
     const nae_sig* pv_dst = dst;
     long long pv_out_len = (long long)pl.out_len;
+    bool mix_in_pv = false;
+    const nae_pv_mix pv_mix = front ? nae_pv_mix{front->a, front->b, front->va, front->vb, src, in_len} : nae_pv_mix{};
     if (pl.rs_first && !(stages & 1)) {
         pv_src = &mid;
         pv_in_len = pl.mid_len;
     } else if (pl.rs_first) {
         rc = 1;
         if (mix_pending && ch == 2) {
-            rc = nae_launch_mix_resample(ctx, &pl, front->a, front->b, front->va, front->vb, src, in_len, n_streams, ctx->d_rs_tab, &mid);
+            if (ctx->mix_in_pv && (stages & 2) && src->frame_stride == 1 && !sigs_overlap(src, in_len, front->a, in_len, n_streams) &&
+                !sigs_overlap(src, in_len, front->b, in_len, n_streams) && !sigs_overlap(src, in_len, dst, pl.out_len, n_streams)) {
+                const nae_pv_run run = nae_pv_resolve(o, pl, ch);
+                PvBlockShape sh;
+                if ((rc = pv_block_shape(ctx, run, pl.frames, ch, n_streams, &sh))) return rc;
+                const nae_pv_segment seg{0, (long long)pl.frames, (long long)pl.frames, pv_out_len, nullptr, nullptr};
+                mix_in_pv = nae_pv_synth_takes_mix(ctx, run, &pl, &mid, pl.mid_len, ch, n_streams, sh.tile, sh.phase_tile, pv_dst, &seg, sh.frames_per_step,
+                                                   &pv_mix);
+            }
+            rc = nae_launch_mix_resample(ctx, &pl, front->a, front->b, front->va, front->vb, src, in_len, n_streams, ctx->d_rs_tab, &mid, !mix_in_pv);
             if (rc < 0) return rc;
             if (rc == 0) mix_pending = false;
+            else mix_in_pv = false;
         }
         if (rc == 1) {
             if ((rc = run_mix())) return rc;
@@ -641,8 +698,9 @@
         rc = nae_launch_pv_phase(ctx, run, &pl, pv_src, pv_in_len, ch, n_streams, sh.phase_tile, sh.tile, static_cast<uint32_t*>(ctx->ws_phase), &seg);
         if (rc) return rc;
         rc = nae_launch_pv_synth(ctx, run, &pl, pv_src, pv_in_len, ch, n_streams, sh.tile, sh.phase_tile, static_cast<uint32_t*>(ctx->ws_phase),
-                                 pv_dst, &seg, sh.frames_per_step);
+                                 pv_dst, &seg, sh.frames_per_step, mix_in_pv ? &pv_mix : nullptr);
         if (rc) return rc;
+        if (mix_in_pv) ctx->mix_in_pv_launches++;
     }
     if (pl.rs_on && !pl.rs_first) {
         const nae_sig* rs_src = pl.pv_on ? &mid : src;
diff --git a/nodey-audio-editor_amd/csrc/nae_internal.h b/nodey-audio-editor_amd/csrc/nae_internal.h
--- a/nodey-audio-editor_amd/csrc/nae_internal.h
+++ b/nodey-audio-editor_amd/csrc/nae_internal.h
@@ -51,6 +51,8 @@
     bool dbg_pv_any = false;
     int dbg_pv_min_ptile = 0;
     int pv_flow = 1;
+    bool mix_in_pv = true;
+    uint64_t mix_in_pv_launches = 0;
     bool pv_lean = false;
     std::vector<const void*> lds_attr_done;
     bool prof_on = false;
@@ -156,14 +158,18 @@
 int nae_pv_reserve_ws(nae_ctx* ctx, const nae_pv_run& r, size_t n_frames, int ch, size_t n_streams, int tile);
 int nae_launch_pv_phase(nae_ctx* ctx, const nae_pv_run& r, const nae_stretch_plan* pl, const nae_sig* src, size_t in_len, int ch, size_t n_streams,
                         int tile, int synth_tile, uint32_t* phase_ws, const nae_pv_segment* seg);
+struct nae_pv_mix { const nae_sig* a; const nae_sig* b; float va, vb; const nae_sig* out; size_t S; };
+bool nae_pv_synth_takes_mix(nae_ctx* ctx, const nae_pv_run& r, const nae_stretch_plan* pl, const nae_sig* src, size_t in_len, int ch, size_t n_streams,
+                            int tile, int phase_tile, const nae_sig* out, const nae_pv_segment* seg, int frames_per_step, const nae_pv_mix* mix);
 int nae_launch_pv_synth(nae_ctx* ctx, const nae_pv_run& r, const nae_stretch_plan* pl, const nae_sig* src, size_t in_len, int ch, size_t n_streams,
-                        int tile, int phase_tile, uint32_t* phase_ws, const nae_sig* out, const nae_pv_segment* seg, int frames_per_step);
+                        int tile, int phase_tile, uint32_t* phase_ws, const nae_sig* out, const nae_pv_segment* seg, int frames_per_step,
+                        const nae_pv_mix* mix = nullptr);
 size_t nae_pv_record_pad(int n_fft);
 int nae_pv_resident(nae_ctx* ctx, const nae_pv_run& r, PvKernels pass3);
 int nae_launch_resample(nae_ctx* ctx, const nae_stretch_plan* pl, const nae_sig* src, size_t src_len, int ch,
                         size_t n_streams, const float* d_tab, const nae_sig* out, size_t j_begin, size_t j_end);
 int nae_launch_mix_resample(nae_ctx* ctx, const nae_stretch_plan* pl, const nae_sig* a, const nae_sig* b, float va, float vb,
-                            const nae_sig* mix_out, size_t S, size_t n_streams, const float* d_tab, const nae_sig* out);
+                            const nae_sig* mix_out, size_t S, size_t n_streams, const float* d_tab, const nae_sig* out, bool store_mix = true);
 int nae_ensure_rs_table(nae_ctx* ctx, double rate_eff);
 int nae_pick_pv_shape(nae_ctx* ctx, size_t frames, size_t n_sc, int* phase_tile, int* frames_per_step);
 constexpr int kPhasePad = 520;
diff --git a/nodey-audio-editor_amd/csrc/pv_roles.h b/nodey-audio-editor_amd/csrc/pv_roles.h
--- a/nodey-audio-editor_amd/csrc/pv_roles.h
+++ b/nodey-audio-editor_amd/csrc/pv_roles.h
@@ -242,6 +242,36 @@
         }
     }
 };
+
+typedef unsigned pipe_u32x2 __attribute__((ext_vector_type(2)));
+__device__ __forceinline__ int mix_piece_frames(const PvMixD& mx, int q)
+{
+    const long long left = mx.S - (long long)kMixPiece * q;
+    return left >= kMixPiece ? kMixPiece : left > 0 ? (int)left : 0;
+}
+__device__ __forceinline__ void mix_piece_load(const PvMixD& mx, long long s_idx, int q, int lane, pipe_u32x2& xa, pipe_u32x2& xb)
+{
+    const int nf = mix_piece_frames(mx, q);
+    const long long at = 2ll * kMixPiece * q;
+    const __amdgpu_buffer_rsrc_t ra = __builtin_amdgcn_make_buffer_rsrc(const_cast<float*>(mx.a) + s_idx * mx.a_ss + at, 0, 8 * nf, 0x00020000);
+    const __amdgpu_buffer_rsrc_t rb = __builtin_amdgcn_make_buffer_rsrc(const_cast<float*>(mx.b) + s_idx * mx.b_ss + at, 0, 8 * nf, 0x00020000);
+    xa = __builtin_amdgcn_raw_buffer_load_b64(ra, 8 * lane, 0, 0);
+    xb = __builtin_amdgcn_raw_buffer_load_b64(rb, 8 * lane, 0, 0);
+}
+__device__ __forceinline__ void mix_piece_step(const PvMixD& mx, long long s_idx, int q, int lane, pipe_u32x2& xa, pipe_u32x2& xb)
+{
+    const int nf = mix_piece_frames(mx, q);
+    float* m0 = mx.mix + s_idx * mx.mix_ss + (long long)kMixPiece * q;
+    const __amdgpu_buffer_rsrc_t r0 = __builtin_amdgcn_make_buffer_rsrc(m0, 0, 4 * nf, 0x00020000);
+    const __amdgpu_buffer_rsrc_t r1 = __builtin_amdgcn_make_buffer_rsrc(m0 + mx.mix_cs, 0, 4 * nf, 0x00020000);
+    float va = mx.va, vb = mx.vb;
+    asm volatile("" : "+s"(va), "+s"(vb));
+    const float yl = (0.0f + __uint_as_float(xa.x) * va) + __uint_as_float(xb.x) * vb;
+    const float yr = (0.0f + __uint_as_float(xa.y) * va) + __uint_as_float(xb.y) * vb;
+    mix_piece_load(mx, s_idx, q + 4, lane, xa, xb);
+    __builtin_amdgcn_raw_buffer_store_b32(__float_as_uint(yl), r0, 4 * lane, 0, 0);
+    __builtin_amdgcn_raw_buffer_store_b32(__float_as_uint(yr), r1, 4 * lane, 0, 0);
+}
 
 template <int kG>
 __device__ __forceinline__ void r2_running_phase(uint32_t (&qs)[5], uint32_t (&mine)[5], const uint32_t (&iv)[kG][5], int j)
diff --git a/nodey-audio-editor_amd/csrc/stft_common.h b/nodey-audio-editor_amd/csrc/stft_common.h
--- a/nodey-audio-editor_amd/csrc/stft_common.h
+++ b/nodey-audio-editor_amd/csrc/stft_common.h
@@ -106,6 +106,14 @@
 }
 
 namespace nae {
+struct PvMixD {
+    const float* a; long long a_ss;
+    const float* b; long long b_ss;
+    float va, vb;
+    float* mix; long long mix_ss, mix_cs;
+    long long S;
+};
+constexpr int kMixPiece = 64;
 struct PvJob {
     int n_fft;
     PvParams p;
@@ -113,9 +121,11 @@
     long long n_sc; bool unit_stride;
     uint32_t* phase_ws;
     int lifter; float g; bool transients, link;
+    PvMixD mix;
 };
 }
 
+bool nae_pv_pipe_takes_mix(const nae_ctx* ctx, const nae::PvJob& j, int frames_per_step);
 int nae_launch_pv_pipe(nae_ctx* ctx, const nae::PvJob& j, int frames_per_step);
 int nae_launch_pvlock_phase(nae_ctx* ctx, const nae::PvJob& j, int n_needed, uint32_t* maps, uint16_t* sig16, const uint32_t* carry_in,
                             uint32_t* carry_out);
```

Result: slower. 43.22 billion (-2.1%).
